# francois-rozet/sda

Measured on AMD Instinct MI355X. Metric: diffusion-steps/s (Kolmogorov 64x256x256 posterior sampling; unit = one predictor-corrector step of a 16-trajectory per-GPU shard), higher is better.
Workload: dtype f32; 1 GPU; kolmogorov256; per_gpu_batch=16, global_batch=16, guided=True, corrections=1, schedule_steps=1000, hipgraph_step=True, observation=fused Subsample (hand-written adjoint; no autograd through A), corrector_noise=row-keyed Philox (sda_randn_rows), parallelism=dp1 (batch-sharded, no in-loop collective), ranks_seen=1, process_group_live=False

## Files before the change

include/sda_hip.h:

```cpp
#ifndef SDA_HIP_H
#define SDA_HIP_H

#include <stdint.h>

#ifdef __cplusplus
extern "C" {
#endif

#define SDA_ABI_VERSION 14

enum {
    SDA_OK = 0,
    SDA_E_BADARG = -1,
    SDA_E_UNSUPPORTED = -2,
    SDA_E_LDS = -3
};

enum { SDA_ACT_NONE = 0, SDA_ACT_SILU = 1, SDA_ACT_RELU = 2, SDA_ACT_ELU = 3, SDA_ACT_GELU = 4, SDA_ACT_SELU = 5 };

int sda_abi_version(void);

typedef struct sda_conv_desc {
    const float* x;
    int64_t x_sn_outer, x_sn_inner;
    int32_t n_inner;
    int32_t x_n_off;
    int64_t x_sc, x_sy, x_sx;
    int32_t cx;
    const float* ctx;
    int64_t ctx_sn;
    int32_t cctx;
    int32_t n;
    int32_t hs, ws;
    int32_t up_h, up_w;
    int32_t zins_h, zins_w;
    const float* mod;
    int64_t mod_sn;
    const float* ln_mean;
    const float* ln_rstd;
    int32_t act_in;
    int32_t kh, kw, stride_h, stride_w, circular;
    const float* w;
    int32_t cin_pad, cout_pad;
    const float* bias;
    float* out;
    int32_t cout, ho, wo;
    const float* dact_z;
    int32_t act_d;
    const float* res;
    int32_t mt;
    int32_t explicit_pad, pad_h, pad_w;
    int64_t out_sn, out_sc, out_sy, out_sx;
    const float* w_wino4;
    int32_t pool_h, pool_w;
    const float* w_wino4_zp;
    const void* w_h2;
    float w_h2_scale;
    float x_amax_static;
    const float* x_amax;
    float* out_amax;
} sda_conv_desc;

int sda_conv_igemm(const sda_conv_desc* d, void* stream);
int sda_conv_parity4(const sda_conv_desc* d, void* stream);
int sda_conv_igemm_path(const sda_conv_desc* d);
int64_t sda_conv_igemm_lds_bytes(const sda_conv_desc* d);

typedef struct sda_wgrad_desc {
    sda_conv_desc conv;
    const float* g;
    float* dw;
    float* db;
    float* work;
    int32_t slabs;
    int32_t accumulate;
} sda_wgrad_desc;

int sda_conv_wgrad(const sda_wgrad_desc* d, void* stream);
int sda_conv_wgrad_slabs(const sda_wgrad_desc* d);
int64_t sda_conv_wgrad_work_floats(const sda_wgrad_desc* d);
int sda_conv_wgrad3_serves(const sda_wgrad_desc* d);
int64_t sda_conv_wgrad3_work_floats(const sda_wgrad_desc* d);
int sda_conv_wgrad3(const sda_wgrad_desc* d, void* stream);
int sda_conv_wgrad3x_serves(const sda_wgrad_desc* d);
int64_t sda_conv_wgrad3x_work_floats(const sda_wgrad_desc* d);
int sda_conv_wgrad3x(const sda_wgrad_desc* d, void* stream);
int sda_plane_sum(const float* x, const float* y, int n, int c, int64_t hw, float* out, int64_t out_sn, int sum_images,
                  int accumulate, void* stream);

typedef struct sda_block1d_desc {
    int32_t n, c, len;
    int32_t circular, act, unbiased;
    float eps;
    int32_t k_pad, m_pad;
    const float* a;
    const float* mod;
    int64_t mod_sn;
    const float* w1; const float* b1;
    const float* w2; const float* b2;
    float* z;
    float* mean; float* rstd;
    float* y;
    const float* g;
    float* gx;
} sda_block1d_desc;
int sda_block1d_fwd(const sda_block1d_desc* d, void* stream);
int sda_block1d_bwd(const sda_block1d_desc* d, void* stream);
int sda_block1d_tile(const sda_block1d_desc* d);

#define SDA_NET1D_MAXB 8
typedef struct sda_net1d_desc {
    int32_t n, len;
    int32_t cin, c, cout;
    int32_t nblocks;
    int32_t circular, act, unbiased;
    float eps;
    const float* x; int64_t x_sn, x_sc, x_sx;
    float* out; int64_t out_sn, out_sc, out_sx;
    const float* w;
    const float* bias;
    const float* mod[SDA_NET1D_MAXB];
    int64_t mod_sn;
    float* a_save; float* z_save; int64_t save_stride;
    float* mean_save; float* rstd_save; int64_t stat_stride;
} sda_net1d_desc;
int sda_net1d_fwd(const sda_net1d_desc* d, void* stream);
int sda_net1d_bwd(const sda_net1d_desc* d, void* stream);

typedef struct sda_net1d_fuse {
    float cx0, cx1, cn;
    const float* coef;
    const float* y; int64_t y_sn;
    int32_t p_start, p_step, p_stop;
    int32_t c_start, c_step, c_stop;
    float std, gamma;
    float* ghat;
    const float* eps;
    int32_t mode;
    float* xs;
    const float* step_coef;
    float* partial; int32_t partial_stride;
} sda_net1d_fuse;
int sda_net1d_fwd_fused(const sda_net1d_desc* d, const sda_net1d_fuse* f, void* stream);
int sda_net1d_bwd_fused(const sda_net1d_desc* d, const sda_net1d_fuse* f, void* stream);
int sda_net1d_tiles(const sda_net1d_desc* d);

typedef struct sda_net1d_train_desc {
    sda_net1d_desc net;
    float* tail_in;
    float* g_save; int64_t g_stride;
    float* mod_part; int32_t mod_tiles;
} sda_net1d_train_desc;
int sda_net1d_fwd_train(const sda_net1d_train_desc* t, void* stream);
int sda_net1d_bwd_train(const sda_net1d_train_desc* t, void* stream);

typedef struct sda_net1d_wgrad_desc {
    sda_net1d_desc net;
    const float* tail_in;
    const float* g_save; int64_t g_stride;
    const float* gout; int64_t gout_sn, gout_sc, gout_sx;
    const float* mod_part; int32_t mod_tiles;
    float* dw[2 + 2 * SDA_NET1D_MAXB];
    float* db[2 + 2 * SDA_NET1D_MAXB];
    float* dmod[SDA_NET1D_MAXB]; int64_t dmod_sn;
    float* work;
    int32_t slabs;
} sda_net1d_wgrad_desc;
int sda_net1d_wgrad(const sda_net1d_wgrad_desc* d, void* stream);
int sda_net1d_wgrad_slabs(const sda_net1d_wgrad_desc* d);
int64_t sda_net1d_wgrad_work_floats(const sda_net1d_wgrad_desc* d);

typedef struct sda_net1d_pack_desc {
    int32_t nblocks, cin, c, cout, cin_keep;
    const float* w[2 + 2 * SDA_NET1D_MAXB];
    const float* b[2 + 2 * SDA_NET1D_MAXB];
    float* wf; float* wb; float* bias;
} sda_net1d_pack_desc;
int sda_net1d_pack(const sda_net1d_pack_desc* p, void* stream);

int sda_step1d_prologue(const float* table, int row_len, int64_t* istep, const float* t_dev, int nt,
                        int alpha_kind, float eta, float k, int sigma_kind,
                        const float* freqs, int nf, const float* w0, const float* b0, int hidden, const float* w2, const float* b2, int e,
                        const float* wp, const float* bp, int cp,
                        float* out_coef, int64_t* out_step, float* mod, void* stream);
int sda_pc_correct_keyed(float* x, const float* eps, int b, int64_t per_sample, const float* partial, int nchunk, float tau,
                         float sigma, const float* coef_dev, uint64_t seed, int64_t row0, const int64_t* draw_dev, int64_t draw_mul,
                         int64_t draw_add, void* stream);

int sda_pack_conv_weight(const float* w, int cout, int cin, int kh, int kw, int transpose, int cin_keep,
                         float* dst, int k_pad, int m_pad, void* stream);

int sda_pack_conv_weight_wino4(const float* w, int cout, int cin, int transpose, int cin_keep, float* dst, int k_pad,
                               int m_pad, void* stream);
int sda_pack_conv_weight_wino4_zp(const float* w_wino4, int k_pad, int m_pad, float* dst, void* stream);
int64_t sda_wino4_zp_floats(int k_pad, int m_pad);

int sda_ln_stats(const float* x, int n, int c, int hw, const float* mod, int64_t mod_sn, float eps, int unbiased,
                 float* mean, float* rstd, void* stream);
int sda_ln_apply(const float* x, int n, int c, int hw, const float* mod, int64_t mod_sn, const float* mean,
                 const float* rstd, float* y, void* stream);
int sda_ln_bwd(const float* gh, const float* x, int n, int c, int h, int w, const float* mod, int64_t mod_sn,
               const float* mean, const float* rstd, int unbiased, int pool_h, int pool_w, const float* res, float* gx,
               void* stream);
int sda_ln_bwd_amax(const float* gh, const float* x, int n, int c, int h, int w, const float* mod, int64_t mod_sn,
                    const float* mean, const float* rstd, int unbiased, int pool_h, int pool_w, const float* res, float* gx,
                    float* amax, void* stream);

int sda_time_embed(const float* t, int nt, const float* freqs, int nf, const float* w0, const float* b0, int hidden,
                   const float* w2, const float* b2, int e, float* emb, void* stream);
int sda_linear_small(const float* x, int rows, int in_f, const float* w, const float* b, int out_f, float* y,
                     void* stream);

int sda_linear(const float* x, int rows, int in_f, const float* w, const float* b, int out_f, int trans_w, int act_in,
// ... 201 lines not shown
```

sda_amd/_lib.py:

```python
import ctypes
import os
from ctypes import POINTER, Structure, c_float, c_int, c_int32, c_int64, c_uint32, c_uint64, c_void_p

import torch

HERE = os.path.dirname(os.path.abspath(__file__))
LIB_PATH = os.environ.get('SDA_HIP_LIB') or os.path.join(HERE, 'lib', 'libsda_hip.so')

ACT_IDS = {None: 0, 'none': 0, 'SiLU': 1, 'ReLU': 2, 'ELU': 3, 'GELU': 4, 'SELU': 5}

c_fp = c_void_p


class ConvDesc(Structure):
    _fields_ = [
        ('x', c_fp),
        ('x_sn_outer', c_int64), ('x_sn_inner', c_int64),
        ('n_inner', c_int32),
        ('x_n_off', c_int32),
        ('x_sc', c_int64), ('x_sy', c_int64), ('x_sx', c_int64),
        ('cx', c_int32),
        ('ctx', c_fp),
        ('ctx_sn', c_int64),
        ('cctx', c_int32),
        ('n', c_int32),
        ('hs', c_int32), ('ws', c_int32),
        ('up_h', c_int32), ('up_w', c_int32),
        ('zins_h', c_int32), ('zins_w', c_int32),
        ('mod', c_fp),
        ('mod_sn', c_int64),
        ('ln_mean', c_fp),
        ('ln_rstd', c_fp),
        ('act_in', c_int32),
        ('kh', c_int32), ('kw', c_int32), ('stride_h', c_int32), ('stride_w', c_int32), ('circular', c_int32),
        ('w', c_fp),
        ('cin_pad', c_int32), ('cout_pad', c_int32),
        ('bias', c_fp),
        ('out', c_fp),
        ('cout', c_int32), ('ho', c_int32), ('wo', c_int32),
        ('dact_z', c_fp),
        ('act_d', c_int32),
        ('res', c_fp),
        ('mt', c_int32),
        ('explicit_pad', c_int32), ('pad_h', c_int32), ('pad_w', c_int32),
        ('out_sn', c_int64), ('out_sc', c_int64), ('out_sy', c_int64), ('out_sx', c_int64),
        ('w_wino4', c_fp),
        ('pool_h', ctypes.c_int32), ('pool_w', ctypes.c_int32),
        ('w_wino4_zp', c_fp),
        ('w_h2', ctypes.c_void_p), ('w_h2_scale', ctypes.c_float), ('x_amax_static', ctypes.c_float),
        ('x_amax', c_fp), ('out_amax', c_fp),
    ]


class Conv3dDesc(Structure):
    _fields_ = [
        ('x', c_fp), ('w', c_fp), ('bias', c_fp), ('z', c_fp), ('res', c_fp), ('out', c_fp),
        ('n', c_int32), ('cin', c_int32), ('cout', c_int32),
        ('in_size', c_int32 * 3), ('out_size', c_int32 * 3),
        ('k', c_int32 * 3), ('pad', c_int32 * 3), ('stride', c_int32 * 3), ('up', c_int32 * 3), ('dil', c_int32 * 3),
        ('circular', c_int32), ('act', c_int32), ('act_in', c_int32),
    ]


class Block1dDesc(Structure):
    _fields_ = [
        ('n', c_int32), ('c', c_int32), ('len', c_int32),
        ('circular', c_int32), ('act', c_int32), ('unbiased', c_int32),
        ('eps', c_float),
        ('k_pad', c_int32), ('m_pad', c_int32),
        ('a', c_fp),
        ('mod', c_fp),
        ('mod_sn', c_int64),
        ('w1', c_fp), ('b1', c_fp),
        ('w2', c_fp), ('b2', c_fp),
        ('z', c_fp),
        ('mean', c_fp), ('rstd', c_fp),
        ('y', c_fp),
        ('g', c_fp),
        ('gx', c_fp),
    ]


NET1D_MAXB = 8


class Net1dDesc(Structure):
    _fields_ = [
        ('n', c_int32), ('len', c_int32),
        ('cin', c_int32), ('c', c_int32), ('cout', c_int32),
        ('nblocks', c_int32),
        ('circular', c_int32), ('act', c_int32), ('unbiased', c_int32),
        ('eps', c_float),
        ('x', c_fp), ('x_sn', c_int64), ('x_sc', c_int64), ('x_sx', c_int64),
        ('out', c_fp), ('out_sn', c_int64), ('out_sc', c_int64), ('out_sx', c_int64),
        ('w', c_fp),
        ('bias', c_fp),
        ('mod', c_fp * NET1D_MAXB),
        ('mod_sn', c_int64),
        ('a_save', c_fp), ('z_save', c_fp), ('save_stride', c_int64),
        ('mean_save', c_fp), ('rstd_save', c_fp), ('stat_stride', c_int64),
    ]


class Net1dTrainDesc(Structure):
    _fields_ = [('net', Net1dDesc), ('tail_in', c_fp), ('g_save', c_fp), ('g_stride', c_int64), ('mod_part', c_fp), ('mod_tiles', c_int32)]


NET1D_MAXV = 2 + 2 * NET1D_MAXB


class Net1dWgradDesc(Structure):
    _fields_ = [
        ('net', Net1dDesc),
        ('tail_in', c_fp),
        ('g_save', c_fp), ('g_stride', c_int64),
        ('gout', c_fp), ('gout_sn', c_int64), ('gout_sc', c_int64), ('gout_sx', c_int64),
        ('mod_part', c_fp), ('mod_tiles', c_int32),
        ('dw', c_fp * NET1D_MAXV),
        ('db', c_fp * NET1D_MAXV),
        ('dmod', c_fp * NET1D_MAXB), ('dmod_sn', c_int64),
        ('work', c_fp),
        ('slabs', c_int32),
    ]


class Net1dPackDesc(Structure):
    _fields_ = [
        ('nblocks', c_int32), ('cin', c_int32), ('c', c_int32), ('cout', c_int32), ('cin_keep', c_int32),
        ('w', c_fp * NET1D_MAXV),
        ('b', c_fp * NET1D_MAXV),
        ('wf', c_fp), ('wb', c_fp), ('bias', c_fp),
    ]


MLP_MAXG = 32


class MlpDesc(Structure):
    _fields_ = [
        ('rows', c_int32), ('ngemm', c_int32),
        ('act', c_int32), ('unbiased', c_int32),
        ('eps', c_float),
        ('kind', c_int32 * MLP_MAXG),
        ('in_f', c_int32 * MLP_MAXG), ('out_f', c_int32 * MLP_MAXG),
        ('w_off', c_int32 * MLP_MAXG), ('b_off', c_int32 * MLP_MAXG),
        ('w', c_fp), ('bias', c_fp),
        ('x', c_fp), ('x_ld', c_int64),
        ('out', c_fp), ('out_ld', c_int64),
        ('a_save', c_fp), ('z_save', c_fp), ('save_stride', c_int64), ('save_ld', c_int32),
        ('mean_save', c_fp), ('rstd_save', c_fp), ('stat_stride', c_int64),
    ]


class MlpTrainDesc(Structure):
    _fields_ = [('mlp', MlpDesc), ('g_save', c_fp), ('g_stride', c_int64), ('g_ld', c_int32)]


class MlpWgradDesc(Structure):
    _fields_ = [
        ('rows', c_int32), ('ngemm', c_int32),
        ('act', c_int32),
        ('kind', c_int32 * MLP_MAXG),
        ('in_f', c_int32 * MLP_MAXG), ('out_f', c_int32 * MLP_MAXG),
        ('src', c_fp * MLP_MAXG), ('src_ld', c_int64 * MLP_MAXG),
        ('mean', c_fp * MLP_MAXG), ('rstd', c_fp * MLP_MAXG),
        ('g', c_fp * MLP_MAXG), ('g_ld', c_int64),
        ('dw', c_fp * MLP_MAXG), ('db', c_fp * MLP_MAXG),
        ('work', c_fp),
        ('slabs', c_int32), ('accumulate', c_int32),
    ]


ADAMW_MAXT = 32


class AdamWDesc(Structure):
    _fields_ = [
        ('ntensor', c_int32),
        ('decay', c_float), ('one_m_beta1', c_float), ('beta2', c_float), ('one_m_beta2', c_float),
        ('step_size', c_float), ('rsqrt_bc2', c_float), ('eps', c_float),
        ('p', c_fp * ADAMW_MAXT), ('g', c_fp * ADAMW_MAXT), ('m', c_fp * ADAMW_MAXT), ('v', c_fp * ADAMW_MAXT),
        ('fwd', c_fp * ADAMW_MAXT), ('bwd', c_fp * ADAMW_MAXT),
        ('numel', c_int64 * ADAMW_MAXT),
        ('pack_kind', c_int32 * ADAMW_MAXT),
        ('out_f', c_int32 * ADAMW_MAXT), ('in_f', c_int32 * ADAMW_MAXT),
        ('blk0', c_int32 * (ADAMW_MAXT + 1)),
    ]


class MlpWin(Structure):
    _fields_ = [
        ('nw', c_int32), ('len', c_int32), ('c', c_int32), ('emb_n', c_int32),
        ('x', c_fp), ('emb', c_fp),
        ('cx0', c_float), ('cx1', c_float), ('cn', c_float),
        ('coef', c_fp),
        ('y', c_fp), ('y_sn', c_int64),
        ('p_start', c_int32), ('p_step', c_int32), ('p_stop', c_int32),
        ('c_start', c_int32), ('c_step', c_int32), ('c_stop', c_int32),
        ('std', c_float), ('gamma', c_float),
        ('eps', c_fp), ('ghat', c_fp),
        ('gwin', c_fp),
    ]

# ... 207 lines not shown
```

sda_amd/build.py:

```python
import hashlib
import os
import subprocess
import sys

HERE = os.path.dirname(os.path.abspath(__file__))
CSRC = os.path.join(HERE, 'csrc')
LIBDIR = os.environ.get('SDA_LIBDIR') or os.path.join(HERE, 'lib')
ARCH = 'gfx950'
SOURCES = ['conv_igemm.hip', 'conv_wino4.hip', 'conv_small1d.hip', 'conv_few.hip', 'conv_par4.hip', 'conv_h2.hip', 'conv3d.hip', 'conv_wgrad.hip', 'conv_wgrad3.hip', 'block1d.hip', 'net1d.hip', 'net1d_train.hip', 'step1d.hip', 'norm.hip', 'elementwise.hip', 'linear.hip', 'mlp1d.hip', 'mlp_train.hip', 'optim.hip', 'train_loss.hip', 'observe.hip', 'metrics.hip', 'noise.hip', 'chain.hip', 'probe.hip']
HIPCC = os.environ.get('HIPCC', '/opt/rocm/bin/hipcc')
EXTRA_FLAGS = os.environ.get('SDA_EXTRA_HIPCC_FLAGS', '').split()
EMU_SOURCES = ['conv_igemm.hip', 'conv_wgrad.hip', 'conv_wgrad3.hip', 'chain.hip', 'mlp_train.hip', 'net1d_train.hip', 'optim.hip']
CONV_PARTS = 4


def _digest(deps, flags=()):
    h = hashlib.sha256()
    for d in deps:
        h.update(os.path.basename(d).encode())
        with open(d, 'rb') as f:
            h.update(f.read())
    h.update(' '.join(flags).encode())
    return h.hexdigest()


def _newer(target, deps, flags=()):
    stamp = target + '.stamp'
    if not os.path.exists(target) or not os.path.exists(stamp):
        return True
    with open(stamp) as f:
        return f.read().strip() != _digest(deps, flags)


def _stamp(target, deps, flags=()):
    with open(target + '.stamp', 'w') as f:
        f.write(_digest(deps, flags))


def _headers():
    hs = [os.path.join(CSRC, f) for f in os.listdir(CSRC) if f.endswith('.hpp')]
    hs.append(os.path.join(os.path.dirname(HERE), 'include', 'sda_hip.h'))
    return hs


def build(force=False, verbose=False):
    os.makedirs(LIBDIR, exist_ok=True)
    objs = []
    hdrs = _headers()
    procs = []
    units = []
    for src in SOURCES:
        if src == 'conv_igemm.hip':
            units += [(src, f'_p{k}', [f'-DSDA_CONV_PART={k}']) for k in range(CONV_PARTS)]
        else:
            units.append((src, '', []))
    for src, suffix, flags in units:
        sp = os.path.join(CSRC, src)
        if not os.path.exists(sp):
            continue
        obj = os.path.join(LIBDIR, src.replace('.hip', suffix + '.o'))
        objs.append(obj)
        cflags = ['-O3', '-std=c++17', '-fPIC', '-ffp-contract=off'] + flags + EXTRA_FLAGS
        if force or _newer(obj, [sp] + hdrs, cflags):
            cmd = [HIPCC, f'--offload-arch={ARCH}'] + cflags + ['-c', sp, '-o', obj]
            if verbose:
                print(' '.join(cmd))
            procs.append((src + suffix, obj, [sp] + hdrs, cflags, subprocess.Popen(cmd, stdout=subprocess.PIPE, stderr=subprocess.STDOUT)))
    for src, obj, deps, cflags, p in procs:
        out, _ = p.communicate()
        if p.returncode != 0:
            raise RuntimeError(f'hipcc failed on {src}:\n{out.decode()}')
        _stamp(obj, deps, cflags)
    lib = os.path.join(LIBDIR, 'libsda_hip.so')
    if force or procs or _newer(lib, objs):
        cmd = [HIPCC, f'--offload-arch={ARCH}', '-shared', '-fPIC', '-o', lib] + objs
        if verbose:
            print(' '.join(cmd))
        subprocess.check_call(cmd)
        _stamp(lib, objs)
    return lib


def build_emu(force=False):
    os.makedirs(LIBDIR, exist_ok=True)
    srcs = [os.path.join(CSRC, f) for f in EMU_SOURCES]
    lib = os.path.join(LIBDIR, 'libsda_emu.so')
    if force or _newer(lib, srcs + _headers()):
        subprocess.check_call([HIPCC, '--offload-host-only', '-DSDA_HOST_EMU', '-O2', '-std=c++17', '-fPIC',
                               '-ffp-contract=off', '-shared'] + srcs + ['-o', lib])
        _stamp(lib, srcs + _headers())
    return lib


if __name__ == '__main__':
    force = '--force' in sys.argv
    if '--emu' in sys.argv:
        print(build_emu(force))
    else:
        print(build(force, verbose=True))
```

sda_amd/csrc/conv_h2.hip:

```cpp
#include "sda_common.hpp"
#include <stdlib.h>
#include <type_traits>

typedef _Float16 h2_h8 __attribute__((ext_vector_type(8)));
typedef float h2_f4 __attribute__((ext_vector_type(4)));
typedef float h2_f16v __attribute__((ext_vector_type(16)));

#define H2_TS 16
#define H2_HS (H2_TS + 2)
#define H2_NPX (H2_HS * H2_HS)
#define H2_CK 16
#define H2_KQ 32
#define H2_PXB 80
#define H2_BTILE (H2_NPX * H2_PXB)
#define H2_ASLAB (9 * 3 * 2 * 1024)
#define H2_STAGE (H2_ASLAB + H2_BTILE)
#define H2_LDS (2 * H2_STAGE)
#define H2_BM 96
#define H2_BM_OF(MB) (32 * (MB))
#define H2_MB_OF(rows) ((rows) % 96 == 0 ? 3 : ((rows) % 64 == 0 ? 2 : 0))
#define H2_PRND 3
#define H2_TARGET_EXP 11

__host__ __device__ __forceinline__ float h2_scale_of(float amax) {
// ... 346 lines not shown
                float bias[16], opnd[2][16];
#pragma unroll
                for (int r = 0; r < 16; ++r) bias[r] = BIAS ? d.bias[co0 + 32 * m + (r & 3) + 8 * (r >> 2) + 4 * (lane >> 5)] : 0.f;
                if (EPI != 0) {
#pragma unroll
                    for (int f = 0; f < 2; ++f)
#pragma unroll
                        for (int r = 0; r < 16; ++r)
                            opnd[f][r] = op[obase + (int64_t)(32 * m + (r & 3) + 8 * (r >> 2)) * osc + (int64_t)(FROW * f) * OW];
                }
#pragma unroll
                for (int f = 0; f < 2; ++f)
#pragma unroll
                    for (int r = 0; r < 16; ++r) {
                        float v = acc[m][f][r] * inv + bias[r];
                        if (EPI == 1) v *= sda_dact(SDA_ACT_SILU, opnd[f][r]);
                        if (EPI == 2) v += opnd[f][r];
                        amax = fmaxf(amax, fabsf(v));
                        if (!(ABL & 8) || v == 1.2345e30f) d.out[obase + (int64_t)(32 * m + (r & 3) + 8 * (r >> 2)) * osc + (int64_t)(FROW * f) * OW] = v;
                    }
            }
        };
        using h2_c0 = std::integral_constant<int, 0>;
        using h2_c1 = std::integral_constant<int, 1>;
        using h2_c2 = std::integral_constant<int, 2>;
        if (d.dact_z) {
            if (d.bias) epilogue(h2_c1{}, std::true_type{}); else epilogue(h2_c1{}, std::false_type{});
        } else if (d.res) {
            if (d.bias) epilogue(h2_c2{}, std::true_type{}); else epilogue(h2_c2{}, std::false_type{});
        } else {
            if (d.bias) epilogue(h2_c0{}, std::true_type{}); else epilogue(h2_c0{}, std::false_type{});
        }
    }
    if (a.out_amax) {
#pragma unroll
        for (int off = 32; off > 0; off >>= 1) amax = fmaxf(amax, __shfl_down(amax, off, SDA_WAVE));
        if (lane == 0) atomicMax(reinterpret_cast<unsigned int*>(a.out_amax), __float_as_uint(amax));
    }
}

__global__ void pack_h2_kernel(const float* __restrict__ w, int cout, int cin, int transpose, float scale, h2_h8* __restrict__ dst,
                               int64_t units, int ntap, int mb) {
    const int64_t u = (int64_t)blockIdx.x * blockDim.x + threadIdx.x;
    if (u >= units) return;
    const int lane = (int)(u & 63);
    int64_t t = u >> 6;
    const int piece = (int)(t & 1); t >>= 1;
    const int m = (int)(t % mb); t /= mb;
    const int tap = (int)(t % ntap); t /= ntap;
    const int M = transpose ? cin : cout, K = transpose ? cout : cin;
    const int nchunk = K / H2_CK;
    const int chunk = (int)(t % nchunk);
    const int ct = (int)(t / nchunk);
    const int row = 32 * mb * ct + 32 * m + (lane & 31);
    h2_h8 out;
#pragma unroll
    for (int i = 0; i < 8; ++i) {
        const int k = H2_CK * chunk + 8 * (lane >> 5) + i;
        float v = 0.f;
        if (row < M) {
            const int co = transpose ? k : row, ci = transpose ? row : k, tp = transpose ? ntap - 1 - tap : tap;
            v = w[((int64_t)co * cin + ci) * ntap + tp] * scale;
        }
        const _Float16 h = (_Float16)v;
        out[i] = piece ? (_Float16)(v - (float)h) : h;
    }
    dst[u] = out;
}

extern "C" int64_t sda_conv_h2_packed_bytes(int cout, int cin, int transpose) {
    const int M = transpose ? cin : cout, K = transpose ? cout : cin;
    const int mb = M > 0 ? H2_MB_OF(M) : 0;
    if (M <= 0 || K <= 0 || !mb || K % H2_KQ) return 0;
    return (int64_t)(M / H2_BM_OF(mb)) * (K / H2_CK) * (9 * mb * 2 * 1024);
}

extern "C" float sda_conv_h2_scale(float amax) { return h2_scale_of(amax); }

extern "C" int sda_pack_conv_weight_h2(const float* w, int cout, int cin, int transpose, float w_amax, void* dst, void* stream) {
    const int64_t bytes = sda_conv_h2_packed_bytes(cout, cin, transpose);
    if (!w || !dst || bytes == 0) return SDA_E_BADARG;
    const int64_t units = bytes / 16;
    hipLaunchKernelGGL(pack_h2_kernel, dim3((unsigned)((units + 255) / 256)), dim3(256), 0, (hipStream_t)stream, w, cout, cin, transpose,
                       h2_scale_of(w_amax), reinterpret_cast<h2_h8*>(dst), units, 9, H2_MB_OF(transpose ? cin : cout));
    return sda_launch_status();
}

extern "C" int64_t sda_conv_h2_up_packed_bytes(int cout, int cin) {
    const int mb = cout > 0 ? H2_MB_OF(cout) : 0;
    if (cout <= 0 || cin <= 0 || !mb || cin % H2_KQ) return 0;
    return (int64_t)4 * (cout / H2_BM_OF(mb)) * (cin / H2_CK) * (4 * mb * 2 * 1024);
}

extern "C" int sda_pack_conv_weight_h2_up(const float* wsum, int cout, int cin, float w_amax, void* dst, void* stream) {
    const int64_t bytes = sda_conv_h2_up_packed_bytes(cout, cin);
    if (!wsum || !dst || bytes == 0) return SDA_E_BADARG;
    const int64_t units = bytes / 16;
    hipLaunchKernelGGL(pack_h2_kernel, dim3((unsigned)((units + 255) / 256)), dim3(256), 0, (hipStream_t)stream, wsum, 4 * cout, cin, 0,
                       h2_scale_of(w_amax), reinterpret_cast<h2_h8*>(dst), units, 4, H2_MB_OF(cout));
    return sda_launch_status();
}

extern "C" int64_t sda_conv_h2_rows_packed_bytes(int rows, int k, int ntap) {
    const int mb = rows > 0 ? H2_MB_OF(rows) : 0;
    if (rows <= 0 || k <= 0 || !mb || k % H2_KQ || (ntap != 1 && ntap != 2 && ntap != 4 && ntap != 9)) return 0;
    return (int64_t)(rows / H2_BM_OF(mb)) * (k / H2_CK) * ((int64_t)ntap * mb * 2 * 1024);
}

extern "C" int sda_pack_conv_weight_h2_rows(const float* w, int rows, int k, int ntap, float w_amax, void* dst, void* stream) {
    const int64_t bytes = sda_conv_h2_rows_packed_bytes(rows, k, ntap);
    if (!w || !dst || bytes == 0) return SDA_E_BADARG;
    const int64_t units = bytes / 16;
    hipLaunchKernelGGL(pack_h2_kernel, dim3((unsigned)((units + 255) / 256)), dim3(256), 0, (hipStream_t)stream, w, rows, k, 0,
                       h2_scale_of(w_amax), reinterpret_cast<h2_h8*>(dst), units, ntap, H2_MB_OF(rows));
    return sda_launch_status();
}

__global__ __launch_bounds__(256) void absmax_kernel(const float* __restrict__ x, int64_t n4, int64_t n, float* __restrict__ amax) {
    float m = 0.f;
    const h2_f4* x4 = reinterpret_cast<const h2_f4*>(x);
    const int64_t stride = (int64_t)gridDim.x * 256;
    int64_t i = (int64_t)blockIdx.x * 256 + threadIdx.x;
    for (; i + 3 * stride < n4; i += 4 * stride) {
        h2_f4 v[4];
#pragma unroll
        for (int k = 0; k < 4; ++k) v[k] = __builtin_nontemporal_load(x4 + i + k * stride);
#pragma unroll
        for (int k = 0; k < 4; ++k) m = fmaxf(fmaxf(fmaxf(m, fabsf(v[k][0])), fabsf(v[k][1])), fmaxf(fabsf(v[k][2]), fabsf(v[k][3])));
    }
    for (; i < n4; i += stride) {
        const h2_f4 v = __builtin_nontemporal_load(x4 + i);
        m = fmaxf(fmaxf(fmaxf(m, fabsf(v[0])), fabsf(v[1])), fmaxf(fabsf(v[2]), fabsf(v[3])));
    }
    if (blockIdx.x == 0 && threadIdx.x < (int)(n - 4 * n4)) m = fmaxf(m, fabsf(x[4 * n4 + threadIdx.x]));
#pragma unroll
    for (int off = 32; off > 0; off >>= 1) m = fmaxf(m, __shfl_down(m, off, SDA_WAVE));
    if ((threadIdx.x & 63) == 0) atomicMax(reinterpret_cast<unsigned int*>(amax), __float_as_uint(m));
}

__global__ void absmax_zero_kernel(float* __restrict__ amax) { amax[0] = 0.f; }

extern "C" int sda_absmax(const float* x, int64_t numel, float* amax, void* stream) {
    if (!x || !amax || numel <= 0 || (reinterpret_cast<uintptr_t>(x) & 15)) return SDA_E_BADARG;
    hipLaunchKernelGGL(absmax_zero_kernel, dim3(1), dim3(1), 0, (hipStream_t)stream, amax);
    const int64_t n4 = numel / 4;
    const int64_t want = (n4 + 255) / 256;
    const unsigned blocks = (unsigned)(want < 1 ? 1 : (want > 2048 ? 2048 : want));
    hipLaunchKernelGGL(absmax_kernel, dim3(blocks), dim3(256), 0, (hipStream_t)stream, x, n4, numel, amax);
    return sda_launch_status();
}

static bool h2_ok(const sda_conv_desc* d) {
    if (!d || !d->x || !d->out || !d->w_h2) return false;
    const bool up = d->up_h == 2 && d->up_w == 2;
    const bool pool = d->pool_h == 2 && d->pool_w == 2;
    const bool zins = d->zins_h == 2 && d->zins_w == 2;
    const bool s2 = d->stride_h == 2 && d->stride_w == 2;
    if (d->kh != 3 || d->kw != 3 || d->explicit_pad || (int)up + (int)pool + (int)zins + (int)s2 > 1) return false;
    if (!(s2 || (d->stride_h == 1 && d->stride_w == 1)) || !(up || (d->up_h == 1 && d->up_w == 1)) ||
        !(zins || (d->zins_h == 1 && d->zins_w == 1)) || !(pool || (d->pool_h <= 1 && d->pool_w <= 1)))
        return false;
    if (d->cctx != 0 || d->n_inner != 1 || d->x_n_off != 0) return false;
    const int ts = (pool || s2) ? 2 * H2_TS : H2_TS;
    const int mb = d->cout > 0 ? H2_MB_OF(d->cout) : 0;
    if (d->cx % H2_KQ || !mb || d->hs % ts || d->ws % ts) return false;
    if (s2 ? (2 * d->ho != d->hs || 2 * d->wo != d->ws) : (d->ho != ((up || zins) ? 2 : 1) * d->hs || d->wo != ((up || zins) ? 2 : 1) * d->ws)) return false;
    if (up && (d->dact_z || d->act_in != SDA_ACT_NONE)) return false;
    if (pool && (d->dact_z || d->res || d->bias || d->ln_mean || d->act_in != SDA_ACT_NONE)) return false;
    if ((zins || s2) && (d->dact_z || d->ln_mean || d->act_in != SDA_ACT_NONE)) return false;
    if (d->out_sn || d->out_sc || d->out_sy || d->out_sx) return false;
    if ((d->ln_mean == nullptr) != (d->ln_rstd == nullptr)) return false;
    if (d->mod && !d->ln_mean) return false;
    if (d->ln_mean && d->act_in != SDA_ACT_NONE) return false;
    if (d->act_in != SDA_ACT_NONE && d->act_in != SDA_ACT_SILU) return false;
    if (d->dact_z && d->act_d != SDA_ACT_SILU) return false;
    if (d->dact_z && d->res) return false;
    if (d->x_sc < 0 || d->x_sy < 0 || d->x_sx < 0 ||
        (int64_t)d->cx * d->x_sc + (int64_t)d->hs * d->x_sy + (int64_t)d->ws * d->x_sx >= (1LL << 31))
        return false;
    const int64_t tiles = (int64_t)d->n * (d->hs / ts) * (d->ws / ts) * (d->cout / H2_BM_OF(mb)) * ((up || zins) ? 4 : 1);
    return tiles >= 1 && tiles <= 0x3fffffffLL;
}

extern "C" int sda_conv_h2_supported(const sda_conv_desc* d) { return h2_ok(d) ? 1 : 0; }

template <int LOADER, int MODE>
static int h2_launch(const sda_conv_desc* d, const h2_args& a, unsigned grid, int lds, int mb, hipStream_t stream) {
    static bool set3[SDA_MAX_DEVICES], set2[SDA_MAX_DEVICES];
    int rc;
    if (mb == 3) {
        if ((rc = sda_raise_dyn_lds(reinterpret_cast<const void*>(conv_h2_kernel<LOADER, MODE, 0, 3>), lds, set3)) != SDA_OK) return rc;
        hipLaunchKernelGGL((conv_h2_kernel<LOADER, MODE, 0, 3>), dim3(grid), dim3(512), (size_t)lds, stream, *d, a);
    } else {
        if ((rc = sda_raise_dyn_lds(reinterpret_cast<const void*>(conv_h2_kernel<LOADER, MODE, 0, 2>), lds, set2)) != SDA_OK) return rc;
        hipLaunchKernelGGL((conv_h2_kernel<LOADER, MODE, 0, 2>), dim3(grid), dim3(512), (size_t)lds, stream, *d, a);
    }
    return sda_launch_status();
}

extern "C" int sda_conv_h2(const sda_conv_desc* d, void* stream) {
    if (!h2_ok(d)) return SDA_E_UNSUPPORTED;
    h2_args a;
    a.w = d->w_h2;
    a.w_scale = d->w_h2_scale;
    a.x_amax = d->x_amax;
    a.x_amax_static = d->x_amax_static;
    a.out_amax = d->out_amax;
    const bool up = d->up_h == 2, pool = d->pool_h == 2, zins = d->zins_h == 2, s2 = d->stride_h == 2;
    const bool planes = pool || s2;
    a.tiles_x = d->ws / (planes ? 2 * H2_TS : H2_TS);
    a.tiles_y = d->hs / (planes ? 2 * H2_TS : H2_TS);
    const int mb = H2_MB_OF(d->cout);
    a.n_ct = (d->cout / H2_BM_OF(mb)) * ((up || zins) ? 4 : 1);
    a.c16 = d->cx / H2_CK;
    a.nchunk = a.c16 * (planes ? 4 : 1);
    a.stagger = 0;
#ifdef SDA_H2_ABLATE
    { static const int stg = getenv("SDA_H2_STAGGER") ? atoi(getenv("SDA_H2_STAGGER")) : 0; a.stagger = stg; }
#endif
    if (!(a.w_scale > 0.f) || (!a.x_amax && !(a.x_amax_static > 0.f))) return SDA_E_BADARG;
    const int lds = H2_LDS;
    a.ntiles = (int)((int64_t)d->n * a.tiles_x * a.tiles_y * a.n_ct);
    int cus = sda_cu_count();
    if (cus <= 0) cus = 256;
    unsigned grid = (unsigned)(a.ntiles < cus ? a.ntiles : cus);
    if (grid >= 8) grid &= ~7u;
    int rc = SDA_OK;
#ifdef SDA_H2_ABLATE
    {
        static const int abl_env = getenv("SDA_H2_ABL") ? atoi(getenv("SDA_H2_ABL")) : 0;
        const int abl = mb == 3 ? abl_env : 0;
        static bool seta[16][SDA_MAX_DEVICES];
        const void* fn = nullptr;
#define H2_ABL_CASE(v) case v: fn = reinterpret_cast<const void*>(conv_h2_kernel<0, 0, v>); \
            if (!d->ln_mean && d->act_in == SDA_ACT_NONE) { if ((rc = sda_raise_dyn_lds(fn, lds, seta[v])) != SDA_OK) return rc; \
                hipLaunchKernelGGL((conv_h2_kernel<0, 0, v>), dim3(grid), dim3(512), (size_t)lds, (hipStream_t)stream, *d, a); return sda_launch_status(); } break;
        switch (abl) {
            H2_ABL_CASE(1) H2_ABL_CASE(2) H2_ABL_CASE(3) H2_ABL_CASE(4) H2_ABL_CASE(7) H2_ABL_CASE(8) H2_ABL_CASE(11) H2_ABL_CASE(15)
            default: break;
        }
    }
#endif
    if (zins) return h2_launch<0, 3>(d, a, grid, lds, mb, (hipStream_t)stream);
    if (s2) return h2_launch<0, 4>(d, a, grid, lds, mb, (hipStream_t)stream);
    if (pool) return h2_launch<0, 2>(d, a, grid, lds, mb, (hipStream_t)stream);
    if (up) return d->ln_mean ? h2_launch<2, 1>(d, a, grid, lds, mb, (hipStream_t)stream) : h2_launch<0, 1>(d, a, grid, lds, mb, (hipStream_t)stream);
    if (d->ln_mean) return h2_launch<2, 0>(d, a, grid, lds, mb, (hipStream_t)stream);
    if (d->act_in != SDA_ACT_NONE) return h2_launch<1, 0>(d, a, grid, lds, mb, (hipStream_t)stream);
    return h2_launch<0, 0>(d, a, grid, lds, mb, (hipStream_t)stream);
}
```

sda_amd/csrc/conv_igemm.hip:

```cpp
#include "sda_common.hpp"
#include <stdlib.h>
#include <string.h>

#ifndef SDA_CONV_CK
#define SDA_CONV_CK 8
#endif
#ifndef SDA_CONV_PART
#define SDA_CONV_PART 0
#endif
#define SDA_CONV_BP 128
#define SDA_CONV_THREADS 256
#define SDA_CONV_MAXPOS 4

struct ConvGeom {
    int cin;
    int hv, wv;
    int pad_h, pad_w;
    int tn, tr, tw;
    int tr_shift, tw_shift;
    int tiles_x, tiles_y, tiles_n;
    int n_pt, n_ct, grid;
    int in_rows, in_cols, plane;
    int S;
    int ntaps;
// ... 556 lines not shown
            float* slab = smem + 2 * BUF + wave * (16 * 32 * NT);
            const int64_t hw_w = g.o_sc;
            const int px4 = (lane & 15) * 4;
            const int64_t gb = conv_pix_out_base(d, g, wave * 32 * NT + px4, n0, oy0, ox0);
            const bool gvalid = gb >= 0;
            const int64_t gbs = gvalid ? gb : 0;
#pragma unroll
            for (int m = 0; m < MT; ++m) {
#pragma unroll
                for (int h = 0; h < 2; ++h) {
#pragma unroll
                    for (int q = 0; q < NT; ++q)
#pragma unroll
                        for (int rr = 0; rr < 8; ++rr)
                            slab[((rr & 3) + 8 * (rr >> 2) + 4 * khalf) * (32 * NT) + q * 32 + l31] = acc[m][q][8 * h + rr];
#pragma unroll
                    for (int it0 = 0; it0 < 4; it0 += 2) {
                        f32x4 val[2], zz[2], rs[2];
                        float bia[2];
#pragma unroll
                        for (int u = 0; u < 2; ++u) {
                            const int lr = (it0 + u) * 4 + (lane >> 4);
                            const int co = co0 + m * 32 + 16 * h + lr;
                            const bool ok = gvalid && co < d.cout;
                            const int64_t off = gbs + (int64_t)(ok ? co : 0) * hw_w;
                            val[u] = *reinterpret_cast<const f32x4*>(slab + lr * (32 * NT) + px4);
                            bia[u] = (d.bias && ok) ? d.bias[co] : 0.f;
                            if (d.dact_z) zz[u] = *reinterpret_cast<const f32x4*>(d.dact_z + off);
                            if (d.res) rs[u] = *reinterpret_cast<const f32x4*>(d.res + off);
                        }
                        if (d.dact_z) {
                            if (d.act_d == SDA_ACT_SILU) {
#pragma unroll
                                for (int u = 0; u < 2; ++u)
#pragma unroll
                                    for (int e = 0; e < 4; ++e) zz[u][e] = sda_dact(SDA_ACT_SILU, zz[u][e]);
                            } else {
#pragma unroll
                                for (int u = 0; u < 2; ++u)
#pragma unroll
                                    for (int e = 0; e < 4; ++e) zz[u][e] = sda_dact(d.act_d, zz[u][e]);
                            }
                        }
#pragma unroll
                        for (int u = 0; u < 2; ++u) {
                            const int lr = (it0 + u) * 4 + (lane >> 4);
                            const int co = co0 + m * 32 + 16 * h + lr;
                            f32x4 v = val[u] + bia[u];
                            if (d.dact_z) v *= zz[u];
                            if (d.res) v += rs[u];
                            if (gvalid && co < d.cout) *reinterpret_cast<f32x4*>(d.out + gbs + (int64_t)co * hw_w) = v;
                        }
                    }
                }
            }
            continue;
        }
        const int64_t hw_o = g.o_sc;
#pragma unroll
        for (int q = 0; q < NT; ++q) {
            const int64_t obase = conv_pix_out_base(d, g, (wave * NT + q) * 32 + l31, n0, oy0, ox0);
            const bool pvalid = obase >= 0;
            const int64_t ob = pvalid ? obase : 0;
#pragma unroll
            for (int m = 0; m < MT; ++m) {
                const int cb = co0 + m * 32 + 4 * khalf;
                float bia[16], zv[16], rv[16];
#pragma unroll
                for (int r = 0; r < 16; ++r) {
                    const int co = cb + (r & 3) + 8 * (r >> 2);
                    const bool ok = pvalid && co < d.cout;
                    const int64_t off = ob + (int64_t)(ok ? co : 0) * hw_o;
                    bia[r] = (d.bias && ok) ? d.bias[co] : 0.f;
                    zv[r] = d.dact_z ? d.dact_z[off] : 0.f;
                    rv[r] = d.res ? d.res[off] : 0.f;
                }
                if (d.dact_z) {
                    if (d.act_d == SDA_ACT_SILU) {
#pragma unroll
                        for (int r = 0; r < 16; ++r) zv[r] = sda_dact(SDA_ACT_SILU, zv[r]);
                    } else {
#pragma unroll
                        for (int r = 0; r < 16; ++r) zv[r] = sda_dact(d.act_d, zv[r]);
                    }
                } else {
#pragma unroll
                    for (int r = 0; r < 16; ++r) zv[r] = 1.f;
                }
#pragma unroll
                for (int r = 0; r < 16; ++r) {
                    const int co = cb + (r & 3) + 8 * (r >> 2);
                    const float v = (acc[m][q][r] + bia[r]) * zv[r] + rv[r];
                    if (pvalid && co < d.cout) d.out[ob + (int64_t)co * hw_o] = v;
                }
            }
        }
        }
    }
}

template <int MT, int NT, int SPAD, int KH, int KW, int CK>
static int conv_launch_ws(const sda_conv_desc* d, const ConvGeom& g, hipStream_t stream) {
    constexpr int lds = conv_ws_lds_bytes(NT, conv_ws_buf_floats(MT, SPAD, KH * KW, CK));
    static_assert(lds <= 160 * 1024, "stage buffers exceed the LDS");
    auto kern = conv_igemm_ws_kernel<MT, NT, SPAD, KH, KW, CK>;
    static bool attr_set[SDA_MAX_DEVICES];
    if (lds > 48 * 1024) {
        const int rc = sda_raise_dyn_lds(reinterpret_cast<const void*>(kern), lds, attr_set);
        if (rc != SDA_OK) return rc;
    }
    const int cus = sda_cu_count();
    if (!cus) return SDA_E_BADARG;
    const int per_cu = (conv_ws_two_per_cu(MT, NT, SPAD, CK) && 2 * lds <= 160 * 1024) ? 2 : 1;
    int grid = cus * per_cu;
    grid -= grid % 8;
    const int need = (g.grid + 7) / 8 * 8;
    if (grid > need) grid = need;
    if (grid < 8) grid = 8;
    hipLaunchKernelGGL(kern, dim3(grid), dim3(512), (size_t)lds, stream, *d, g);
    return sda_launch_status();
}

template <int MT, int NPOS>
static int conv_launch_t(const sda_conv_desc* d, const ConvGeom& g, hipStream_t stream) {
    auto kern = conv_igemm_kernel<MT, NPOS>;
    static bool attr_set[SDA_MAX_DEVICES];
    const int rc = g.lds_bytes > 48 * 1024 ? sda_raise_dyn_lds(reinterpret_cast<const void*>(kern), 160 * 1024, attr_set) : SDA_OK;
    if (rc != SDA_OK) return rc;
    hipLaunchKernelGGL(kern, dim3(g.grid), dim3(SDA_CONV_THREADS), (size_t)g.lds_bytes, stream, *d, g);
    return sda_launch_status();
}

typedef int (*conv_launch_fn)(const sda_conv_desc*, const ConvGeom&, hipStream_t);
conv_launch_fn sda_conv_variant_p0(const ConvPick& p), sda_conv_variant_p1(const ConvPick& p), sda_conv_variant_p2(const ConvPick& p),
    sda_conv_variant_p3(const ConvPick& p);
#define CONV_WS_VARIANT(KH, KW, MT, NT, SPAD, CK) {CONV_WS_PICK(KH, KW, MT, NT, SPAD, CK) conv_launch_ws<MT, NT, SPAD, KH, KW, CK>},
#define CONV_V1_VARIANT(MT, NPOS) {CONV_V1_PICK(MT, NPOS) conv_launch_t<MT, NPOS>},
#define CONV_PART_NAME_(stem, k) stem##k
#define CONV_PART_NAME(stem, k) CONV_PART_NAME_(stem, k)
conv_launch_fn CONV_PART_NAME(sda_conv_variant_p, SDA_CONV_PART)(const ConvPick& p) {
    static const struct { ConvPick pick; conv_launch_fn launch; } rows[] = {
        CONV_PART_NAME(CONV_ROWS_P, SDA_CONV_PART)(CONV_WS_VARIANT, CONV_V1_VARIANT)};
    for (const auto& v : rows)
        if (!memcmp(&v.pick, &p, sizeof(p))) return v.launch;
    return nullptr;
}

#if SDA_CONV_PART == 0
int sda_wino4_try(const sda_conv_desc* d, hipStream_t stream);
int sda_small1d_try(const sda_conv_desc* d, hipStream_t stream);
int sda_few_try(const sda_conv_desc* d, hipStream_t stream);
int sda_wino4_path(const sda_conv_desc* d), sda_small1d_path(const sda_conv_desc* d), sda_few_path(const sda_conv_desc* d);
typedef const sda_conv_desc* conv_dp;
struct ConvTier { bool (*offered)(conv_dp d); int (*run)(conv_dp d, hipStream_t stream); int (*path)(conv_dp d); };
static const ConvTier CONV_TIERS[] = {
    {[](conv_dp d) { return !!d->w_wino4; }, sda_wino4_try, [](conv_dp d) { const int p = sda_wino4_path(d); return p == 2 ? 5 : p ? 2 : 0; }},
    {[](conv_dp d) { return d->pool_h > 1 || d->pool_w > 1; }, nullptr, nullptr},
    {[](conv_dp d) { return d->kh == 1 && d->kw == 3; }, sda_small1d_try, [](conv_dp d) { return sda_small1d_path(d) ? 3 : 0; }},
    {[](conv_dp d) { return d->kh == 3 && d->kw == 3 && d->cout <= 16; }, sda_few_try, [](conv_dp d) { return sda_few_path(d) ? 4 : 0; }},
};

extern "C" int sda_conv_igemm(const sda_conv_desc* d, void* stream) {
    if (!d) return SDA_E_BADARG;
    for (const ConvTier& t : CONV_TIERS) {
        if (!t.offered(d)) continue;
        if (!t.run) return SDA_E_UNSUPPORTED;
        const int rc = t.run(d, (hipStream_t)stream);
        if (rc != SDA_E_UNSUPPORTED) return rc;
    }
    static const ConvSwitches sw = [] {
        const char *v1 = getenv("SDA_CONV_V1"), *nt = getenv("SDA_CONV_NT"), *ck32 = getenv("SDA_CONV_CK32"), *ck16 = getenv("SDA_CONV_CK16");
        return ConvSwitches{v1 != nullptr, nt ? atoi(nt) : 0, !(ck32 && atoi(ck32) == 0), !(ck16 && atoi(ck16) == 0)};
    }();
    ConvGeom g; ConvPick p;
    const int rc = conv_pick(d, sw, &g, &p);
    if (rc != SDA_OK) return rc;
    for (auto part : {sda_conv_variant_p0, sda_conv_variant_p1, sda_conv_variant_p2, sda_conv_variant_p3})
        if (conv_launch_fn launch = part(p)) return launch(d, g, (hipStream_t)stream);
    return SDA_E_UNSUPPORTED;
}

extern "C" int sda_conv_igemm_path(const sda_conv_desc* d) {
    if (!d) return SDA_E_BADARG;
    for (const ConvTier& t : CONV_TIERS) {
        if (!t.offered(d)) continue;
        if (!t.path) return SDA_E_UNSUPPORTED;
        if (const int id = t.path(d)) return id;
    }
    return 0;
}

extern "C" int64_t sda_conv_igemm_lds_bytes(const sda_conv_desc* d) {
    ConvGeom g;
    int rc = conv_plan(d, &g);
    return rc != SDA_OK ? (int64_t)rc : g.lds_bytes;
}


__global__ void pack_conv_weight_kernel(const float* __restrict__ w, int cout, int cin, int kh, int kw, int transpose,
                                        int cin_keep, float* __restrict__ dst, int k_pad, int m_pad) {
    const int64_t total = (int64_t)kh * kw * k_pad * m_pad;
    for (int64_t i = (int64_t)blockIdx.x * blockDim.x + threadIdx.x; i < total; i += (int64_t)gridDim.x * blockDim.x) {
        int mm = (int)(i % m_pad);
        int64_t r = i / m_pad;
        int kk = (int)(r % k_pad);
        int tap = (int)(r / k_pad);
        int dy = tap / kw, dx = tap % kw;
        float v = 0.f;
        if (!transpose) {
            int ci = kk, co = mm;
            if (ci < cin && co < cout) v = w[(((int64_t)co * cin + ci) * kh + dy) * kw + dx];
        } else {
            int co = kk, ci = mm;
            int sdy = kh - 1 - dy, sdx = kw - 1 - dx;
            if (ci < cin_keep && ci < cin && co < cout) v = w[(((int64_t)co * cin + ci) * kh + sdy) * kw + sdx];
        }
        dst[i] = v;
    }
}

extern "C" int sda_pack_conv_weight(const float* w, int cout, int cin, int kh, int kw, int transpose, int cin_keep,
                                    float* dst, int k_pad, int m_pad, void* stream) {
    if (!w || !dst || cout <= 0 || cin <= 0 || kh <= 0 || kw <= 0 || k_pad <= 0 || m_pad <= 0) return SDA_E_BADARG;
    int64_t total = (int64_t)kh * kw * k_pad * m_pad;
    int blocks = (int)((total + 255) / 256);
    if (blocks > 4096) blocks = 4096;
    hipLaunchKernelGGL(pack_conv_weight_kernel, dim3(blocks), dim3(256), 0, (hipStream_t)stream, w, cout, cin, kh, kw,
                       transpose, cin_keep, dst, k_pad, m_pad);
    return sda_launch_status();
}

#endif
#endif

#ifdef SDA_HOST_EMU
#include <vector>
extern "C" int sda_conv_igemm_emulate(const sda_conv_desc* dp) {
    ConvGeom g;
    int rc = conv_plan(dp, &g);
    if (rc != SDA_OK) return rc;
    const sda_conv_desc& d = *dp;
    constexpr int CK = SDA_CONV_CK;
    const int BM = g.bm, MT = d.mt;
    std::vector<float> s_w((size_t)g.ntaps * CK * BM), s_in((size_t)CK * g.S);
    std::vector<float> acc((size_t)SDA_CONV_THREADS * MT * 16);
    for (int b = 0; b < g.grid; ++b) {
        int ct, n0, oy0, ox0;
        conv_decode_block(g, conv_logical_block(b, g.grid), ct, n0, oy0, ox0);
        const int co0 = ct * BM;
        std::fill(acc.begin(), acc.end(), 0.f);
        for (int st = 0; st < g.nstage; ++st) {
            const int c0 = st * CK;
            for (int tid = 0; tid < SDA_CONV_THREADS; ++tid) {
                const int ROW4 = BM / 4, total4 = g.ntaps * CK * ROW4;
                for (int f = tid; f < total4; f += SDA_CONV_THREADS) {
                    int row = f / ROW4, c4 = f - row * ROW4, tap = row / CK, ck = row - tap * CK;
                    const float* src = d.w + ((int64_t)tap * d.cin_pad + c0 + ck) * d.cout_pad + co0 + c4 * 4;
                    for (int q = 0; q < 4; ++q) s_w[(size_t)row * BM + c4 * 4 + q] = src[q];
                }
                for (int pos = tid; pos < g.S; pos += SDA_CONV_THREADS) {
                    ConvPos ps = conv_decode_pos(d, g, pos, n0, oy0, ox0);
                    float mean = 0.f, rstd = 1.f;
                    if (d.ln_mean && ps.xoff >= 0) { mean = d.ln_mean[ps.stat]; rstd = d.ln_rstd[ps.stat]; }
                    for (int ck = 0; ck < CK; ++ck) s_in[(size_t)ck * g.S + pos] = conv_load_value(d, g, ps, c0 + ck, mean, rstd);
                }
            }
            for (int wave = 0; wave < 4; ++wave) {
                int dy = 0, dx = 0;
                for (int tap = 0; tap < g.ntaps; ++tap) {
                    for (int k2 = 0; k2 < CK / 2; ++k2) {
                        for (int m = 0; m < MT; ++m) {
                            float A[32][2], B[2][32];
                            for (int lane = 0; lane < 64; ++lane) {
                                int l31 = lane & 31, kh_ = lane >> 5, ck = 2 * k2 + kh_;
                                int pix = wave * 32 + l31;
                                int toff = dy * g.in_cols + dx + conv_pix_lds_base(d, g, pix);
                                B[kh_][l31] = s_in[(size_t)ck * g.S + toff];
                                A[l31][kh_] = s_w[((size_t)tap * CK + ck) * BM + m * 32 + l31];
                            }
                            for (int lane = 0; lane < 64; ++lane)
                                for (int r = 0; r < 16; ++r) {
                                    int i = mfma32_row(r, lane), j = lane & 31;
                                    float& c = acc[((size_t)(wave * 64 + lane) * MT + m) * 16 + r];
                                    c = fmaf(A[i][0], B[0][j], c);
                                    c = fmaf(A[i][1], B[1][j], c);
                                }
                        }
                    }
                    if (++dx == d.kw) { dx = 0; ++dy; }
                }
            }
        }
        for (int tid = 0; tid < SDA_CONV_THREADS; ++tid) {
            int lane = tid & 63, wave = tid >> 6, pix = wave * 32 + (lane & 31);
            int64_t obase = conv_pix_out_base(d, g, pix, n0, oy0, ox0);
            for (int m = 0; m < MT; ++m)
                for (int r = 0; r < 16; ++r)
                    conv_epilogue_store(d, g, obase, co0 + m * 32 + mfma32_row(r, lane), acc[((size_t)tid * MT + m) * 16 + r]);
        }
    }
    return SDA_OK;
}

extern "C" int sda_conv_igemm_pick(const sda_conv_desc* d, int force_v1, int nt, int ck32, int ck16, int out[16]) {
    ConvGeom g; ConvPick p;
    const int rc = conv_pick(d, ConvSwitches{force_v1 != 0, nt, ck32 != 0, ck16 != 0}, &g, &p);
    if (rc != SDA_OK) return rc;
    const int lds = p.kernel ? conv_ws_lds_bytes(p.nt, conv_ws_buf_floats(p.mt, p.spad, p.kh * p.kw, p.ck)) : (int)g.lds_bytes;
    const int geom[8] = {g.tn, g.tr, g.tw, g.S, g.grid, g.nstage, g.wide_out, lds};
    memcpy(out, &p, sizeof(p));
    memcpy(out + 8, geom, sizeof(geom));
    return SDA_OK;
}
extern "C" int sda_conv_igemm_variants(int* out, int cap) {
    static const ConvPick rows[] = {CONV_ROWS_P0(CONV_WS_PICK, CONV_V1_PICK) CONV_ROWS_P1(CONV_WS_PICK, CONV_V1_PICK)
                                    CONV_ROWS_P2(CONV_WS_PICK, CONV_V1_PICK) CONV_ROWS_P3(CONV_WS_PICK, CONV_V1_PICK)};
    if (cap >= (int)(sizeof(rows) / sizeof(rows[0]))) memcpy(out, rows, sizeof(rows));
    return (int)(sizeof(rows) / sizeof(rows[0]));
}

extern "C" void sda_pack_conv_weight_host(const float* w, int cout, int cin, int kh, int kw, int transpose, int cin_keep,
                                          float* dst, int k_pad, int m_pad) {
    const int64_t total = (int64_t)kh * kw * k_pad * m_pad;
    for (int64_t i = 0; i < total; ++i) {
        int mm = (int)(i % m_pad);
        int64_t r = i / m_pad;
        int kk = (int)(r % k_pad), tap = (int)(r / k_pad), dy = tap / kw, dx = tap % kw;
        float v = 0.f;
        if (!transpose) {
            if (kk < cin && mm < cout) v = w[(((int64_t)mm * cin + kk) * kh + dy) * kw + dx];
        } else {
            int sdy = kh - 1 - dy, sdx = kw - 1 - dx;
            if (mm < cin_keep && mm < cin && kk < cout) v = w[(((int64_t)kk * cin + mm) * kh + sdy) * kw + sdx];
        }
        dst[i] = v;
    }
// ... 3 lines not shown
```

sda_amd/csrc/conv_par4.hip:

```cpp
#include "sda_common.hpp"
#include <stdlib.h>

#define P4_CK 8
#define P4_TR 8
#define P4_TW 16
#define P4_HR (P4_TR + 1)
#define P4_HC (P4_TW + 1)
#define P4_NPOS (P4_HR * P4_HC)
#define P4_PLANE 176
#define P4_BM_OF(MT) (32 * (MT))
#define P4_WSZ_OF(MT) (9 * P4_CK * P4_BM_OF(MT))
#define P4_BUF_OF(MT) (P4_WSZ_OF(MT) + P4_CK * P4_PLANE)
#define P4_NLD ((P4_CK * P4_NPOS + 255) / 256)
#define P4_NW_OF(MT) ((P4_WSZ_OF(MT) / 4 + 255) / 256)

typedef float p4_f32x16 __attribute__((ext_vector_type(16)));
typedef float p4_f32x2 __attribute__((ext_vector_type(2)));

__device__ constexpr int P4_CL[9] = {0, 1, 1, 2, 2, 3, 3, 3, 3};
__device__ constexpr int P4_DY[9] = {0, 0, 0, 0, 1, 0, 0, 1, 1};
__device__ constexpr int P4_DX[9] = {0, 0, 1, 0, 0, 0, 1, 0, 1};

template <int MT>
__global__ __launch_bounds__(512, 2) void conv_par4_kernel(const sda_conv_desc d, int tiles_x, int tiles_y, int n_ct) {
    constexpr int P4_BM = P4_BM_OF(MT), P4_WSZ = P4_WSZ_OF(MT), P4_BUF = P4_BUF_OF(MT), P4_NW = P4_NW_OF(MT);
    extern __shared__ __attribute__((aligned(16))) float smem[];
    const int tid = threadIdx.x, lane = tid & 63, l31 = lane & 31, khalf = lane >> 5;
    const int wave = __builtin_amdgcn_readfirstlane(tid >> 6);
    int t = blockIdx.x;
    const int ct = t % n_ct; t /= n_ct;
    const int bx = t % tiles_x; t /= tiles_x;
    const int by = t % tiles_y;
    const int n = t / tiles_y;
    const int oy0 = by * P4_TR, ox0 = bx * P4_TW, co0 = ct * P4_BM;
    const int nstage = d.cin_pad / P4_CK;
    if (wave >= 4) {
        const int ptid = tid - 256;
        const float* gimg = d.x + (int64_t)n * d.x_sn_outer;
        unsigned goff[P4_NLD];
        int loff[P4_NLD];
        unsigned live = 0;
#pragma unroll
        for (int i = 0; i < P4_NLD; ++i) {
            const int e = ptid + 256 * i;
            const bool in = e < P4_CK * P4_NPOS;
            const int ch = in ? e / P4_NPOS : 0, pos = in ? e - ch * P4_NPOS : 0;
            const int hy = pos / P4_HC, hx = pos - hy * P4_HC;
            int y = oy0 + hy, x = ox0 + hx;
            bool ok = in;
            if (d.circular) {
                y = y >= d.hs ? y - d.hs : y;
                x = x >= d.ws ? x - d.ws : x;
            } else {
                ok = ok && y < d.hs && x < d.ws;
            }
            goff[i] = (unsigned)(ch * (int)d.x_sc + (ok ? y : 0) * (int)d.x_sy + (ok ? x : 0) * (int)d.x_sx);
            loff[i] = in ? P4_WSZ + ch * P4_PLANE + hy * P4_HC + hx : -1;
            live |= ok ? (1u << i) : 0u;
        }
        unsigned woff[P4_NW];
#pragma unroll
        for (int i = 0; i < P4_NW; ++i) {
            const int f = ptid + 256 * i;
            const int row = f / (P4_BM / 4), c4 = f - row * (P4_BM / 4);
            const int tap = row / P4_CK, ck = row - tap * P4_CK;
            woff[i] = (unsigned)((tap * d.cin_pad + ck) * d.cout_pad + co0 + 4 * c4);
        }
        auto produce = [&](int st, float* buf) {
            const float* ws = d.w + (int64_t)(st * P4_CK) * d.cout_pad;
#pragma unroll
            for (int i = 0; i < P4_NW; ++i) {
                const int f = ptid + 256 * i;
                if (i + 1 < P4_NW || f < P4_WSZ / 4)
                    __builtin_amdgcn_global_load_lds((const __attribute__((address_space(1))) void*)(ws + woff[i]),
                                                     (__attribute__((address_space(3))) void*)(buf + (f - lane) * 4), 16, 0, 0);
            }
            const float* xs = gimg + (int64_t)(st * P4_CK) * d.x_sc;
            float vin[P4_NLD];
#pragma unroll
            for (int i = 0; i < P4_NLD; ++i) vin[i] = xs[goff[i]];
#pragma unroll
            for (int i = 0; i < P4_NLD; ++i)
                if (loff[i] >= 0) buf[loff[i]] = ((live >> i) & 1u) ? vin[i] : 0.f;
            asm volatile("s_waitcnt vmcnt(0)" ::: "memory");
        };
        produce(0, smem);
        __syncthreads();
        for (int st = 0; st < nstage; ++st) {
            if (st + 1 < nstage) produce(st + 1, smem + ((st + 1) & 1) * P4_BUF);
            __syncthreads();
        }
        return;
    }
    p4_f32x16 acc[4][MT];
#pragma unroll
    for (int c = 0; c < 4; ++c)
#pragma unroll
        for (int m = 0; m < MT; ++m)
#pragma unroll
            for (int r = 0; r < 16; ++r) acc[c][m][r] = 0.f;
    const int bbase = P4_WSZ + khalf * P4_PLANE + (2 * wave + (l31 >> 4)) * P4_HC + (l31 & 15);
    const int abase = khalf * P4_BM + l31;
    __syncthreads();
    for (int st = 0; st < nstage; ++st) {
        const float* buf = smem + (st & 1) * P4_BUF;
#pragma unroll
        for (int k2 = 0; k2 < P4_CK / 2; ++k2) {
            float b[4];
#pragma unroll
            for (int o = 0; o < 4; ++o) b[o] = buf[bbase + 2 * k2 * P4_PLANE + (o >> 1) * P4_HC + (o & 1)];
#pragma unroll
            for (int tap = 0; tap < 9; ++tap) {
                float a[MT];
#pragma unroll
                for (int m = 0; m < MT; ++m) a[m] = buf[abase + (tap * P4_CK + 2 * k2) * P4_BM + 32 * m];
#pragma unroll
                for (int m = 0; m < MT; ++m)
                    acc[P4_CL[tap]][m] = __builtin_amdgcn_mfma_f32_32x32x2f32(a[m], b[2 * P4_DY[tap] + P4_DX[tap]], acc[P4_CL[tap]][m], 0, 0, 0);
            }
        }
        __syncthreads();
    }
    const int oy = oy0 + 2 * wave + (l31 >> 4), ox = ox0 + (l31 & 15);
    const int64_t row_sz = d.out_sy / 2;
    const int64_t pbase = (int64_t)n * d.out_sn + (int64_t)oy * d.out_sy + (int64_t)ox * d.out_sx;
    const int64_t cbase = pbase + (int64_t)(co0 + 4 * khalf) * d.out_sc;
#pragma unroll
    for (int m = 0; m < MT; ++m)
#pragma unroll
        for (int rh = 0; rh < 2; ++rh) {
            p4_f32x2 rv[16];
#pragma unroll
            for (int j = 0; j < 8; ++j) {
                const int r = 8 * rh + j;
                const int64_t o = cbase + (int64_t)(32 * m + (r & 3) + 8 * (r >> 2)) * d.out_sc;
#pragma unroll
                for (int py = 0; py < 2; ++py)
                    rv[2 * j + py] = d.res ? *reinterpret_cast<const p4_f32x2*>(d.res + o + py * row_sz) : p4_f32x2{0.f, 0.f};
            }
#pragma unroll
            for (int j = 0; j < 8; ++j) {
                const int r = 8 * rh + j;
                const int64_t o = cbase + (int64_t)(32 * m + (r & 3) + 8 * (r >> 2)) * d.out_sc;
#pragma unroll
                for (int py = 0; py < 2; ++py) {
                    const p4_f32x2 v = p4_f32x2{acc[2 * py][m][r], acc[2 * py + 1][m][r]} + rv[2 * j + py];
                    *reinterpret_cast<p4_f32x2*>(d.out + o + py * row_sz) = v;
                }
            }
        }
}

static bool par4_ok(const sda_conv_desc* d) {
    static const bool off = getenv("SDA_CONV_PAR4") && atoi(getenv("SDA_CONV_PAR4")) == 0;
    if (off || !d || !d->x || !d->w || !d->out) return false;
    if (d->kh != 2 || d->kw != 2 || !d->explicit_pad || d->pad_h != 0 || d->pad_w != 0 || d->stride_h != 1 || d->stride_w != 1 ||
        d->up_h != 1 || d->up_w != 1 || d->zins_h != 1 || d->zins_w != 1)
        return false;
    if (d->cctx != 0 || d->mod || d->ln_mean || d->ln_rstd || d->act_in != SDA_ACT_NONE || d->dact_z || d->bias || d->n_inner != 1 ||
        d->x_n_off != 0)
        return false;
    if ((d->cout % 32) || d->cout_pad != d->cout || d->cin_pad % P4_CK || d->cx != d->cin_pad) return false;
    if (d->ho != d->hs || d->wo != d->ws || (d->ho % P4_TR) || (d->wo % P4_TW)) return false;
    if (d->out_sx != 2 || d->out_sy != 4 * (int64_t)d->wo || d->out_sc != 4 * (int64_t)d->ho * d->wo ||
        d->out_sn != d->out_sc * d->cout)
        return false;
    if ((reinterpret_cast<uintptr_t>(d->out) & 7) || (d->res && (reinterpret_cast<uintptr_t>(d->res) & 7)) ||
        (reinterpret_cast<uintptr_t>(d->w) & 15) || (d->cout_pad & 3))
        return false;
    if (d->x_sc < 0 || d->x_sy < 0 || d->x_sx < 0 ||
        (int64_t)d->cx * d->x_sc + (int64_t)d->hs * d->x_sy + (int64_t)d->ws * d->x_sx >= (1LL << 31))
        return false;
    if ((int64_t)9 * d->cin_pad * d->cout_pad >= (1LL << 31)) return false;
    const int64_t tiles = (int64_t)d->n * (d->ho / P4_TR) * (d->wo / P4_TW) * (d->cout / P4_BM_OF(d->cout % 96 == 0 ? 3 : (d->cout % 64 == 0 ? 2 : 1)));
    return tiles >= 1 && tiles <= 0x7fffffffLL;
}

template <int MT>
static int par4_launch(const sda_conv_desc* d, hipStream_t stream) {
    static bool attr_set[SDA_MAX_DEVICES];
    const int lds = 2 * P4_BUF_OF(MT) * 4;
    const int rc = sda_raise_dyn_lds(reinterpret_cast<const void*>(conv_par4_kernel<MT>), lds, attr_set);
    if (rc != SDA_OK) return rc;
    const int tx = d->wo / P4_TW, ty = d->ho / P4_TR, n_ct = d->cout / P4_BM_OF(MT);
    hipLaunchKernelGGL(conv_par4_kernel<MT>, dim3((unsigned)((int64_t)d->n * tx * ty * n_ct)), dim3(512), (size_t)lds, stream, *d, tx, ty, n_ct);
    return sda_launch_status();
}

extern "C" int sda_conv_parity4(const sda_conv_desc* d, void* stream) {
    if (!par4_ok(d)) return SDA_E_UNSUPPORTED;
    return d->cout % 96 == 0 ? par4_launch<3>(d, (hipStream_t)stream)
                             : (d->cout % 64 == 0 ? par4_launch<2>(d, (hipStream_t)stream) : par4_launch<1>(d, (hipStream_t)stream));
}
```

sda_amd/csrc/conv_wino4.hip:

```cpp
#include "sda_common.hpp"
#include <stdlib.h>
#include <type_traits>

#define W4_CK 8
#define W4_BM_OF(MF) (32 * (MF))
#define W4_T 32
#define W4_HC 18
#define W4_HRW 10
#define W4_HS 24
#define W4_HPLANE (W4_HRW * W4_HS)
#define W4_NSLOT 3
#define W4_UPP_OF(MF) (2 * (MF) * 64 * 4)
#define W4_UBUF_OF(MF) (8 * W4_UPP_OF(MF))
#define W4_NULZ_OF(MF) ((MF) == 3 ? 7 : (MF) == 2 ? 5 : 3)
#define W4_UZP_OF(MF) (W4_NULZ_OF(MF) * 4 * 256)
#define W4_VKQ 128
#define W4_VPP (4 * W4_VKQ)
#define W4_VBUF (8 * W4_VPP)
#define W4_LDS_BYTES_OF(MF) ((2 * W4_UBUF_OF(MF) + 2 * W4_VBUF + 4 * 2 * W4_HPLANE) * 4)

struct Wino4Geom {
    int cin, hv, wv;
    int bx_n, by_n;
    int n_ct, grid, nstage, debug, mtiles;
    int walk;
    int sc, sx, sy, sn;
    long long* trace;
    int mf;
};

typedef float f32x4 __attribute__((ext_vector_type(4)));
typedef float f32x2 __attribute__((ext_vector_type(2)));
typedef unsigned w4_u32x2 __attribute__((ext_vector_type(2)));

template <int I, int N, class F>
__device__ __forceinline__ void w4_static_for(F&& f) {
    if constexpr (I < N) {
        f(std::integral_constant<int, I>{});
        w4_static_for<I + 1, N>(f);
    }
}

static int wino4_config(const sda_conv_desc* d);

int sda_wino4_plan(const sda_conv_desc* d, Wino4Geom* g) {
    if (!d || !d->x || !d->w_wino4 || !d->out) return SDA_E_UNSUPPORTED;
    if (d->kh != 3 || d->kw != 3 || d->stride_h != 1 || d->stride_w != 1 || d->zins_h != 1 || d->zins_w != 1)
        return SDA_E_UNSUPPORTED;
    if (d->explicit_pad || d->out_sn || d->out_sc || d->out_sy || d->out_sx) return SDA_E_UNSUPPORTED;
    if (d->cctx < 0 || (d->cctx > 0 && !d->ctx) || (d->cout % 32) || d->cout_pad != d->cout || d->cin_pad % W4_CK || d->cin_pad < d->cx) return SDA_E_UNSUPPORTED;
    if ((d->ho & 7) || (d->wo & 15) || d->ho != d->hs * d->up_h || d->wo != d->ws * d->up_w) return SDA_E_UNSUPPORTED;
    if (d->up_h > 2 || d->up_w > 2 || d->up_h < 1 || d->up_w < 1) return SDA_E_UNSUPPORTED;
    if (d->pool_h > 1 || d->pool_w > 1) {
        if (!d->w_wino4_zp || (reinterpret_cast<uintptr_t>(d->w_wino4_zp) & 15)) return SDA_E_UNSUPPORTED;
        if (d->pool_h != 2 || d->pool_w != 2 || d->mod || d->ln_mean || d->act_in != SDA_ACT_NONE || d->res || d->dact_z || d->cctx ||
            (reinterpret_cast<uintptr_t>(d->out) & 3))
            return SDA_E_UNSUPPORTED;
    }
    if (d->mod && d->mod_sn != 0) return SDA_E_UNSUPPORTED;
    if (d->act_in != SDA_ACT_NONE && d->act_in != SDA_ACT_SILU) return SDA_E_UNSUPPORTED;
    if ((d->ln_mean == nullptr) != (d->ln_rstd == nullptr)) return SDA_E_UNSUPPORTED;
    if (wino4_config(d) < 0) return SDA_E_UNSUPPORTED;
    if ((reinterpret_cast<uintptr_t>(d->out) & 7) || (d->res && (reinterpret_cast<uintptr_t>(d->res) & 7)) ||
        (d->dact_z && (reinterpret_cast<uintptr_t>(d->dact_z) & 7)) || (reinterpret_cast<uintptr_t>(d->w_wino4) & 15) ||
        (d->bias && (reinterpret_cast<uintptr_t>(d->bias) & 15)))
        return SDA_E_UNSUPPORTED;
    if (d->x_sc < 0 || d->x_sy < 0 || d->x_sx < 0 || d->n_inner < 1) return SDA_E_UNSUPPORTED;
    if (d->cctx > 0 && (d->x_sy != d->ws || d->x_sx != 1 || d->mod || d->ln_mean || d->act_in != SDA_ACT_NONE || d->up_h != 1 ||
                        d->up_w != 1 || d->ctx_sn < 0 || (int64_t)d->cctx * d->hs * d->ws >= (1LL << 28)))
        return SDA_E_UNSUPPORTED;
    if ((int64_t)d->cx * d->x_sc + (int64_t)d->hs * d->x_sy + (int64_t)d->ws * d->x_sx >= (1LL << 30)) return SDA_E_UNSUPPORTED;
    if ((int64_t)48 * d->ho * d->wo * 4 >= (1LL << 31)) return SDA_E_UNSUPPORTED;
    if ((int64_t)d->cout * d->ho * d->wo >= (1LL << 30) || (int64_t)d->n * d->hs * d->ws >= (1LL << 31)) return SDA_E_UNSUPPORTED;
    g->cin = d->cx + d->cctx;
    g->hv = d->ho; g->wv = d->wo;
    g->bx_n = d->wo / 16; g->by_n = d->ho / 8;
    g->mf = d->cout % 96 == 0 ? 3 : (d->cout % 64 == 0 ? 2 : 1);
    g->n_ct = d->cout / W4_BM_OF(g->mf);
    g->mtiles = d->cout / 16;
    const int64_t total = (int64_t)g->bx_n * g->by_n * d->n * g->n_ct;
    if (total > 0x3fffffffLL || total < 1) return SDA_E_UNSUPPORTED;
    g->grid = (int)total;
    g->nstage = d->cin_pad / W4_CK;
    if ((int64_t)g->nstage * total > 0x7fffffffLL) return SDA_E_UNSUPPORTED;
#ifdef SDA_W4_VARIANTS
    g->debug = sda_debug_env();
#else
    { static const int dbg = sda_debug_env(); g->debug = dbg; }
#endif
    g->trace = nullptr;
    g->walk = 1; g->sc = 1; g->sx = 0; g->sy = 0; g->sn = 0;
    return SDA_OK;
}

struct W4Tile { int ct, n, by, bx; };
__device__ __forceinline__ W4Tile w4_decode(const Wino4Geom& g, int tile) {
    W4Tile t;
    t.ct = tile % g.n_ct;
    int rest = tile / g.n_ct;
    t.bx = rest % g.bx_n; rest /= g.bx_n;
    t.by = rest % g.by_n;
    t.n = rest / g.by_n;
    return t;
}

struct W4Cur { int st, ct, bx, by, n; };
__device__ __forceinline__ int w4_eq(int a, int n) { return (int)(((unsigned)(n - a) - 1u) >> 31); }
__device__ __forceinline__ int w4_ge(int a, int n) { return (int)((unsigned)(n - 1 - a) >> 31); }
__device__ __forceinline__ void w4_advance(const Wino4Geom& g, W4Cur& c) {
    const int t_next = w4_eq(c.st + 1, g.nstage);
    c.st = (c.st + 1) * (1 - t_next);
    const int ct = c.ct + t_next * g.sc;
    const int cc = w4_ge(ct, g.n_ct);
    c.ct = ct - cc * g.n_ct;
    const int bx = c.bx + t_next * g.sx + cc;
    const int cx = w4_ge(bx, g.bx_n);
    c.bx = bx - cx * g.bx_n;
    const int by = c.by + t_next * g.sy + cx;
    const int cy = w4_ge(by, g.by_n);
    c.by = by - cy * g.by_n;
    c.n += t_next * g.sn + cy;
}

#define W4_DBG(b) SDA_DBG(g, b)
#define W4_TRACE_DECL long long w4tr_[8] = {0, 0, 0, 0, 0, 0, 0, 0}; long long w4tl_ = 0, w4tb_ = 0; (void)w4tr_; (void)w4tl_; (void)w4tb_; if constexpr (VAR == 11) w4tb_ = __builtin_readcyclecounter()
#define W4_T0() do { if constexpr (VAR == 11) w4tl_ = __builtin_readcyclecounter(); } while (0)
#define W4_STAMP(k) do { if constexpr (VAR == 11) if (!SDA_DBG(g, 4096)) { const long long n_ = __builtin_readcyclecounter(); w4tr_[k] += n_ - w4tl_; w4tl_ = n_; } } while (0)
#define W4_MARK(v) do { if constexpr (VAR == 11) if SDA_DBG(g, 8192) asm volatile("s_memtime %0" : "=s"(v) :: "memory"); } while (0)
#define W4_MARK_ADD(k, a, b) do { if constexpr (VAR == 11) if SDA_DBG(g, 8192) w4tr_[k] += (long long)((b) - (a)); } while (0)
#define W4_MARK_WAIT() do { if constexpr (VAR == 11) if SDA_DBG(g, 8192) asm volatile("s_waitcnt lgkmcnt(0)" ::: "memory"); } while (0)
#define W4_TRACE_OUT() do { if constexpr (VAR == 11) { w4tr_[7] = __builtin_readcyclecounter() - w4tb_; if (g.trace && lane == 0) for (int k_ = 0; k_ < 8; ++k_) g.trace[(blockIdx.x * 8 + wave) * 8 + k_] = w4tr_[k_]; } } while (0)

__device__ __forceinline__ void w4_ld1(float& dst, const char* base, unsigned off) {
    asm volatile("s_nop 4\n\tglobal_load_dword %0, %1, %2" : "=v"(dst) : "v"(off), "s"(base) : "memory");
}
__device__ __forceinline__ void w4_ld2(f32x2& dst, const char* base, unsigned off) {
    asm volatile("s_nop 4\n\tglobal_load_dwordx2 %0, %1, %2" : "=v"(dst) : "v"(off), "s"(base) : "memory");
}
template <int OFF>
__device__ __forceinline__ void w4_ld4(f32x4& dst, const char* base, unsigned off) {
    asm volatile("s_nop 4\n\tglobal_load_dwordx4 %0, %1, %2 offset:%3" : "=v"(dst) : "v"(off), "s"(base), "n"(OFF) : "memory");
}


__device__ __forceinline__ f32x2 w4_dsilu2(f32x2 z) {
    z = f32x2{__builtin_fmaxf(z[0], -80.f), __builtin_fmaxf(z[1], -80.f)};
    const f32x2 t = z * f32x2{-1.4426950408889634f, -1.4426950408889634f};
    const f32x2 e = {__builtin_amdgcn_exp2f(t[0]), __builtin_amdgcn_exp2f(t[1])};
    const f32x2 dn = e + f32x2{1.f, 1.f};
    const f32x2 sg = {__builtin_amdgcn_rcpf(dn[0]), __builtin_amdgcn_rcpf(dn[1])};
    const f32x2 u = z * e;
    const f32x2 w = __builtin_elementwise_fma(u, sg, f32x2{1.f, 1.f});
    return sg * w;
}

template <int ZP>
__host__ __device__ constexpr bool w4_dead(int p) { return ZP != 0 && ((p >> 2) == 2 || (p & 3) == 2); }

template <bool MOD, bool LN, bool SILU, int EPM, int VAR = 0, int ZP = 0, int MF = 3>
__global__ __launch_bounds__(512, 2) void conv_wino4_kernel(const sda_conv_desc d, const Wino4Geom g) {
    static_assert(MF >= 1 && MF <= 3, "cout tile = 32, 64 or 96");
    static_assert(MF == 3 || EPM != 1, "the helper-fed epilogue operand exists for the 96-cout tile only");
    static_assert(MF > 1 || ZP != 1, "the 32-cout tile has no up-sampled zero-position form");
    constexpr bool ZPOS = ZP != 0;
    constexpr bool EPI = EPM == 1;
    constexpr int W4_BM = W4_BM_OF(MF), W4_UPP = W4_UPP_OF(MF), W4_UBUF = W4_UBUF_OF(MF), W4_UZP = W4_UZP_OF(MF);
    constexpr int W4_LDS_BYTES = W4_LDS_BYTES_OF(MF);
    constexpr int NULZ = W4_NULZ_OF(MF);
    constexpr int NUF = 4 * MF;
    (void)W4_BM; (void)W4_UZP; (void)W4_LDS_BYTES; (void)NULZ; (void)NUF;
    extern __shared__ __attribute__((aligned(16))) float smem[];
    const int tid = threadIdx.x, lane = tid & 63;
    const int wave = __builtin_amdgcn_readfirstlane(tid >> 6);
    float* const ubuf = smem;
    float* const vbuf = smem + 2 * W4_UBUF;

    const int xcd = blockIdx.x & 7, slot = blockIdx.x >> 3, per_xcd = gridDim.x >> 3;
    const int tq = g.grid >> 3, tr_ = g.grid & 7;
    const int t_begin = xcd * tq + (xcd < tr_ ? xcd : tr_);
    const int t_cnt = tq + (xcd < tr_ ? 1 : 0);
    int first, my_tiles;
    if (g.walk) {
        first = t_begin + slot;
        my_tiles = slot < t_cnt ? (t_cnt - slot + per_xcd - 1) / per_xcd : 0;
    } else {
        const int sq = t_cnt / per_xcd, sr = t_cnt % per_xcd;
        first = t_begin + slot * sq + (slot < sr ? slot : sr);
        my_tiles = sq + (slot < sr ? 1 : 0);
    }
    if (my_tiles <= 0) return;
    const int Q = my_tiles * g.nstage;
    W4Cur c0;
    {
        const W4Tile t0 = w4_decode(g, first);
        c0.st = 0; c0.ct = t0.ct; c0.bx = t0.bx; c0.by = t0.by; c0.n = t0.n;
    }

    if (wave >= 4) {
        const int pw = wave - 4;
        if (W4_DBG(8192)) return;
        float* const priv = smem + 2 * W4_UBUF + 2 * W4_VBUF + pw * (2 * W4_HPLANE);
        int hy[W4_NSLOT], hx[W4_NSLOT], lidx[W4_NSLOT];
#pragma unroll
        for (int i = 0; i < W4_NSLOT; ++i) {
            const int pos = lane + 64 * i;
            const bool valid = pos < W4_HRW * W4_HC;
            hy[i] = valid ? pos / W4_HC : -1000;
            hx[i] = valid ? pos - W4_HC * (pos / W4_HC) : 0;
            lidx[i] = valid ? (pos / W4_HC) * W4_HS + hx[i] : W4_HS - 1;
        }
        const int up_sh_h = d.up_h == 2 ? 1 : 0, up_sh_w = d.up_w == 2 ? 1 : 0;
        const bool circ = d.circular != 0;
        constexpr int NSL = ZP == 1 ? 1 : W4_NSLOT;
        const int sj = lane / 10, si = lane - 10 * (lane / 10);
        int lidx4[4];
        {
            const int r0 = 2 * sj - 1 < 0 ? 0 : 2 * sj - 1, r1 = 2 * sj > W4_HRW - 1 ? W4_HRW - 1 : 2 * sj;
            const int q0 = 2 * si - 1 < 0 ? 0 : 2 * si - 1, q1 = 2 * si > W4_HC - 1 ? W4_HC - 1 : 2 * si;
            const bool sv = lane < 60;
            lidx4[0] = sv ? r0 * W4_HS + q0 : W4_HS - 1; lidx4[1] = sv ? r0 * W4_HS + q1 : W4_HS - 1;
            lidx4[2] = sv ? r1 * W4_HS + q0 : W4_HS - 1; lidx4[3] = sv ? r1 * W4_HS + q1 : W4_HS - 1;
        }
        const int pe = lane >> 5;
        const int pbase = pe * W4_HPLANE + (2 * ((lane & 31) >> 3)) * W4_HS + 2 * (lane & 7);
        const int vwr = pw * W4_VKQ + lane * 2;
        const unsigned lane16 = lane * 16u;

        unsigned goff[W4_NSLOT], gstat[W4_NSLOT] = {0u, 0u, 0u}, glive = 0;
        const float* gimg = d.x;
        const float* gctx = d.ctx;
        auto geometry = [&](const W4Cur& t) {
            const int m_img = t.n + d.x_n_off;
            const int m_out = d.n_inner == 1 ? m_img : m_img / d.n_inner;
            gimg = d.x + (int64_t)m_out * d.x_sn_outer + (int64_t)(m_img - m_out * d.n_inner) * d.x_sn_inner;
            if (d.cctx > 0) gctx = d.ctx + (int64_t)t.n * d.ctx_sn;
            glive = 0;
            if constexpr (ZP == 1) {
                const int sy0 = 4 * t.by - 1 + sj, sx0 = 8 * t.bx - 1 + si;
                const bool inside = sy0 >= 0 && sy0 < d.hs && sx0 >= 0 && sx0 < d.ws;
                const int syw = sy0 < 0 ? sy0 + d.hs : (sy0 >= d.hs ? sy0 - d.hs : sy0);
                const int sxw = sx0 < 0 ? sx0 + d.ws : (sx0 >= d.ws ? sx0 - d.ws : sx0);
                const bool ok = lane < 60 && (circ || inside);
                const int sy = ok ? syw : 0, sx = ok ? sxw : 0;
                goff[0] = (unsigned)(sy * (int)d.x_sy + sx * (int)d.x_sx) * 4u;
                glive = ok ? 1u : 0u;
                if constexpr (LN) gstat[0] = (unsigned)((t.n * d.hs + sy) * d.ws + sx) * 4u;
                return;
            }
#pragma unroll
            for (int i = 0; i < W4_NSLOT; ++i) {
                const int vy0 = 8 * t.by - 1 + hy[i], vx0 = 16 * t.bx - 1 + hx[i];
                const bool inside = vy0 >= 0 && vy0 < g.hv && vx0 >= 0 && vx0 < g.wv;
                const int vyw = vy0 < 0 ? vy0 + g.hv : (vy0 >= g.hv ? vy0 - g.hv : vy0);
                const int vxw = vx0 < 0 ? vx0 + g.wv : (vx0 >= g.wv ? vx0 - g.wv : vx0);
                const bool ok = (hy[i] >= 0) && (circ || inside);
                const int vy = ok ? vyw : 0, vx = ok ? vxw : 0;
                const int sy = vy >> up_sh_h, sx = vx >> up_sh_w;
                goff[i] = (unsigned)(sy * (int)d.x_sy + sx * (int)d.x_sx) * 4u;
                glive |= ok ? (1u << i) : 0u;
                if constexpr (LN) gstat[i] = (unsigned)((t.n * d.hs + sy) * d.ws + sx) * 4u;
            }
        };
        struct Halo { float v[2][W4_NSLOT]; float mean[W4_NSLOT], rstd[W4_NSLOT], mv[2]; unsigned live; };
        auto issue = [&](const W4Cur& t, Halo& h) {
#pragma unroll
            for (int ch = 0; ch < 2; ++ch) {
                const int cc = W4_CK * t.st + 2 * pw + ch;
                const int cce = cc < g.cin ? cc : 0;
                const char* xc = reinterpret_cast<const char*>(gimg + (int64_t)cce * d.x_sc);
                if (cce >= d.cx) xc = reinterpret_cast<const char*>(gctx + (int64_t)(cce - d.cx) * (d.hs * d.ws));
#pragma unroll
                for (int i = 0; i < NSL; ++i) w4_ld1(h.v[ch][i], xc, goff[i]);
                if constexpr (MOD) w4_ld1(h.mv[ch], reinterpret_cast<const char*>(d.mod + cce), 0u);
            }
            if constexpr (LN) {
#pragma unroll
                for (int i = 0; i < NSL; ++i) {
                    w4_ld1(h.mean[i], reinterpret_cast<const char*>(d.ln_mean), gstat[i]);
                    w4_ld1(h.rstd[i], reinterpret_cast<const char*>(d.ln_rstd), gstat[i]);
                }
            }
        };
        auto tag = [&](Halo& h) { h.live = glive; };
#define W4_WAIT_HALO(N, h)                                                                                                     \
    do {                                                                                                                       \
        asm volatile("s_waitcnt vmcnt(%6)" : "+v"((h).v[0][0]), "+v"((h).v[0][1]), "+v"((h).v[0][2]), "+v"((h).v[1][0]),         \
                     "+v"((h).v[1][1]), "+v"((h).v[1][2]) : "n"((N) > 63 ? 63 : (N)) : "memory");    \
        if constexpr (LN) asm volatile("" : "+v"((h).mean[0]), "+v"((h).mean[1]), "+v"((h).mean[2]), "+v"((h).rstd[0]),        \
                                       "+v"((h).rstd[1]), "+v"((h).rstd[2]) :: "memory");                                      \
        if constexpr (MOD) asm volatile("" : "+v"((h).mv[0]), "+v"((h).mv[1]) :: "memory");                                    \
    } while (0)
        const bool raw_commit = !MOD && !LN && !SILU && circ && (g.cin % W4_CK) == 0;
        auto commit_raw = [&](const Halo& h) {
#pragma unroll
            for (int ch = 0; ch < 2; ++ch)
#pragma unroll
                for (int i = 0; i < W4_NSLOT; ++i) priv[ch * W4_HPLANE + lidx[i]] = h.v[ch][i];
        };
        auto commit = [&](const W4Cur& t, const Halo& h) {
#pragma unroll
            for (int ch = 0; ch < 2; ++ch) {
                const int cc = W4_CK * t.st + 2 * pw + ch;
                const bool real = cc < g.cin;
                if constexpr (ZP == 1) {
                    float v = h.v[ch][0];
                    if constexpr (MOD) v += h.mv[ch];
                    if constexpr (LN) v = (v - h.mean[0]) * h.rstd[0];
                    if constexpr (SILU) v = sda_act(SDA_ACT_SILU, v);
                    v = (real && (h.live & 1u)) ? v : 0.f;
#pragma unroll
                    for (int k = 0; k < 4; ++k) priv[ch * W4_HPLANE + lidx4[k]] = v;
                    continue;
                }
                float val[W4_NSLOT];
// ... 354 lines not shown
                        const int p = 2 * s + h;
                        if (w4_dead<ZP>(p)) continue;
                        if constexpr (VAR == 12 || VAR == 14) { if (k4 == 1) continue; }
                        if constexpr (VAR == 13 || VAR == 15) { if (k4 == 1 || m == 2) continue; }
                        f32x4 c;
                        if (FIRST && k4 == 0) c = (p == 5) ? binit[m] : f32x4{0.f, 0.f, 0.f, 0.f};
                        else c = acc[p][m];
                        const float aop = (ZPOS && s == 7) ? av7[m][k4] : ((ZPOS && s == 1) ? av[s & 1][m][k4] : av[s & 1][m][2 * h + k4]);
                        acc[p][m] = __builtin_amdgcn_mfma_f32_16x16x4f32(aop, bv[s & 1][k4][h], c, 0, 0, 0);
                    }
            if constexpr (MF == 1) {
                if constexpr (s == 6) {
                    __builtin_amdgcn_sched_group_barrier(0x100, 3, 0);
                    __builtin_amdgcn_sched_group_barrier(0x008, 4, 0);
                } else if constexpr (nmfma == 2) {
                    __builtin_amdgcn_sched_group_barrier(0x008, 1, 0);
                    __builtin_amdgcn_sched_group_barrier(0x100, 3, 0);
                    __builtin_amdgcn_sched_group_barrier(0x008, 1, 0);
                } else {
                    __builtin_amdgcn_sched_group_barrier(0x008, 1, 0);
                    __builtin_amdgcn_sched_group_barrier(0x100, 2, 0);
                    __builtin_amdgcn_sched_group_barrier(0x008, 1, 0);
                    __builtin_amdgcn_sched_group_barrier(0x100, 1, 0);
                    __builtin_amdgcn_sched_group_barrier(0x008, 2, 0);
                }
            } else if constexpr (MF == 2) {
                if constexpr (s == 6) {
                    __builtin_amdgcn_sched_group_barrier(0x100, 4, 0);
                    __builtin_amdgcn_sched_group_barrier(0x008, 8, 0);
                } else if constexpr (nmfma == 4) {
                    __builtin_amdgcn_sched_group_barrier(0x008, 1, 0);
                    __builtin_amdgcn_sched_group_barrier(0x100, 2, 0);
                    __builtin_amdgcn_sched_group_barrier(0x008, 1, 0);
                    __builtin_amdgcn_sched_group_barrier(0x100, 1, 0);
                    __builtin_amdgcn_sched_group_barrier(0x008, 1, 0);
                    __builtin_amdgcn_sched_group_barrier(0x100, 1, 0);
                    __builtin_amdgcn_sched_group_barrier(0x008, 1, 0);
                } else {
                    __builtin_amdgcn_sched_group_barrier(0x008, 1, 0);
                    __builtin_amdgcn_sched_group_barrier(0x100, 2, 0);
                    __builtin_amdgcn_sched_group_barrier(0x008, 2, 0);
                    __builtin_amdgcn_sched_group_barrier(0x100, 1, 0);
                    __builtin_amdgcn_sched_group_barrier(0x008, 2, 0);
                    __builtin_amdgcn_sched_group_barrier(0x100, 1, 0);
                    __builtin_amdgcn_sched_group_barrier(0x008, 3, 0);
                }
            } else if constexpr (s == 6) {
                __builtin_amdgcn_sched_group_barrier(0x100, 5, 0);
                __builtin_amdgcn_sched_group_barrier(0x008, 12, 0);
            } else if constexpr (nmfma == 6) {
                __builtin_amdgcn_sched_group_barrier(0x008, 1, 0);
                __builtin_amdgcn_sched_group_barrier(0x100, 2, 0);
                __builtin_amdgcn_sched_group_barrier(0x008, 1, 0);
                __builtin_amdgcn_sched_group_barrier(0x100, 1, 0);
                __builtin_amdgcn_sched_group_barrier(0x008, 1, 0);
                __builtin_amdgcn_sched_group_barrier(0x100, 1, 0);
                __builtin_amdgcn_sched_group_barrier(0x008, 1, 0);
                __builtin_amdgcn_sched_group_barrier(0x100, 1, 0);
                __builtin_amdgcn_sched_group_barrier(0x008, 2, 0);
            } else {
                __builtin_amdgcn_sched_group_barrier(0x008, 1, 0);
                __builtin_amdgcn_sched_group_barrier(0x100, 2, 0);
                __builtin_amdgcn_sched_group_barrier(0x008, 3, 0);
                __builtin_amdgcn_sched_group_barrier(0x100, 1, 0);
                __builtin_amdgcn_sched_group_barrier(0x008, 3, 0);
                __builtin_amdgcn_sched_group_barrier(0x100, 1, 0);
                __builtin_amdgcn_sched_group_barrier(0x008, 3, 0);
                __builtin_amdgcn_sched_group_barrier(0x100, 1, 0);
                __builtin_amdgcn_sched_group_barrier(0x008, 2, 0);
            }
            __builtin_amdgcn_sched_barrier(0);
            if constexpr (!FIRST && s == 0) c0.st += 1;
            if constexpr (s == 3) {
                W4_STAMP(0);
                unsigned long long mc0 = 0, mc1 = 0;
                W4_MARK(mc0);
                __builtin_amdgcn_s_barrier();
                asm volatile("" ::: "memory");
                if constexpr (VAR == 11) if SDA_DBG(g, 8192) asm volatile("s_memtime %0\n\ts_waitcnt lgkmcnt(0)" : "=s"(mc1), "+s"(mc0) :: "memory");
                W4_MARK_ADD(1, mc0, mc1);
                W4_STAMP(1);
                __builtin_amdgcn_sched_barrier(0);
            }
            if constexpr (s == 6) {
                asm volatile("s_waitcnt lgkmcnt(0)" ::: "memory");
                W4_STAMP(0);
                __builtin_amdgcn_s_barrier();
                asm volatile("" ::: "memory");
                W4_STAMP(3);
                __builtin_amdgcn_sched_barrier(0);
            }
            if constexpr (s == 7) W4_STAMP(0);
        });
        ++q;
    };
    for (int tl = 0; tl < my_tiles; ++tl) {
        f32x4 binit[MF];
        int lane_b;
        asm volatile("v_mbcnt_lo_u32_b32 %0, -1, 0\n\tv_mbcnt_hi_u32_b32 %0, -1, %0" : "=v"(lane_b));
        if constexpr (EPM == 2) {
            ard = (MF * wm * 64 + lane_b) * 4;
            brd = (lane_b >> 4) * W4_VKQ + (16 * wn + (lane_b & 15)) * 2;
        }
#pragma unroll
        for (int m = 0; m < MF; ++m) {
            binit[m] = f32x4{0.f, 0.f, 0.f, 0.f};
            if (d.bias) binit[m] = *reinterpret_cast<const f32x4*>(d.bias + W4_BM * c0.ct + 16 * MF * wm + 16 * m + 4 * (lane_b >> 4));
        }
        stage(std::true_type{}, binit);
        constexpr bool PRE = EPM == 2 && MF < 3;
        f32x2 pre0[PRE ? MF : 1][4], pre1[PRE ? MF : 1][4];
        for (int st = 1; st < g.nstage - (PRE ? 1 : 0); ++st) {
            stage(std::false_type{}, binit);
        }
        if constexpr (PRE) {
            const int hw_p = d.ho * d.wo;
            int lane_p;
            asm volatile("v_mbcnt_lo_u32_b32 %0, -1, 0\n\tv_mbcnt_hi_u32_b32 %0, -1, %0" : "=v"(lane_p));
            const int tp_ = 16 * wn + (lane_p & 15);
            const int lo0p = ((4 * (lane_p >> 4)) * hw_p + (8 * c0.by + 2 * (tp_ >> 3)) * d.wo + 16 * c0.bx + 2 * (tp_ & 7)) * 4, lo1p = lo0p + d.wo * 4;
            const float* pp = d.dact_z ? d.dact_z : d.res;
            const auto r_pre = __builtin_amdgcn_make_buffer_rsrc(const_cast<float*>(pp + ((int64_t)c0.n * d.cout + W4_BM * c0.ct + 16 * MF * wm) * hw_p),
                                                                 (short)0, 16 * MF * hw_p * 4, 0x00020000);
#pragma unroll
            for (int m = 0; m < MF; ++m)
#pragma unroll
                for (int r = 0; r < 4; ++r) {
                    pre0[m][r] = __builtin_bit_cast(f32x2, __builtin_amdgcn_raw_buffer_load_b64(r_pre, lo0p, (16 * m + r) * hw_p * 4, 0));
                    pre1[m][r] = __builtin_bit_cast(f32x2, __builtin_amdgcn_raw_buffer_load_b64(r_pre, lo1p, (16 * m + r) * hw_p * 4, 0));
                }
            __builtin_amdgcn_sched_barrier(0);
            if (g.nstage > 1) stage(std::false_type{}, binit);
        }
        {
            const W4Cur& tt = c0;
            const int hw_o = d.ho * d.wo;
            int lane_e;
            asm volatile("v_mbcnt_lo_u32_b32 %0, -1, 0\n\tv_mbcnt_hi_u32_b32 %0, -1, %0" : "=v"(lane_e));
            const int li_e = lane_e & 15, kq_e = lane_e >> 4;
            const int t = 16 * wn + li_e;
            const int oy = 8 * tt.by + 2 * (t >> 3), ox = 16 * tt.bx + 2 * (t & 7);
            const int lo0 = ((4 * kq_e) * hw_o + oy * d.wo + ox) * 4, lo1 = lo0 + d.wo * 4;
            const int64_t sbase = ((int64_t)tt.n * d.cout + W4_BM * tt.ct + 16 * MF * wm) * hw_o;
            const int plane_bytes = 16 * MF * hw_o * 4;
            auto rsrc_of = [&](const float* p) {
                return __builtin_amdgcn_make_buffer_rsrc(const_cast<float*>(p + sbase), (short)0, plane_bytes, 0x00020000);
            };
            auto run = [&](auto DACT_, auto RES_) {
                constexpr int DACT_KIND = decltype(DACT_)::value;
                constexpr bool DACT = DACT_KIND != 0, RES = decltype(RES_)::value;
                const auto r_out = rsrc_of(d.out);
                const auto r_z = rsrc_of(DACT ? d.dact_z : d.out);
                const auto r_res = rsrc_of(RES ? d.res : d.out);
                const float* el = ubuf + ((q + 1) & 1) * W4_UBUF + (wave * 8 * MF * 64 + lane_e) * 2;
                f32x2 el0[MF > 1 ? 4 * (MF - 1) : 1], el1[MF > 1 ? 4 * (MF - 1) : 1];
#pragma unroll
                for (int m = 0; m < MF; ++m) {
                    if constexpr (EPM != 0) __builtin_amdgcn_sched_barrier(0);
                    f32x4 s0[4], s1[4];
#pragma unroll
                    for (int nu = 0; nu < 4; ++nu) {
                        s0[nu] = (acc[nu][m] + acc[4 + nu][m]) + acc[8 + nu][m];
                        s1[nu] = (acc[4 + nu][m] - acc[8 + nu][m]) - acc[12 + nu][m];
                    }
                    const f32x4 y00 = (s0[0] + s0[1]) + s0[2], y01 = (s0[1] - s0[2]) - s0[3];
                    const f32x4 y10 = (s1[0] + s1[1]) + s1[2], y11 = (s1[1] - s1[2]) - s1[3];
                    if constexpr (EPI) {
                        if (m == 0) {
                            asm volatile("" :: "v"(y00), "v"(y01), "v"(y10), "v"(y11));
                            __builtin_amdgcn_sched_barrier(0);
                            __builtin_amdgcn_s_barrier();
                            asm volatile("" ::: "memory");
                        }
                    }
                    if constexpr (EPI) {
                        if (m == 1) {
#pragma unroll
                            for (int r = 0; r < 4 * (MF - 1); ++r) {
                                el0[r] = *reinterpret_cast<const f32x2*>(el + ((4 + r) * 2 + 0) * 128);
                                el1[r] = *reinterpret_cast<const f32x2*>(el + ((4 + r) * 2 + 1) * 128);
                            }
                            asm volatile("s_waitcnt lgkmcnt(0)" ::: "memory");
                            __builtin_amdgcn_s_barrier();
                            asm volatile("" ::: "memory");
                        }
                    }
#pragma unroll
                    for (int r = 0; r < 4; ++r) {
                        if constexpr (DACT_KIND == 1) { if (r == 2) __builtin_amdgcn_sched_barrier(0); }
                        const int so = (16 * m + r) * hw_o * 4;
                        f32x2 y0 = {y00[r], y01[r]}, y1 = {y10[r], y11[r]};
                        f32x2 e0, e1;
                        if constexpr (EPI) {
                            if (m >= 1) { e0 = el0[4 * (m - 1) + r]; e1 = el1[4 * (m - 1) + r]; }
                            else {
                                e0 = *reinterpret_cast<const f32x2*>(el + ((4 * m + r) * 2 + 0) * 128);
                                e1 = *reinterpret_cast<const f32x2*>(el + ((4 * m + r) * 2 + 1) * 128);
                            }
                        }
                        if constexpr (DACT) {
                            f32x2 q0, q1;
                            if constexpr (EPI) { q0 = e0; q1 = e1; }
                            else if constexpr (PRE) { q0 = pre0[m][r]; q1 = pre1[m][r]; }
                            else {
                                q0 = __builtin_bit_cast(f32x2, __builtin_amdgcn_raw_buffer_load_b64(r_z, lo0, so, 0));
                                q1 = __builtin_bit_cast(f32x2, __builtin_amdgcn_raw_buffer_load_b64(r_z, lo1, so, 0));
                            }
                            if (DACT_KIND == 1 || d.act_d == SDA_ACT_SILU) {
                                y0 *= w4_dsilu2(q0);
                                y1 *= w4_dsilu2(q1);
                            } else {
                                y0[0] *= sda_dact(d.act_d, q0[0]); y0[1] *= sda_dact(d.act_d, q0[1]);
                                y1[0] *= sda_dact(d.act_d, q1[0]); y1[1] *= sda_dact(d.act_d, q1[1]);
                            }
                        }
                        if constexpr (RES) {
                            if constexpr (EPI) { y0 += e0; y1 += e1; }
                            else if constexpr (PRE && !DACT) { y0 += pre0[m][r]; y1 += pre1[m][r]; }
                            else {
                                y0 += __builtin_bit_cast(f32x2, __builtin_amdgcn_raw_buffer_load_b64(r_res, lo0, so, 0));
                                y1 += __builtin_bit_cast(f32x2, __builtin_amdgcn_raw_buffer_load_b64(r_res, lo1, so, 0));
                            }
                        }
                        if (!SDA_DBG(g, 8)) {
                            __builtin_amdgcn_raw_buffer_store_b64(__builtin_bit_cast(w4_u32x2, y0), r_out, lo0, so, 0);
                            __builtin_amdgcn_raw_buffer_store_b64(__builtin_bit_cast(w4_u32x2, y1), r_out, lo1, so, 0);
                        }
                    }
                }
            };
            using K0 = std::integral_constant<int, 0>;
            using K1 = std::integral_constant<int, 1>;
            using K2 = std::integral_constant<int, 2>;
            if constexpr (ZP == 2) {
                const int wo_p = d.wo >> 1, hw_p = (d.ho >> 1) * wo_p;
                const int lo_p = ((4 * kq_e) * hw_p + (4 * tt.by + (t >> 3)) * wo_p + 8 * tt.bx + (t & 7)) * 4;
                const int64_t sbase_p = ((int64_t)tt.n * d.cout + W4_BM * tt.ct + 16 * MF * wm) * hw_p;
                const auto r_p = __builtin_amdgcn_make_buffer_rsrc(d.out + sbase_p, (short)0, 16 * MF * hw_p * 4, 0x00020000);
#pragma unroll
                for (int m = 0; m < MF; ++m) {
                    const f32x4 c0v = (acc[0][m] + 2.f * acc[4][m]) - acc[12][m];
                    const f32x4 c1v = (acc[1][m] + 2.f * acc[5][m]) - acc[13][m];
                    const f32x4 c3v = (acc[3][m] + 2.f * acc[7][m]) - acc[15][m];
                    const f32x4 y = (c0v + 2.f * c1v) - c3v;
#pragma unroll
                    for (int r = 0; r < 4; ++r) {
                        const float yr = y[r];
                        __builtin_amdgcn_raw_buffer_store_b32(__float_as_uint(yr), r_p, lo_p, (16 * m + r) * hw_p * 4, 0);
                    }
                }
            } else if constexpr (EPM == 0) {
                run(K0{}, std::false_type{});
            } else if constexpr (EPI) {
                if (d.dact_z) run(K1{}, std::false_type{});
                else run(K0{}, std::true_type{});
            } else if (d.dact_z) {
                if (d.res) run(K2{}, std::true_type{});
                else run(K2{}, std::false_type{});
            } else {
                if (d.res) run(K0{}, std::true_type{});
                else run(K0{}, std::false_type{});
            }
        }
        w4_advance(g, c0);
        W4_STAMP(2);
    }
    W4_TRACE_OUT();
}

#ifdef SDA_W4_VARIANTS
static long long* w4_trace_buf = nullptr;
static int w4_trace_grid = 0;
extern "C" int sda_w4_trace_read(double* out) {
    if (!w4_trace_buf || !out) return SDA_E_BADARG;
    static long long host[256 * 64];
    if (hipMemcpy(host, w4_trace_buf, sizeof(host), hipMemcpyDeviceToHost) != hipSuccess) return SDA_E_BADARG;
    for (int i = 0; i < 64; ++i) {
        double s = 0;
        for (int b = 0; b < w4_trace_grid; ++b) s += (double)host[b * 64 + i];
        out[i] = s / w4_trace_grid;
    }
    return SDA_OK;
}
#endif

template <bool MOD, bool LN, bool SILU, int EPI, int VAR, int ZP, int MF>
static int wino4_launch_mf(const sda_conv_desc* d, const Wino4Geom& g, int grid, hipStream_t stream) {
    static_assert(W4_LDS_BYTES_OF(MF) <= 160 * 1024, "LDS");
    static bool attr_set[SDA_MAX_DEVICES];
    const int rc = sda_raise_dyn_lds(reinterpret_cast<const void*>(conv_wino4_kernel<MOD, LN, SILU, EPI, VAR, ZP, MF>), W4_LDS_BYTES_OF(MF), attr_set);
    if (rc != SDA_OK) return rc;
    hipLaunchKernelGGL((conv_wino4_kernel<MOD, LN, SILU, EPI, VAR, ZP, MF>), dim3(grid), dim3(512), (size_t)W4_LDS_BYTES_OF(MF), stream, *d, g);
    return sda_launch_status();
}

template <bool MOD, bool LN, bool SILU, int EPI, int VAR, int ZP = 0>
static int wino4_launch_t(const sda_conv_desc* d, const Wino4Geom& g, int grid, hipStream_t stream) {
    if constexpr ((VAR == 0 || VAR == 11) && EPI != 1) {
        if (g.mf == 2) return wino4_launch_mf<MOD, LN, SILU, EPI, VAR, ZP, 2>(d, g, grid, stream);
        if constexpr (ZP != 1 && VAR == 0) {
            if (g.mf == 1) return wino4_launch_mf<MOD, LN, SILU, EPI, VAR, ZP, 1>(d, g, grid, stream);
        }
    }
    if (g.mf != 3) return SDA_E_UNSUPPORTED;
    return wino4_launch_mf<MOD, LN, SILU, EPI, VAR, ZP, 3>(d, g, grid, stream);
}

static int wino4_config(const sda_conv_desc* d) {
    const bool mod = d->mod != nullptr, ln = d->ln_mean != nullptr, silu = d->act_in == SDA_ACT_SILU;
    const int key = (mod ? 4 : 0) | (ln ? 2 : 0) | (silu ? 1 : 0);
    return (key == 0 || key == 1 || key == 2 || key == 6) ? key : -1;
}

static int wino4_epm(const sda_conv_desc* d, const Wino4Geom& g) {
    static const bool epi_on = !(getenv("SDA_W4_EPI") && atoi(getenv("SDA_W4_EPI")) == 0);
    const bool epi = epi_on && g.mf == 3 && ((d->res != nullptr) != (d->dact_z != nullptr)) && g.nstage >= 12 &&
                     (!d->dact_z || d->act_d == SDA_ACT_SILU);
    return epi ? 1 : ((d->res || d->dact_z) ? 2 : 0);
}

static int wino4_zp(const sda_conv_desc* d, const Wino4Geom& g) {
    static const bool zp_on = !(getenv("SDA_W4_ZP") && atoi(getenv("SDA_W4_ZP")) == 0);
    if (d->pool_h > 1 || d->pool_w > 1) return 2;
    if (!(zp_on && d->w_wino4_zp && !(reinterpret_cast<uintptr_t>(d->w_wino4_zp) & 15) && d->up_h == 2 && d->up_w == 2 && wino4_config(d) == 2))
        return 0;
    if (g.mf == 3) return wino4_epm(d, g) == 1 ? 1 : 0;
    return (g.mf == 2 && ((d->res != nullptr) != (d->dact_z != nullptr)) && (!d->dact_z || d->act_d == SDA_ACT_SILU)) ? 1 : 0;
}

int sda_wino4_launch(const sda_conv_desc* d, const Wino4Geom& g_in, hipStream_t stream) {
    const int cus = sda_cu_count();
    if (!cus) return SDA_E_BADARG;
    int grid = cus - cus % 8;
    const int need = (g_in.grid + 7) / 8 * 8;
    if (grid > need) grid = need;
    if (grid < 8) grid = 8;
    static const bool walk_on = !(getenv("SDA_W4_WALK") && atoi(getenv("SDA_W4_WALK")) == 0);
    Wino4Geom g = g_in;
    g.walk = walk_on ? 1 : 0;
    {
        int step = walk_on ? grid / 8 : 1;
        g.sc = step % g.n_ct; step /= g.n_ct;
        g.sx = step % g.bx_n; step /= g.bx_n;
        g.sy = step % g.by_n;
        g.sn = step / g.by_n;
    }
    const int epm = wino4_epm(d, g);
#define W4_LAUNCH3(MOD, LN, SILU)                                                                                              \
    (epm == 1 ? wino4_launch_t<MOD, LN, SILU, 1, 0>(d, g, grid, stream)                                                        \
              : epm == 2 ? wino4_launch_t<MOD, LN, SILU, 2, 0>(d, g, grid, stream)                                             \
                         : wino4_launch_t<MOD, LN, SILU, 0, 0>(d, g, grid, stream))
    const int zp = wino4_zp(d, g);
#ifdef SDA_W4_VARIANTS
    if (zp && getenv("SDA_W4_VAR") && atoi(getenv("SDA_W4_VAR")) == 11) {
        static long long* tbuf = nullptr;
        if (!tbuf && hipMalloc(&tbuf, 256 * 64 * sizeof(long long)) != hipSuccess) return SDA_E_BADARG;
        (void)hipMemsetAsync(tbuf, 0, 256 * 64 * sizeof(long long), stream);
        Wino4Geom gt = g; gt.trace = tbuf; w4_trace_buf = tbuf; w4_trace_grid = grid;
        return zp == 2 ? wino4_launch_t<false, false, false, 0, 11, 2>(d, gt, grid, stream)
                       : wino4_launch_t<false, true, false, 1, 11, 1>(d, gt, grid, stream);
    }
#endif
    if (zp == 2) return wino4_launch_t<false, false, false, 0, 0, 2>(d, g, grid, stream);
    if (zp == 1) return g.mf == 2 ? wino4_launch_mf<false, true, false, 2, 0, 1, 2>(d, g, grid, stream)
                                  : wino4_launch_t<false, true, false, 1, 0, 1>(d, g, grid, stream);
    switch (wino4_config(d)) {
        case 0: {
#ifdef SDA_W4_VARIANTS
            const char* ev = getenv("SDA_W4_VAR");
            switch (ev ? atoi(ev) : 0) {
                case 11: {
                    static long long* tbuf = nullptr;
                    if (!tbuf && hipMalloc(&tbuf, 256 * 64 * sizeof(long long)) != hipSuccess) return SDA_E_BADARG;
                    (void)hipMemsetAsync(tbuf, 0, 256 * 64 * sizeof(long long), stream);
                    Wino4Geom gt = g; gt.trace = tbuf; w4_trace_buf = tbuf; w4_trace_grid = grid;
                    return epm == 1 ? wino4_launch_t<false, false, false, 1, 11>(d, gt, grid, stream)
                         : epm == 2 ? wino4_launch_t<false, false, false, 2, 11>(d, gt, grid, stream)
                                    : wino4_launch_t<false, false, false, 0, 11>(d, gt, grid, stream);
                }
                case 12: if (epm == 0) return wino4_launch_t<false, false, false, 0, 12>(d, g, grid, stream); break;
                case 13: if (epm == 0) return wino4_launch_t<false, false, false, 0, 13>(d, g, grid, stream); break;
                case 14: if (epm == 0) return wino4_launch_t<false, false, false, 0, 14>(d, g, grid, stream); break;
                case 15: if (epm == 0) return wino4_launch_t<false, false, false, 0, 15>(d, g, grid, stream); break;
                default: break;
            }
#endif
            return W4_LAUNCH3(false, false, false);
        }
        case 1: return W4_LAUNCH3(false, false, true);
        case 2: return W4_LAUNCH3(false, true, false);
        case 6: return epm == 0 ? wino4_launch_t<true, true, false, 0, 0>(d, g, grid, stream)
                                : wino4_launch_t<true, true, false, 2, 0>(d, g, grid, stream);
        default: return SDA_E_UNSUPPORTED;
    }
#undef W4_LAUNCH3
}

static bool wino4_disabled() {
    static const bool off = (getenv("SDA_CONV_WINO") && atoi(getenv("SDA_CONV_WINO")) == 0) ||
                            (getenv("SDA_CONV_WINO4") && atoi(getenv("SDA_CONV_WINO4")) == 0);
    return off;
}

int sda_wino4_path(const sda_conv_desc* d) {
    Wino4Geom g;
    if (wino4_disabled() || sda_wino4_plan(d, &g) != SDA_OK) return 0;
    return wino4_zp(d, g) ? 2 : 1;
}

int sda_wino4_try(const sda_conv_desc* d, hipStream_t stream) {
    if (wino4_disabled()) return SDA_E_UNSUPPORTED;
    Wino4Geom g;
    const int rc = sda_wino4_plan(d, &g);
    if (rc != SDA_OK) return rc;
    return sda_wino4_launch(d, g, stream);
}

__global__ void pack_wino4_kernel(const float* __restrict__ w, int cout, int cin, int transpose, int cin_keep,
                                  float* __restrict__ dst, int k_pad, int m_pad) {
    const float G[4][3] = {{1.f, 0.f, 0.f}, {0.5f, 0.5f, 0.5f}, {0.5f, -0.5f, 0.5f}, {0.f, 0.f, 1.f}};
    const int64_t total = (int64_t)k_pad * m_pad;
    const int mtiles = m_pad / 16;
    for (int64_t i = (int64_t)blockIdx.x * blockDim.x + threadIdx.x; i < total; i += (int64_t)gridDim.x * blockDim.x) {
        const int mm = (int)(i % m_pad), kk = (int)(i / m_pad);
        float gk[3][3];
        bool live;
        int co, ci;
        if (!transpose) { ci = kk; co = mm; live = ci < cin && co < cout; }
        else { co = kk; ci = mm; live = ci < cin_keep && ci < cin && co < cout; }
#pragma unroll
        for (int dy = 0; dy < 3; ++dy)
#pragma unroll
            for (int dx = 0; dx < 3; ++dx) {
                const int sy = transpose ? 2 - dy : dy, sx = transpose ? 2 - dx : dx;
                gk[dy][dx] = live ? w[(((int64_t)co * cin + ci) * 3 + sy) * 3 + sx] : 0.f;
            }
        float tmp[4][3];
#pragma unroll
        for (int xi = 0; xi < 4; ++xi)
#pragma unroll
            for (int dx = 0; dx < 3; ++dx) tmp[xi][dx] = G[xi][0] * gk[0][dx] + G[xi][1] * gk[1][dx] + G[xi][2] * gk[2][dx];
        const int st = kk >> 3, kq_ = (kk >> 1) & 3, k4 = kk & 1, mt = mm >> 4, ii = mm & 15;
#pragma unroll
        for (int xi = 0; xi < 4; ++xi)
#pragma unroll
            for (int nu = 0; nu < 4; ++nu) {
                const float uu = tmp[xi][0] * G[nu][0] + tmp[xi][1] * G[nu][1] + tmp[xi][2] * G[nu][2];
                const int pp = 2 * xi + (nu >> 1), h = nu & 1;
                dst[((((int64_t)st * 8 + pp) * mtiles + mt) * 64 + (kq_ * 16 + ii)) * 4 + 2 * h + k4] = uu;
            }
    }
}

extern "C" int sda_pack_conv_weight_wino4(const float* w, int cout, int cin, int transpose, int cin_keep, float* dst,
                                          int k_pad, int m_pad, void* stream) {
    if (!w || !dst || cout <= 0 || cin <= 0 || k_pad <= 0 || m_pad <= 0 || (k_pad & 7) || (m_pad % 32)) return SDA_E_BADARG;
    int64_t total = (int64_t)k_pad * m_pad;
    int blocks = (int)((total + 255) / 256);
    if (blocks > 4096) blocks = 4096;
    hipLaunchKernelGGL(pack_wino4_kernel, dim3(blocks), dim3(256), 0, (hipStream_t)stream, w, cout, cin, transpose, cin_keep,
                       dst, k_pad, m_pad);
    return sda_launch_status();
}

__global__ void pack_wino4_zp_kernel(const float* __restrict__ src, float* __restrict__ dst, int nstage, int n_ct, int mf) {
    const int upp = W4_UPP_OF(mf), uzp = W4_UZP_OF(mf);
    const int64_t total = (int64_t)nstage * n_ct * uzp;
    const int mtiles = 2 * mf * n_ct;
    for (int64_t i = (int64_t)blockIdx.x * blockDim.x + threadIdx.x; i < total; i += (int64_t)gridDim.x * blockDim.x) {
        const int j = (int)(i % uzp);
        const int64_t blk = i / uzp;
        const int ct = (int)(blk % n_ct), st = (int)(blk / n_ct);
        auto at = [&](int pair, int m, int lane, int e) {
            return src[((((int64_t)st * 8 + pair) * mtiles + 2 * mf * ct + m) * 64 + lane) * 4 + e];
        };
        float v = 0.f;
        if (j < 3 * upp) {
            const int fi = j / upp, r = j % upp;
            v = at(fi == 0 ? 0 : (fi == 1 ? 2 : 6), r / 256, (r % 256) / 4, r & 3);
        } else if (j < 4 * upp) {
            const int r = j - 3 * upp, e = r & 3;
            v = e < 2 ? at(1, r / 256, (r % 256) / 4, 2 + e) : at(3, r / 256, (r % 256) / 4, e);
        } else if (j < 4 * upp + upp / 2) {
            const int r = j - 4 * upp;
            v = at(7, r / 128, (r % 128) / 2, 2 + (r & 1));
        }
        dst[i] = v;
    }
}

static int wino4_mf_of(int m_pad) { return m_pad % 96 == 0 ? 3 : (m_pad % 64 == 0 ? 2 : (m_pad % 32 == 0 ? 1 : 0)); }

extern "C" int64_t sda_wino4_zp_floats(int k_pad, int m_pad) {
    const int mf = wino4_mf_of(m_pad);
    if (k_pad <= 0 || m_pad <= 0 || (k_pad & 7) || !mf) return SDA_E_BADARG;
    return (int64_t)(k_pad / 8) * (m_pad / W4_BM_OF(mf)) * W4_UZP_OF(mf);
}

extern "C" int sda_pack_conv_weight_wino4_zp(const float* w_wino4, int k_pad, int m_pad, float* dst, void* stream) {
    const int mf = wino4_mf_of(m_pad);
    if (!w_wino4 || !dst || k_pad <= 0 || m_pad <= 0 || (k_pad & 7) || !mf) return SDA_E_BADARG;
    const int64_t total = sda_wino4_zp_floats(k_pad, m_pad);
    int blocks = (int)((total + 255) / 256);
    if (blocks > 4096) blocks = 4096;
    hipLaunchKernelGGL(pack_wino4_zp_kernel, dim3(blocks), dim3(256), 0, (hipStream_t)stream, w_wino4, dst, k_pad / 8, m_pad / W4_BM_OF(mf), mf);
    return sda_launch_status();
}
```

sda_amd/engine.py:

```python
import math
from dataclasses import dataclass
from typing import List, Optional

import torch
import torch.nn as nn
from torch import Tensor

from . import ops
from ._lib import SdaHipError
from .ops import PackedConv, conv_out_size, make_conv_desc


def _lib_net1d_maxb() -> int:
    from ._lib import NET1D_MAXB
    return NET1D_MAXB


def _net1d_span_ok(sc: int, sx: int, channels: int, length: int) -> bool:
    return sc >= 0 and sx >= 0 and sc * channels + sx * length < 1 << 30


CHUNK_HBM_FRACTION = 0.45
KEEP_HBM_FRACTION = 0.45
PARITY_SPLIT = True
_warned_training = False


@dataclass
class Source:
    x: Tensor
    n: int
    cx: int
    hs: int
    ws: int
    sn_outer: int
    sc: int
    sy: int
    sx: int
    sn_inner: int = 0
    n_inner: int = 1
    ctx: Optional[Tensor] = None
    cctx: int = 0
    ctx_sn: int = 0


def _source0(src: Source, lo: int, n: int):
    sdesc = dict(x_ptr=src.x.data_ptr(), n=n, cx=src.cx, hs=src.hs, ws=src.ws, x_sn_outer=src.sn_outer,
                 x_sn_inner=src.sn_inner, n_inner=src.n_inner, x_n_off=lo, x_sc=src.sc, x_sy=src.sy, x_sx=src.sx)
    ctx = src.ctx
    if ctx is not None and src.ctx_sn:
        ctx = ctx[lo * src.ctx_sn:]
    return sdesc, ctx


def planar_source(a: Tensor) -> dict:
    n, c, h, w = a.shape
    return dict(x_ptr=a.data_ptr(), n=n, cx=c, hs=h, ws=w, x_sn_outer=c * h * w, x_sc=h * w, x_sy=w, x_sx=1)


class _ConvCache:

    def __init__(self, conv: nn.Module):
        if conv.dilation != (1,) * len(conv.dilation) or conv.groups != 1:
            raise NotImplementedError('dilated / grouped convolutions have no gfx950 kernel')
        if conv.padding_mode not in ('zeros', 'circular'):
            raise NotImplementedError(f"padding_mode={conv.padding_mode!r} (supported: 'zeros', 'circular')")
        ks = conv.kernel_size
        if any(k % 2 == 0 for k in ks):
            raise NotImplementedError('even kernel sizes are not supported')
        self.conv = conv
        self.kh, self.kw = (1, ks[0]) if len(ks) == 1 else ks
        st = conv.stride
        self.sh, self.sw = (1, st[0]) if len(st) == 1 else st
        self.circular = conv.padding_mode == 'circular'
        self.cin, self.cout = conv.in_channels, conv.out_channels
        self._key = None
        self._fwd = None
        self._bwd = {}
        self._parity = None

    def _sync(self):
        w = self.conv.weight
        key = (w.data_ptr(), ops.tensor_version(w), str(w.device), None if self.conv.bias is None else ops.tensor_version(self.conv.bias),
               ops.MULTIPLY)
        if key != self._key:
            self._key, self._fwd, self._bwd, self._parity = key, None, {}, None

    def invalidate(self):
        self._key = None

    def fwd(self) -> PackedConv:
        self._sync()
        if self._fwd is None:
            self._fwd = PackedConv(self.conv.weight, self.conv.bias, transpose=False)
        return self._fwd

    def bwd(self, cin_keep: Optional[int] = None) -> PackedConv:
        self._sync()
        if cin_keep not in self._bwd:
            self._bwd[cin_keep] = PackedConv(self.conv.weight, None, transpose=True, cin_keep=cin_keep)
        return self._bwd[cin_keep]

    def bwd_parity(self):
        self._sync()
        if self._parity is None:
            taps = []
            for k, s in ((self.kh, self.sh), (self.kw, self.sw)):
                if s == 1:
                    taps.append([(None, list(range(k)), k // 2)])
                elif s == 2 and k == 3:
                    taps.append([(0, [1], 0), (1, [0, 2], 0)])
                else:
                    taps = None
                    break
            if taps is None or (self.sh == 1 and self.sw == 1):
                self._parity = False
            else:
                w = self.conv.weight.detach()
                if w.dim() == 3:
                    w = w.unsqueeze(2)
                out = []
                for py, ty, ph in taps[0]:
                    for px, tx, pw in taps[1]:
                        sy, sx = (slice(v[0], v[-1] + 1, v[1] - v[0] if len(v) > 1 else 1) for v in (ty, tx))
                        sub = w[:, :, sy, sx].contiguous()
                        out.append((py, px, PackedConv(sub, None, transpose=True), (ph, pw)))
                self._parity = out
        return self._parity or None

    def bwd_parity4(self):
        classes = self.bwd_parity()
        if not classes or len(classes) != 4 or [(py, px) for py, px, _, _ in classes] != [(0, 0), (0, 1), (1, 0), (1, 1)]:
            return None
        if getattr(self, '_parity4', None) is None or self._parity4[0] is not classes:
            pks = [pk for _, _, pk, _ in classes]
            if any(pk.k_pad != pks[0].k_pad or pk.m_pad != pks[0].m_pad or pk.m_pad != pk.m_real for pk in pks):
                return None
            self._parity4 = (classes, torch.cat([pk.packed for pk in pks]))
        return self._parity4[1]


def launch_conv(pk: PackedConv, src: dict, out: Tensor, ho: int, wo: int, *, circular: bool, stride=(1, 1), up=(1, 1),
                zins=(1, 1), bias: Optional[Tensor] = None, mod: Optional[Tensor] = None, mod_sn: int = 0,
                ln=None, act_in: int = 0, dact_z: Optional[Tensor] = None, act_d: int = 0, res: Optional[Tensor] = None,
                ctx: Optional[Tensor] = None, cctx: int = 0, ctx_sn: int = 0, pad=None, parity4_w: Optional[Tensor] = None,
                pool=(1, 1), x_amax=None, out_amax: Optional[Tensor] = None, h2_only: bool = False):
    out_strides = (0, 0, 0, 0)
    if not out.is_contiguous():
        out_strides = tuple(out.stride())
        for t in (dact_z, res):
            if t is not None and tuple(t.stride()) != out_strides:
                raise SdaHipError('conv epilogue operands must share the layout of the output view')
    zp = pk.wino4_zp() if (tuple(up) == (2, 2) or tuple(pool) == (2, 2)) and hasattr(pk, 'wino4_zp') else None
    d = make_conv_desc(**src, w_ptr=pk.packed.data_ptr(), cin_pad=pk.k_pad, cout_pad=pk.m_pad, cout=pk.m_real,
                       kh=pk.kh, kw=pk.kw, out_ptr=out.data_ptr(), ho=ho, wo=wo, mt=pk.mt,
                       stride_h=stride[0], stride_w=stride[1], circular=circular, up_h=up[0], up_w=up[1],
                       zins_h=zins[0], zins_w=zins[1],
                       ctx_ptr=None if ctx is None else ctx.data_ptr(), cctx=cctx, ctx_sn=ctx_sn,
                       mod_ptr=None if mod is None else mod.data_ptr(), mod_sn=mod_sn,
                       ln_mean_ptr=None if ln is None else ln[0].data_ptr(),
                       ln_rstd_ptr=None if ln is None else ln[1].data_ptr(),
                       act_in=act_in, bias_ptr=None if bias is None else bias.data_ptr(),
                       dact_z_ptr=None if dact_z is None else dact_z.data_ptr(), act_d=act_d,
                       res_ptr=None if res is None else res.data_ptr(),
                       w_wino4_ptr=None if getattr(pk, 'wino4', None) is None else pk.wino4.data_ptr(),
                       pad=pad, out_strides=out_strides, pool=pool, w_wino4_zp_ptr=None if zp is None else zp.data_ptr())
    if pool != (1, 1):
        if tuple(pool) == (2, 2) and ops.H2_POOL and x_amax is not None and getattr(pk, 'h2', None) is not None:
            packing = pk.h2_pool()
            if packing is not None and ops.conv_h2(d, pk, x_amax, out_amax, packing=packing):
                return d
        return d if ops.conv_pooled(d) else None
    if getattr(pk, 'h2', None) is not None and parity4_w is None:
        bound = math.sqrt(src['cx']) if ln is not None else x_amax
        packing = None
        if tuple(up) == (2, 2):
            packing = pk.h2_up() if ops.H2_UP else None
            if packing is None:
                bound = None
        elif tuple(zins) == (2, 2) or tuple(stride) == (2, 2):
            packing = (pk.h2_zins() if tuple(zins) == (2, 2) else pk.h2_s2()) if ops.H2_S2 else None
            if packing is None:
                bound = None
        if ops.conv_h2(d, pk, bound, out_amax, packing=packing):
            return d
    if h2_only:
        return None
    if parity4_w is not None:
        d.w = parity4_w.data_ptr()
        d.kh = d.kw = 2
        return d if ops.conv_parity4(d) else None
    ops.conv_igemm(d)
    return d


class _Block:
    def __init__(self, block, width: int, mod_off: int):
        from .nn import LayerNorm, activation_id
        residue = block.residue
        if not (len(residue) == 4 and isinstance(residue[0], LayerNorm)):
            raise NotImplementedError('unexpected residue structure')
        self.ln = residue[0]
        self.conv1 = _ConvCache(residue[1])
        self.act = activation_id(residue[2])
        self.conv2 = _ConvCache(residue[3])
        self.project = block.project[0]
        self.width = width
        self.mod_off = mod_off


class _Level:
    pass


class UNetEngine:
    def __init__(self, unet):
        from .nn import LN_UNBIASED
        if unet.spatial not in (1, 2):
            raise NotImplementedError('this engine serves spatial = 1, 2 (spatial = 3: engine3d.UNet3dEngine)')
        self.unet = unet
        self.unbiased = LN_UNBIASED
        self.depth = len(unet.hidden_blocks)
        D = self.depth
        self.levels: List[_Level] = []
        off = 0
        for lvl in range(D):
            lev = _Level()
            lev.C = unet.hidden_channels[lvl]
            j = D - 1 - lvl
            head = unet.heads[lvl] if lvl == 0 else unet.heads[lvl][0]
            lev.head = _ConvCache(head)
            if lvl == 0:
                lev.tail = _ConvCache(unet.tails[j])
                lev.tail_ln = None
            else:
                lev.tail_ln = unet.tails[j][0]
                lev.tail = _ConvCache(unet.tails[j][2])
            lev.descent, lev.ascent = [], []
            for blk in unet.descent[lvl]:
                lev.descent.append(_Block(blk, lev.C, off)); off += lev.C
            for blk in unet.ascent[j]:
                lev.ascent.append(_Block(blk, lev.C, off)); off += lev.C
            self.levels.append(lev)
        self.mod_total = off
        self._proj_key = None
        self._proj = None
        st = unet.stride
        self.sh, self.sw = (1, st[0]) if len(st) == 1 else st

    def convs(self) -> List[_ConvCache]:
        out = []
        for lev in self.levels:
            out += [lev.head, lev.tail]
            for blk in lev.descent + lev.ascent:
                out += [blk.conv1, blk.conv2]
        return out

    def train_params(self) -> List[Tensor]:
        ps = []
        for cc in self.convs():
            ps.append(cc.conv.weight)
            if cc.conv.bias is not None:
                ps.append(cc.conv.bias)
        return ps

    def param_grads(self, pg: Optional['ParamGrads'], params: List[Tensor]) -> list:
        if pg is None:
            return [None] * len(params)
        by_id = {}
        for cc in self.convs():
            hit = pg.conv_grads.get(id(cc))
            if hit is None:
                continue
            if hit[0] is not None:
                by_id[id(cc.conv.weight)] = hit[0].view(cc.conv.weight.shape)
            if cc.conv.bias is not None and hit[1] is not None:
                by_id[id(cc.conv.bias)] = hit[1]
        return [by_id.get(id(p)) if p.requires_grad else None for p in params]

    def invalidate(self):
        for lev in self.levels:
            lev.head.invalidate()
            lev.tail.invalidate()
            for blk in lev.descent + lev.ascent:
                blk.conv1.invalidate()
                blk.conv2.invalidate()
        self._proj_key = None
        self.__dict__.pop('_net1d_cache', None)

    def _blocks(self):
        for lev in self.levels:
            yield from lev.descent
            yield from lev.ascent

    def projection(self):
        key = tuple((b.project.weight.data_ptr(), ops.tensor_version(b.project.weight), ops.tensor_version(b.project.bias)) for b in self._blocks())
        if key != self._proj_key:
            blocks = sorted(self._blocks(), key=lambda b: b.mod_off)
            w = torch.cat([b.project.weight.detach() for b in blocks], dim=0).contiguous()
            bias = torch.cat([b.project.bias.detach() for b in blocks], dim=0).contiguous()
            self._proj_key, self._proj = key, (w, bias)
        return self._proj

    def modulation(self, emb: Tensor) -> Tensor:
        w, b = self.projection()
        return ops.linear_small(emb.contiguous(), w, b)

    def modulation_train(self, emb: Tensor) -> Tensor:
        blocks = sorted(self._blocks(), key=lambda b: b.mod_off)
        w = torch.cat([b.project.weight for b in blocks], dim=0)
        bias = torch.cat([b.project.bias for b in blocks], dim=0)
        return torch.nn.functional.linear(emb, w, bias).contiguous()

    def bytes_per_image(self, hs: int, ws: int, save: bool) -> int:
        total, h, w = 0, hs, ws
        for lvl, lev in enumerate(self.levels):
            if lvl > 0:
                h = conv_out_size(h, lev.head.kh, lev.head.sh)
                w = conv_out_size(w, lev.head.kw, lev.head.sw)
# ... 98 lines not shown
        lev, blocks = plan['lev'], plan['blocks']
        convs = [lev.head] + [c for b in blocks for c in (b.conv1, b.conv2)] + [lev.tail]
        for cc in convs:
            cc._sync()
        key = (backward, cin_keep, tuple(cc._key for cc in convs))
        cache = self.__dict__.setdefault('_net1d_cache', {})
        hit = cache.get(backward)
        if hit is not None and hit[0] == key:
            return hit[1], hit[2]
        dev = lev.head.conv.weight.device
        if backward:
            order = [(lev.tail, None)] + [(c, None) for b in reversed(blocks) for c in (b.conv2, b.conv1)] + [(lev.head, cin_keep)]
        else:
            order = [(cc, None) for cc in convs]
        w = torch.empty(len(order), 3 * 64 * 64, device=dev, dtype=torch.float32)
        from . import training
        if training.net1d_enabled():
            bias = None if backward else torch.empty(len(order), 64, device=dev, dtype=torch.float32)
            self._net1d_pack(plan, convs, backward, cin_keep, w, bias)
            cache[backward] = (key, w, bias)
            return w, bias
        bias = None if backward else torch.zeros(len(order), 64, device=dev, dtype=torch.float32)
        for i, (cc, keep) in enumerate(order):
            wt = cc.conv.weight.detach().contiguous()
            cout, cin = wt.shape[0], wt.shape[1]
            ops.pack_conv_weight(wt, cout, cin, 1, 3, backward, (cin if keep is None else keep) if backward else cin, w[i], 64, 64)
            if bias is not None and cc.conv.bias is not None:
                bias[i, :cout] = cc.conv.bias.detach()
        cache[backward] = (key, w, bias)
        return w, bias

    def _net1d_desc(self, plan, n: int, length: int, mod_all, lo: int, per_image: bool, backward: bool, cin_keep: int = 0):
        from ._lib import Net1dDesc
        lev, blocks = plan['lev'], plan['blocks']
        d = Net1dDesc()
        d.n, d.len, d.c, d.nblocks = n, length, lev.C, len(blocks)
        d.circular, d.unbiased = int(lev.head.circular), int(self.unbiased)
        d.act = blocks[0].act if blocks else 0
        d.eps = blocks[0].ln.eps if blocks else 1e-5
        w, bias = self._net1d_weights(plan, backward, cin_keep)
        d.w, d.bias = w.data_ptr(), None if bias is None else bias.data_ptr()
        if not backward:
            d.cin, d.cout = lev.head.cin, lev.tail.cout
        else:
            d.cin, d.cout = lev.tail.cout, cin_keep
        keep = [w, bias]
        for k, blk in enumerate(blocks):
            mod, mod_sn = self._mod_for(blk, mod_all, lo, per_image)
            d.mod[k] = None if mod is None else mod.data_ptr()
            d.mod_sn = mod_sn
            keep.append(mod)
        return d, keep

    def _net1d_forward(self, plan, src: Source, lo: int, hi: int, mod_all, per_image: bool, out: Tensor, save: bool,
                       train: bool = False):
        n, length = hi - lo, src.ws
        d, keep = self._net1d_desc(plan, n, length, mod_all, lo, per_image, False)
        d.x = src.x.data_ptr() + 4 * lo * src.sn_outer
        d.x_sn, d.x_sc, d.x_sx = src.sn_outer, src.sc, src.sx
        d.out = out.data_ptr()
        d.out_sn, d.out_sc, d.out_sx = out.stride(0), out.stride(1), out.stride(3)
        saved = None
        if save:
            nb, C, dev = len(plan['blocks']), plan['lev'].C, out.device
            a_s = torch.empty(max(nb, 1), n, C, length, device=dev, dtype=torch.float32)
            z_s = torch.empty_like(a_s)
            m_s = torch.empty(max(nb, 1), n, length, device=dev, dtype=torch.float32)
            r_s = torch.empty_like(m_s)
            d.a_save, d.z_save, d.save_stride = a_s.data_ptr(), z_s.data_ptr(), n * C * length
            d.mean_save, d.rstd_save, d.stat_stride = m_s.data_ptr(), r_s.data_ptr(), n * length
            saved = dict(net1d=(plan, a_s, z_s, m_s, r_s), dims=[(1, length)])
        if train:
            from ._lib import Net1dTrainDesc
            t = Net1dTrainDesc()
            t.net = d
            saved['net1d_train'] = tail_in = torch.empty(n, plan['lev'].C, length, device=out.device, dtype=torch.float32)
            t.tail_in = tail_in.data_ptr()
            ops.net1d_fwd_train(t)
            return saved
        ops.net1d_launch(d, False)
        return saved

    def _net1d_backward(self, saved, g_out: Tensor, src: Source, lo: int, mod_all, per_image: bool, g_in: Tensor):
        plan, a_s, z_s, m_s, r_s = saved['net1d']
        n, length = g_out.shape[0], src.ws
        if not _net1d_span_ok(g_out.stride(1), g_out.stride(3), g_out.shape[1], length):
            g_out = g_out.contiguous()
        d, keep = self._net1d_desc(plan, n, length, mod_all, lo, per_image, True, cin_keep=src.cx)
        d.x = g_out.data_ptr()
        d.x_sn, d.x_sc, d.x_sx = g_out.stride(0), g_out.stride(1), g_out.stride(3)
        d.out = g_in.data_ptr()
        d.out_sn, d.out_sc, d.out_sx = g_in.stride(0), g_in.stride(1), g_in.stride(3)
        C = plan['lev'].C
        d.a_save, d.z_save, d.save_stride = a_s.data_ptr(), z_s.data_ptr(), n * C * length
        d.mean_save, d.rstd_save, d.stat_stride = m_s.data_ptr(), r_s.data_ptr(), n * length
        ops.net1d_launch(d, True)

    def _net1d_backward_train(self, saved, g_out: Tensor, src: Source, lo: int, mod_all, per_image: bool, g_in: Optional[Tensor],
                              pg: 'ParamGrads'):
        from ._lib import Net1dTrainDesc, Net1dWgradDesc
        plan, a_s, z_s, m_s, r_s = saved['net1d']
        lev, blocks = plan['lev'], plan['blocks']
        n, length, C, nb, dev = g_out.shape[0], src.ws, lev.C, len(blocks), g_out.device
        if not _net1d_span_ok(g_out.stride(1), g_out.stride(3), g_out.shape[1], length):
            g_out = g_out.contiguous()
        if g_in is None:
            g_in = torch.empty(n, src.cx, 1, length, device=dev, dtype=torch.float32)
        d, keep = self._net1d_desc(plan, n, length, mod_all, lo, per_image, True, cin_keep=src.cx)
        d.x = g_out.data_ptr()
        d.x_sn, d.x_sc, d.x_sx = g_out.stride(0), g_out.stride(1), g_out.stride(3)
        d.out = g_in.data_ptr()
        d.out_sn, d.out_sc, d.out_sx = g_in.stride(0), g_in.stride(1), g_in.stride(3)
        d.a_save, d.z_save, d.save_stride = a_s.data_ptr(), z_s.data_ptr(), n * C * length
        d.mean_save, d.rstd_save, d.stat_stride = m_s.data_ptr(), r_s.data_ptr(), n * length
        tiles = ops.net1d_tiles(d)
        g_s = torch.empty(2 * nb + 1, n, C, length, device=dev, dtype=torch.float32)
        mod_part = torch.empty(max(nb, 1), n, tiles, C, device=dev, dtype=torch.float32)
        t = Net1dTrainDesc()
        t.net = d
        t.g_save, t.g_stride = g_s.data_ptr(), n * C * length
        t.mod_part, t.mod_tiles = mod_part.data_ptr(), tiles
        ops.net1d_bwd_train(t)
        fd, fkeep = self._net1d_desc(plan, n, length, mod_all, lo, per_image, False)
        fd.x = src.x.data_ptr() + 4 * lo * src.sn_outer
        fd.x_sn, fd.x_sc, fd.x_sx = src.sn_outer, src.sc, src.sx
        fd.a_save, fd.z_save, fd.save_stride = d.a_save, d.z_save, d.save_stride
        fd.mean_save, fd.rstd_save, fd.stat_stride = d.mean_save, d.rstd_save, d.stat_stride
        wd = Net1dWgradDesc()
        wd.net = fd
        wd.tail_in = saved['net1d_train'].data_ptr()
        wd.g_save, wd.g_stride = t.g_save, t.g_stride
        wd.gout, wd.gout_sn, wd.gout_sc, wd.gout_sx = g_out.data_ptr(), g_out.stride(0), g_out.stride(1), g_out.stride(3)
        wd.mod_part, wd.mod_tiles = t.mod_part, tiles
        convs = [lev.head] + [c for b in blocks for c in (b.conv1, b.conv2)] + [lev.tail]
        for v, cc in enumerate(convs):
            w, b = cc.conv.weight, cc.conv.bias
            dw = torch.empty(w.shape, device=dev, dtype=torch.float32) if w.requires_grad else None
            db = torch.empty(b.shape, device=dev, dtype=torch.float32) if (b is not None and b.requires_grad) else None
            wd.dw[v], wd.db[v] = None if dw is None else dw.data_ptr(), None if db is None else db.data_ptr()
            pg.conv_grads[id(cc)] = (dw, db)
        if pg.gmod is not None:
            rows = pg.gmod[lo:] if per_image else pg.gmod
            for k, blk in enumerate(blocks):
                wd.dmod[k] = rows[:, blk.mod_off:].data_ptr()
            wd.dmod_sn = self.mod_total
        ops.net1d_wgrad(wd, dev)

    def _mod_for(self, blk: _Block, mod_all: Optional[Tensor], lo: int, per_image: bool):
        if mod_all is None:
            return None, 0
        row = mod_all[lo:] if per_image else mod_all
        return row[:, blk.mod_off:], (self.mod_total if per_image else 0)

    def _block_fwd(self, blk: _Block, a: Tensor, mod_all, lo, per_image, saved):
        n, c, h, w = a.shape
        dev = a.device
        mod, mod_sn = self._mod_for(blk, mod_all, lo, per_image)
        c1, c2 = blk.conv1, blk.conv2
        if (c1.circular == c2.circular and (c1.sh, c1.sw, c2.sh, c2.sw) == (1, 1, 1, 1) and
                ops.block1d_eligible(c, h, c1.fwd(), c2.fwd())):
            y = torch.empty_like(a)
            if saved is not None:
                mean = torch.empty(n * h * w, device=dev, dtype=torch.float32)
                rstd = torch.empty_like(mean)
                z = torch.empty_like(a)
                ops.block1d_fwd(a, mod, mod_sn, c1.fwd(), c2.fwd(), c1.circular, blk.act, blk.ln.eps, self.unbiased, y, z, mean, rstd)
                saved.append((a, mean, rstd, z))
            else:
                ops.block1d_fwd(a, mod, mod_sn, c1.fwd(), c2.fwd(), c1.circular, blk.act, blk.ln.eps, self.unbiased, y)
            return y
        mean = torch.empty(n * h * w, device=dev, dtype=torch.float32)
        rstd = torch.empty_like(mean)
        ops.ln_stats(a, mod, mod_sn, blk.ln.eps, self.unbiased, mean, rstd)
        z = torch.empty_like(a)
        pk = c1.fwd()
        z_amax = getattr(pk, 'out_amax', None)
        d1 = launch_conv(pk, planar_source(a), z, h, w, circular=c1.circular, bias=pk.bias, mod=mod, mod_sn=mod_sn,
                         ln=(mean, rstd), out_amax=z_amax)
        if not (d1 is not None and d1.w_h2):
            z_amax = None
        y = torch.empty_like(a)
        c2 = blk.conv2
        pk = c2.fwd()
        launch_conv(pk, planar_source(z), y, h, w, circular=c2.circular, bias=pk.bias, act_in=blk.act, res=a, x_amax=z_amax)
        if saved is not None:
            saved.append((a, mean, rstd, z))
        return y

    def forward_chunk(self, src: Source, lo: int, hi: int, mod_all: Optional[Tensor], per_image: bool, out: Tensor,
                      save: bool, train: bool = False):
        plan = None if train else self.net1d_plan(src)
        if plan is not None:
            return self._net1d_forward(plan, src, lo, hi, mod_all, per_image, out, save)
        n = hi - lo
        dev = out.device
        L, D = self.levels, self.depth
        saved = dict(blocks={}, tails={}, dims=[], head_in={}, tail0_in=None) if save else None
        skips, dims = [], []
        a, h, w = None, src.hs, src.ws
        for lvl, lev in enumerate(L):
            hd = lev.head
            pk = hd.fwd()
            if lvl == 0:
                ho, wo = conv_out_size(h, hd.kh, hd.sh), conv_out_size(w, hd.kw, hd.sw)
                a = torch.empty(n, lev.C, ho, wo, device=dev, dtype=torch.float32)
                sdesc, ctx = _source0(src, lo, n)
                launch_conv(pk, sdesc, a, ho, wo, circular=hd.circular, stride=(hd.sh, hd.sw), bias=pk.bias, ctx=ctx,
                            cctx=src.cctx, ctx_sn=src.ctx_sn)
            else:
                ho, wo = conv_out_size(h, hd.kh, hd.sh), conv_out_size(w, hd.kw, hd.sw)
                a2 = torch.empty(n, lev.C, ho, wo, device=dev, dtype=torch.float32)
                if save and train:
                    saved['head_in'][lvl] = a
                xa = None
                if ops.MULTIPLY == 'f16x2' and ops.H2_S2 and (hd.sh, hd.sw) == (2, 2) and getattr(pk, 'h2', None) is not None and a.is_contiguous():
                    xa = ops.absmax(a, pk.in_amax)
                launch_conv(pk, planar_source(a), a2, ho, wo, circular=hd.circular, stride=(hd.sh, hd.sw), bias=pk.bias, x_amax=xa)
                a = a2
            h, w = ho, wo
            dims.append((h, w))
            for bi, blk in enumerate(lev.descent):
                rec = [] if save else None
                a = self._block_fwd(blk, a, mod_all, lo, per_image, rec)
                if save:
                    saved['blocks'][('d', lvl, bi)] = rec[0]
            skips.append(a)
        skips.pop()
        for lvl in reversed(range(D)):
            lev = L[lvl]
            for bi, blk in enumerate(lev.ascent):
                rec = [] if save else None
                a = self._block_fwd(blk, a, mod_all, lo, per_image, rec)
                if save:
                    saved['blocks'][('a', lvl, bi)] = rec[0]
            tl = lev.tail
            pk = tl.fwd()
            if lvl > 0:
                hu, wu = dims[lvl - 1]
                uh, uw = L[lvl].head.sh, L[lvl].head.sw
                if (h * uh, w * uw) != (hu, wu):
                    raise SdaHipError(f'U-Net level {lvl}: upsampled size {(h * uh, w * uw)} != skip size {(hu, wu)} '
                                      f'(spatial sizes must be divisible by the strides, as in the reference)')
                mean = torch.empty(n * h * w, device=dev, dtype=torch.float32)
                rstd = torch.empty_like(mean)
                ops.ln_stats(a, None, 0, lev.tail_ln.eps, self.unbiased, mean, rstd)
                t = torch.empty(n, L[lvl - 1].C, hu, wu, device=dev, dtype=torch.float32)
                launch_conv(pk, planar_source(a), t, hu, wu, circular=tl.circular, up=(uh, uw), bias=pk.bias,
                            ln=(mean, rstd), res=skips.pop())
                if save:
                    saved['tails'][lvl] = (a, mean, rstd)
                a, h, w = t, hu, wu
            else:
                if save and train:
                    saved['tail0_in'] = a
                launch_conv(pk, planar_source(a), out, h, w, circular=tl.circular, bias=pk.bias)
        if save:
            saved['dims'] = dims
        return saved

    def _block_bwd(self, blk: _Block, g: Tensor, rec, mod_all, lo, per_image, g_amax_in=None, pg: Optional['ParamGrads'] = None):
        a, mean, rstd, z = rec
        n, c, h, w = a.shape
        mod, mod_sn = self._mod_for(blk, mod_all, lo, per_image)
        c1, c2 = blk.conv1, blk.conv2
        if (pg is None and c1.circular == c2.circular and (c1.sh, c1.sw, c2.sh, c2.sw) == (1, 1, 1, 1) and
                ops.block1d_eligible(c, h, c1.fwd(), c2.fwd())):
            gx = torch.empty_like(a)
            ops.block1d_bwd(g, a, z, mean, rstd, mod, mod_sn, c1.bwd(), c2.bwd(), c1.circular, blk.act, self.unbiased, gx)
            return gx, None
        gz = torch.empty_like(a)
        pk2 = c2.bwd()
        g_amax = gz_amax = None
        if getattr(pk2, 'h2', None) is not None and g.is_contiguous():
            g_amax, gz_amax = (g_amax_in if g_amax_in is not None else ops.absmax(g, pk2.in_amax)), pk2.out_amax
        d2 = launch_conv(pk2, planar_source(g), gz, h, w, circular=c2.circular, dact_z=z, act_d=blk.act, x_amax=g_amax, out_amax=gz_amax)
        if not (d2 is not None and d2.w_h2):
            gz_amax = None
        if pg is not None:
            self._wgrad(pg, c2, planar_source(z), g, h, w, act_in=blk.act)
            self._wgrad(pg, c1, planar_source(a), gz, h, w, mod=mod, mod_sn=mod_sn, ln=(mean, rstd))
        gh = torch.empty_like(a)
        c1 = blk.conv1
        launch_conv(c1.bwd(), planar_source(gz), gh, h, w, circular=c1.circular, x_amax=gz_amax)
        gx = torch.empty_like(a)
        gx_amax = None
        if getattr(pk2, 'h2', None) is not None:
            gx_amax = getattr(blk, '_gx_amax', None)
            if gx_amax is None or gx_amax.device != a.device:
                gx_amax = blk._gx_amax = torch.zeros(1, device=a.device, dtype=torch.float32)
        ops.ln_bwd(gh, a, h, w, mod, mod_sn, mean, rstd, self.unbiased, (1, 1), g, gx, out_amax=gx_amax)
        if pg is not None and mod is not None:
            pg.modulation(blk, gx, g, lo, self.mod_total)
        return gx, gx_amax

    def _wgrad(self, pg: 'ParamGrads', cc: _ConvCache, sdesc: dict, g: Tensor, ho: int, wo: int, *, mod=None, mod_sn=0, ln=None,
               act_in=0, up=(1, 1), ctx=None, cctx=0, ctx_sn=0):
        d = make_conv_desc(**sdesc, w_ptr=0, cin_pad=0, cout_pad=0, cout=cc.cout, kh=cc.kh, kw=cc.kw, out_ptr=0, ho=ho, wo=wo,
                           mt=1, stride_h=cc.sh, stride_w=cc.sw, circular=cc.circular, up_h=up[0], up_w=up[1],
                           ctx_ptr=None if ctx is None else ctx.data_ptr(), cctx=cctx, ctx_sn=ctx_sn,
                           mod_ptr=None if mod is None else mod.data_ptr(), mod_sn=mod_sn,
                           ln_mean_ptr=None if ln is None else ln[0].data_ptr(), ln_rstd_ptr=None if ln is None else ln[1].data_ptr(),
                           act_in=act_in)
        pg.conv(cc, d, g)

    def backward_chunk(self, saved, g_out: Tensor, src: Source, lo: int, mod_all, per_image: bool, g_in: Optional[Tensor],
                       pg: Optional['ParamGrads'] = None):
        if 'net1d' in saved:
            if pg is not None:
                if 'net1d_train' not in saved:
                    raise SdaHipError('this whole-net 1-D forward kept nothing for parameter gradients (it ran outside the net1d training route)')
                return self._net1d_backward_train(saved, g_out, src, lo, mod_all, per_image, g_in, pg)
            return self._net1d_backward(saved, g_out, src, lo, mod_all, per_image, g_in)
        g_out = g_out.contiguous()
        L, D = self.levels, self.depth
        dims = saved['dims']
        n = g_out.shape[0]
        dev = g_out.device
        h, w = dims[0]
        tl = L[0].tail
        g = torch.empty(n, L[0].C, h, w, device=dev, dtype=torch.float32)
        if pg is not None:
            self._wgrad(pg, tl, planar_source(saved['tail0_in']), g_out, h, w)
        launch_conv(tl.bwd(), planar_source(g_out), g, h, w, circular=tl.circular)
        g_amax = None
        g_skip = {}
        for lvl in range(D):
            lev = L[lvl]
            if lvl > 0:
                g_skip[lvl - 1] = g
                hu, wu = dims[lvl - 1]
                h, w = dims[lvl]
                uh, uw = lev.head.sh, lev.head.sw
                if (uh, uw) not in ((2, 2), (1, 2)):
                    raise NotImplementedError('VJP through Upsample is implemented for scale factor 2')
                tl = lev.tail
                a, mean, rstd = saved['tails'][lvl]
                if pg is not None:
                    self._wgrad(pg, tl, planar_source(a), g, hu, wu, ln=(mean, rstd), up=(uh, uw))
                pooled = None
                if ops.POOLED and (uh, uw) == (2, 2) and hu == 2 * h and wu == 2 * w:
                    pooled = torch.empty(n, lev.C, h, w, device=dev, dtype=torch.float32)
                    xa = None
                    if ops.MULTIPLY == 'f16x2' and getattr(tl.bwd(), 'h2', None) is not None and g.is_contiguous():
                        xa = g_amax if g_amax is not None else ops.absmax(g, tl.bwd().in_amax)
                    if launch_conv(tl.bwd(), planar_source(g), pooled, hu, wu, circular=tl.circular, pool=(2, 2), x_amax=xa) is None:
                        pooled = None
                if pooled is None:
                    ghup = torch.empty(n, lev.C, hu, wu, device=dev, dtype=torch.float32)
                    launch_conv(tl.bwd(), planar_source(g), ghup, hu, wu, circular=tl.circular)
                g = torch.empty(n, lev.C, h, w, device=dev, dtype=torch.float32)
                g_amax = None
                if ops.MULTIPLY == 'f16x2':
                    g_amax = getattr(lev, '_g_amax', None)
                    if g_amax is None or g_amax.device != dev:
                        g_amax = lev._g_amax = torch.zeros(1, device=dev, dtype=torch.float32)
                if pooled is not None:
                    ops.ln_bwd(pooled, a, h, w, None, 0, mean, rstd, self.unbiased, (1, 1), None, g, out_amax=g_amax)
                else:
                    ops.ln_bwd(ghup, a, h, w, None, 0, mean, rstd, self.unbiased, (uh, uw), None, g, out_amax=g_amax)
            for bi in reversed(range(len(lev.ascent))):
                g, g_amax = self._block_bwd(lev.ascent[bi], g, saved['blocks'][('a', lvl, bi)], mod_all, lo, per_image, g_amax, pg)
        for lvl in reversed(range(D)):
            lev = L[lvl]
            for bi in reversed(range(len(lev.descent))):
                g, g_amax = self._block_bwd(lev.descent[bi], g, saved['blocks'][('d', lvl, bi)], mod_all, lo, per_image, g_amax, pg)
            hd = lev.head
            if pg is not None:
                if lvl > 0:
                    self._wgrad(pg, hd, planar_source(saved['head_in'][lvl]), g, *dims[lvl])
                else:
                    sdesc, ctx = _source0(src, lo, n)
                    self._wgrad(pg, hd, sdesc, g, *dims[lvl], ctx=ctx, cctx=src.cctx, ctx_sn=src.ctx_sn)
            if lvl > 0:
                hu, wu = dims[lvl - 1]
                if hd.circular and ((hd.sh > 1 and hu % hd.sh) or (hd.sw > 1 and wu % hd.sw)):
                    raise NotImplementedError('VJP of a strided circular conv needs sizes divisible by the stride')
                g2 = torch.empty(n, L[lvl - 1].C, hu, wu, device=dev, dtype=torch.float32)
                skip = g_skip.pop(lvl - 1)
                classes = hd.bwd_parity() if PARITY_SPLIT and hu % hd.sh == 0 and wu % hd.sw == 0 else None
                done = False
                if (ops.MULTIPLY == 'f16x2' and ops.H2_S2 and (hd.sh, hd.sw) == (2, 2) and g.is_contiguous() and skip.is_contiguous() and
                        skip.shape == g2.shape and g.shape[2] % 16 == 0 and g.shape[3] % 16 == 0 and hd.bwd().h2_zins() is not None):
                    xa = g_amax if g_amax is not None else ops.absmax(g, hd.bwd().in_amax)
                    done = launch_conv(hd.bwd(), planar_source(g), g2, hu, wu, circular=hd.circular, zins=(hd.sh, hd.sw), res=skip,
                                       x_amax=xa, h2_only=True) is not None
                if not done and classes is not None and ops.PARITY4:
                    w4 = hd.bwd_parity4()
                    if w4 is not None and skip.is_contiguous() and skip.shape == g2.shape:
                        pk0, pad0 = classes[0][2], classes[0][3]
                        view = g2[:, :, 0::2, 0::2]
                        done = launch_conv(pk0, planar_source(g), view, view.shape[2], view.shape[3], circular=hd.circular, pad=pad0,
                                           res=skip[:, :, 0::2, 0::2], parity4_w=w4) is not None
                if done:
                    pass
                elif classes is not None:
                    gsrc = planar_source(g)
                    for py, px, pk, pad in classes:
                        ys = slice(None) if py is None else slice(py, None, 2)
                        xs = slice(None) if px is None else slice(px, None, 2)
                        view = g2[:, :, ys, xs]
                        launch_conv(pk, gsrc, view, view.shape[2], view.shape[3], circular=hd.circular, pad=pad,
                                    res=skip[:, :, ys, xs])
                else:
                    launch_conv(hd.bwd(), planar_source(g), g2, hu, wu, circular=hd.circular, zins=(hd.sh, hd.sw),
                                res=skip)
                g = g2
                g_amax = None
            elif g_in is not None:
                launch_conv(hd.bwd(cin_keep=src.cx), planar_source(g), g_in, src.hs, src.ws, circular=hd.circular,
                            zins=(hd.sh, hd.sw))



class ParamGrads:

    def __init__(self, mod_all: Optional[Tensor], per_image: bool, need_mod: bool):
        self.conv_grads = {}
        self.per_image = per_image
        self.gmod = torch.empty_like(mod_all) if (need_mod and mod_all is not None) else None
        self._mod_written = set()
        from . import training
        self.route = training.wgrad_route()

    def conv(self, cc: _ConvCache, desc, g: Tensor):
        hit = self.conv_grads.get(id(cc))
        accumulate = hit is not None
        if hit is None:
            w, b = cc.conv.weight, cc.conv.bias
# ... 169 lines not shown
```

sda_amd/ops.py:

```python
import ctypes
import math
import os
from typing import Optional

import torch
from torch import Tensor

from . import _lib
from ._lib import ACT_IDS, ConvDesc

CONV_CK = 8
WINOGRAD = os.environ.get('SDA_CONV_WINO', '1') != '0'
WINOGRAD4 = os.environ.get('SDA_CONV_WINO4', '1') != '0'
MULTIPLY = os.environ.get('SDA_MULTIPLY', 'f32')
if MULTIPLY not in ('f32', 'f16x2'):
    raise ValueError(f"SDA_MULTIPLY={MULTIPLY!r} (expected 'f32' or 'f16x2')")


def set_multiply(mode: str) -> str:
    global MULTIPLY
    if mode not in ('f32', 'f16x2'):
        raise ValueError(f"multiply mode {mode!r} (expected 'f32' or 'f16x2')")
    prev, MULTIPLY = MULTIPLY, mode
    return prev


H2_UP = os.environ.get('SDA_H2_UP', '1') != '0'
H2_POOL = os.environ.get('SDA_H2_POOL', '1') != '0'
H2_S2 = os.environ.get('SDA_H2_S2', '1') != '0'


def tensor_version(t) -> int:
    return 0 if t is None or t.is_inference() else t._version


def _dev(*tensors):
    for t in tensors:
        if t is None:
            continue
        if not t.is_cuda:
            raise _lib.SdaHipError('sda_amd ops run on MI355X only: got a CPU tensor (there is no CPU fallback)')
        if t.dtype != torch.float32:
            raise _lib.SdaHipError(f'sda_amd ops are fp32: got {t.dtype}')


def _ptr(t: Optional[Tensor]):
    return None if t is None else t.data_ptr()


def _stream():
    return torch.cuda.current_stream().cuda_stream


def round_up(v: int, m: int) -> int:
    return (v + m - 1) // m * m


def pick_mt(cout: int) -> int:
    best, best_pad = 1, None
    for mt in (3, 4, 2, 1):
        pad = round_up(cout, 32 * mt)
        if best_pad is None or pad < best_pad:
            best, best_pad = mt, pad
    return best


def conv_out_size(size_v: int, k: int, stride: int) -> int:
    return (size_v + 2 * (k // 2) - k) // stride + 1


def make_conv_desc(*, x_ptr, n, cx, hs, ws, x_sc, x_sy, x_sx, x_sn_outer, x_sn_inner=0, n_inner=1, x_n_off=0,
                   w_ptr, cin_pad, cout_pad, cout, kh, kw, out_ptr, ho, wo, mt,
                   stride_h=1, stride_w=1, circular=False, up_h=1, up_w=1, zins_h=1, zins_w=1,
                   ctx_ptr=None, cctx=0, ctx_sn=0, mod_ptr=None, mod_sn=0, ln_mean_ptr=None, ln_rstd_ptr=None,
                   act_in=0, bias_ptr=None, dact_z_ptr=None, act_d=0, res_ptr=None,
                   w_wino4_ptr=None, pad=None, out_strides=(0, 0, 0, 0), pool=(1, 1), w_wino4_zp_ptr=None) -> ConvDesc:
    d = ConvDesc()
    d.x = x_ptr
    d.x_sn_outer, d.x_sn_inner, d.n_inner, d.x_n_off = x_sn_outer, x_sn_inner, n_inner, x_n_off
    d.x_sc, d.x_sy, d.x_sx = x_sc, x_sy, x_sx
    d.cx = cx
    d.ctx, d.ctx_sn, d.cctx = ctx_ptr, ctx_sn, cctx
    d.n, d.hs, d.ws = n, hs, ws
    d.up_h, d.up_w, d.zins_h, d.zins_w = up_h, up_w, zins_h, zins_w
    d.mod, d.mod_sn = mod_ptr, mod_sn
    d.ln_mean, d.ln_rstd = ln_mean_ptr, ln_rstd_ptr
    d.act_in = act_in
    d.kh, d.kw, d.stride_h, d.stride_w, d.circular = kh, kw, stride_h, stride_w, int(bool(circular))
    d.w, d.cin_pad, d.cout_pad = w_ptr, cin_pad, cout_pad
    d.bias = bias_ptr
    d.out, d.cout, d.ho, d.wo = out_ptr, cout, ho, wo
    d.dact_z, d.act_d = dact_z_ptr, act_d
    d.res = res_ptr
    d.mt = mt
    d.w_wino4 = w_wino4_ptr
    d.explicit_pad = 0 if pad is None else 1
    d.pad_h, d.pad_w = (0, 0) if pad is None else pad
    d.out_sn, d.out_sc, d.out_sy, d.out_sx = out_strides
    d.pool_h, d.pool_w = pool
    d.w_wino4_zp = w_wino4_zp_ptr
    return d


class ConvProfile:

    def __init__(self):
        self.records = []
        self.family_bytes = {}
        self.mem_records = []

    def flops(self, d: ConvDesc) -> float:
        pixels = d.ho * d.wo / (d.zins_h * d.zins_w)
        return 2.0 * d.n * pixels * d.cout * (d.cx + d.cctx) * d.kh * d.kw

    def alg_bytes(self, d: ConvDesc):
        cin = d.cx + d.cctx
        rd = 4.0 * d.n * d.cx * d.hs * d.ws + 4.0 * d.cctx * d.hs * d.ws * (d.n if d.ctx_sn else 1)
        rd += 4.0 * cin * d.cout * (16 if d.w_wino4 and conv_path(d) in (2, 5) else d.kh * d.kw)
        if d.ln_mean:
            rd += 8.0 * d.n * d.hs * d.ws
        out = 4.0 * d.n * d.cout * d.ho * d.wo / (max(1, d.pool_h) * max(1, d.pool_w))
        rd += out * ((1 if d.res else 0) + (1 if d.dact_z else 0))
        return rd, out

    def bracket_mem(self, kernel: str, nbytes: float, launch):
        e0, e1 = torch.cuda.Event(enable_timing=True), torch.cuda.Event(enable_timing=True)
        e0.record()
        launch()
        e1.record()
        self.mem_records.append((e0, e1, nbytes, kernel))

    def mem_summary(self):
        torch.cuda.synchronize()
        out = {}
        for a, b, nb, k in self.mem_records:
            r = out.setdefault(k, dict(launches=0, ms=0.0, bytes=0.0))
            r['launches'] += 1
            r['ms'] += a.elapsed_time(b)
            r['bytes'] += nb
        return out

    def summary(self):
        torch.cuda.synchronize()
        out = dict(launches=len(self.records), total_ms=0.0, total_flops=0.0, families={})
        for a, b, f, fam in self.records:
            ms = a.elapsed_time(b)
            out['total_ms'] += ms
            out['total_flops'] += f
            r = out['families'].setdefault(fam, dict(launches=0, ms=0.0, flops=0.0))
            r['launches'] += 1
            r['ms'] += ms
            r['flops'] += f
        return out


conv_profile: Optional[ConvProfile] = None


def conv_igemm(desc: ConvDesc):
    lib = _lib.load()
    prof = conv_profile
    if prof is not None:
        e0, e1 = torch.cuda.Event(enable_timing=True), torch.cuda.Event(enable_timing=True)
        e0.record()
        _lib.check(lib.sda_conv_igemm(ctypes.byref(desc), _stream()), 'sda_conv_igemm')
        e1.record()
        fam = CONV_FAMILIES[max(0, conv_path(desc))]
        prof.records.append((e0, e1, prof.flops(desc) / float(max(1, desc.zins_h) * max(1, desc.zins_w)), fam))
        rd, wr = prof.alg_bytes(desc)
        b = prof.family_bytes.setdefault(fam, [0.0, 0.0])
        b[0] += rd
        b[1] += wr
        return
    _lib.check(lib.sda_conv_igemm(ctypes.byref(desc), _stream()), 'sda_conv_igemm')


def absmax(x: Tensor, out: Tensor) -> Tensor:
    _dev(x, out)
    if not x.is_contiguous():
        raise _lib.SdaHipError('absmax reads a contiguous tensor')
    _lib.check(_lib.load().sda_absmax(x.data_ptr(), x.numel(), out.data_ptr(), _stream()), 'sda_absmax')
    return out


def conv_h2(desc: ConvDesc, pk: 'PackedConv', x_amax, out_amax: Optional[Tensor], packing=None) -> bool:
    if getattr(pk, 'h2', None) is None or x_amax is None:
        return False
    lib = _lib.load()
    if packing is None:
        desc.w_h2, desc.w_h2_scale = pk.h2.data_ptr(), pk.h2_scale
    else:
        desc.w_h2, desc.w_h2_scale = packing[0].data_ptr(), packing[1]
    if torch.is_tensor(x_amax):
        desc.x_amax, desc.x_amax_static = x_amax.data_ptr(), 0.0
    else:
        desc.x_amax, desc.x_amax_static = None, float(x_amax)
    desc.out_amax = None if out_amax is None else out_amax.data_ptr()
    if not lib.sda_conv_h2_supported(ctypes.byref(desc)):
        desc.w_h2 = None
        return False
    prof = conv_profile
    if prof is not None:
        e0, e1 = torch.cuda.Event(enable_timing=True), torch.cuda.Event(enable_timing=True)
        e0.record()
    if out_amax is not None:
        out_amax.zero_()
    _lib.check(lib.sda_conv_h2(ctypes.byref(desc), _stream()), 'sda_conv_h2')
    if prof is not None:
        e1.record()
        fam = 'h2up' if (desc.up_h == 2 or desc.pool_h == 2) else 'h2s2' if (desc.zins_h == 2 or desc.stride_h == 2) else 'h2'
        prof.records.append((e0, e1, prof.flops(desc) / float(max(1, desc.zins_h) * max(1, desc.zins_w)), fam))
        rd, wr = prof.alg_bytes(desc)
        b = prof.family_bytes.setdefault(fam, [0.0, 0.0])
        b[0] += rd
        b[1] += wr
    return True


PARITY4 = os.environ.get('SDA_CONV_PAR4', '1') != '0'
WINO4_BM64 = os.environ.get('SDA_W4_BM64', '1') != '0'


def conv_parity4(desc: ConvDesc) -> bool:
    lib = _lib.load()
    prof = conv_profile
    if prof is not None:
        e0, e1 = torch.cuda.Event(enable_timing=True), torch.cuda.Event(enable_timing=True)
        e0.record()
    rc = lib.sda_conv_parity4(ctypes.byref(desc), _stream())
    if rc == -2:
        return False
    _lib.check(rc, 'sda_conv_parity4')
    if prof is not None:
        e1.record()
        prof.records.append((e0, e1, 2.0 * desc.n * desc.ho * desc.wo * desc.cout * desc.cx * 9, 'par4'))
        b = prof.family_bytes.setdefault('par4', [0.0, 0.0])
        b[0] += 4.0 * desc.n * desc.cx * desc.hs * desc.ws + 4.0 * 9 * desc.cx * desc.cout + (16.0 * desc.n * desc.cout * desc.ho * desc.wo if desc.res else 0.0)
        b[1] += 16.0 * desc.n * desc.cout * desc.ho * desc.wo
    return True


POOLED = os.environ.get('SDA_CONV_POOLED', '1') != '0'


def conv_pooled(desc: ConvDesc) -> bool:
    lib = _lib.load()
    if lib.sda_conv_igemm_path(ctypes.byref(desc)) < 0:
        return False
    conv_igemm(desc)
    return True


CONV_FAMILIES = ('direct', 'wino', 'wino4', 'small1d', 'few', 'wino4zp')


def conv_path(desc: ConvDesc) -> int:
    return _lib.load().sda_conv_igemm_path(ctypes.byref(desc))


def pack_conv_weight(w: Tensor, cout: int, cin: int, kh: int, kw: int, transpose: bool, keep: int, dst: Tensor,
                     k_pad: int, m_pad: int):
    _lib.check(_lib.load().sda_pack_conv_weight(w.data_ptr(), cout, cin, kh, kw, int(transpose), keep, dst.data_ptr(),
                                                k_pad, m_pad, _stream()), 'sda_pack_conv_weight')




def wgrad_desc(conv: ConvDesc, g: Tensor, dw: Tensor, db: Optional[Tensor], accumulate: bool, slabs: int = 0):
    d = _lib.WgradDesc()
    d.conv = conv
    d.g, d.dw, d.db = g.data_ptr(), dw.data_ptr(), _ptr(db)
    d.work = 1
    d.slabs, d.accumulate = slabs, int(bool(accumulate))
    return d


def wgrad_flops(conv: ConvDesc) -> float:
    return 2.0 * conv.n * conv.ho * conv.wo * conv.cout * (conv.cx + conv.cctx) * conv.kh * conv.kw


WGRAD_ROUTES = ('general', 'tiled', 'tiled_ht')


def conv_wgrad(conv: ConvDesc, g: Tensor, dw: Tensor, db: Optional[Tensor], accumulate: bool, slabs: int = 0, route: str = 'general'):
    if route not in WGRAD_ROUTES:
        raise ValueError(f"conv_wgrad route {route!r} (expected 'general', 'tiled' or 'tiled_ht')")
    _dev(g, dw, db)
    if not g.is_contiguous() or tuple(g.shape) != (conv.n, conv.cout, conv.ho, conv.wo):
        raise _lib.SdaHipError(f'conv_wgrad: cotangent must be planar contiguous {(conv.n, conv.cout, conv.ho, conv.wo)}, got {tuple(g.shape)}')
    cin = conv.cx + conv.cctx
    if not dw.is_contiguous() or dw.numel() != conv.cout * cin * conv.kh * conv.kw or (db is not None and db.numel() != conv.cout):
        raise _lib.SdaHipError('conv_wgrad: dw / db do not match the layer')
    lib = _lib.load()
    d = wgrad_desc(conv, g, dw, db, accumulate, slabs)
    if route != 'general' and lib.sda_conv_wgrad3_serves(ctypes.byref(d)):
        planner, launch, name, family = lib.sda_conv_wgrad3_work_floats, lib.sda_conv_wgrad3, 'sda_conv_wgrad3', 'wgrad3'
    elif route == 'tiled_ht' and lib.sda_conv_wgrad3x_serves(ctypes.byref(d)):
        planner, launch, name, family = lib.sda_conv_wgrad3x_work_floats, lib.sda_conv_wgrad3x, 'sda_conv_wgrad3x', 'wgrad3x'
    else:
        planner, launch, name, family = lib.sda_conv_wgrad_work_floats, lib.sda_conv_wgrad, 'sda_conv_wgrad', 'wgrad'
    floats = planner(ctypes.byref(d))
    _lib.check(int(min(floats, 0)), name + '_work_floats')
    work = torch.empty(int(floats), device=g.device, dtype=torch.float32)
    d.work = work.data_ptr()
    prof = conv_profile
    if prof is not None:
        e0, e1 = torch.cuda.Event(enable_timing=True), torch.cuda.Event(enable_timing=True)
        e0.record()
        _lib.check(launch(ctypes.byref(d), _stream()), name)
        e1.record()
        prof.records.append((e0, e1, wgrad_flops(conv), family))
        return
    _lib.check(launch(ctypes.byref(d), _stream()), name)


def plane_sum(x: Tensor, y: Optional[Tensor], out: Tensor, out_sn: int, sum_images: bool, accumulate: bool):
    _dev(x, y, out)
    if not x.is_contiguous() or (y is not None and (not y.is_contiguous() or y.shape != x.shape)):
        raise _lib.SdaHipError('plane_sum: operands must be planar contiguous and alike')
    n, c = x.shape[0], x.shape[1]
    hw = x[0, 0].numel()

    def launch():
        _lib.check(_lib.load().sda_plane_sum(x.data_ptr(), _ptr(y), n, c, hw, out.data_ptr(), out_sn, int(bool(sum_images)),
                                             int(bool(accumulate)), _stream()), 'sda_plane_sum')
    if conv_profile is not None:
        conv_profile.bracket_mem('plane_sum', 4.0 * n * c * hw * (2 if y is not None else 1), launch)
    else:
        launch()

class PackedConv:

    def __init__(self, weight: Tensor, bias: Optional[Tensor], transpose: bool = False, cin_keep: Optional[int] = None):
        _dev(weight, bias)
        w = weight.detach().contiguous()
        cout, cin = w.shape[0], w.shape[1]
        ks = tuple(w.shape[2:])
        self.kh, self.kw = (1, ks[0]) if len(ks) == 1 else ks
        self._transpose = bool(transpose)
        self._w_ref = w if (MULTIPLY == 'f16x2' and len(ks) == 2) else None
        self._h2_up = None
        self._h2_pool = None
        self._h2_zins = None
        self._h2_s2 = None
        if transpose:
            keep = cin if cin_keep is None else cin_keep
            self.k_real, self.m_real = cout, keep
        else:
            keep = cin
            self.k_real, self.m_real = cin, cout
        self.mt = pick_mt(self.m_real)
        self.k_pad = round_up(self.k_real, CONV_CK)
        self.m_pad = round_up(self.m_real, 32 * self.mt)
        self.packed = torch.empty(self.kh * self.kw * self.k_pad * self.m_pad, device=w.device, dtype=torch.float32)
        pack_conv_weight(w, cout, cin, self.kh, self.kw, transpose, keep, self.packed, self.k_pad, self.m_pad)
        self.bias = None if (bias is None or transpose) else bias.detach().contiguous()
        self.wino4 = None
        if (WINOGRAD and WINOGRAD4 and (self.kh, self.kw) == (3, 3) and self.m_pad == self.m_real and
                (self.m_real % 96 == 0 or (WINO4_BM64 and self.m_real % 32 == 0))):
            self.wino4 = torch.empty(16 * self.k_pad * self.m_pad, device=w.device, dtype=torch.float32)
            _lib.check(_lib.load().sda_pack_conv_weight_wino4(w.data_ptr(), cout, cin, int(transpose), keep,
                                                              self.wino4.data_ptr(), self.k_pad, self.m_pad, _stream()),
                       'sda_pack_conv_weight_wino4')
        self._wino4_zp = None
        if self.wino4 is not None:
            lib = _lib.load()
            self._wino4_zp = torch.empty(int(lib.sda_wino4_zp_floats(self.k_pad, self.m_pad)), device=w.device, dtype=torch.float32)
            _lib.check(lib.sda_pack_conv_weight_wino4_zp(self.wino4.data_ptr(), self.k_pad, self.m_pad, self._wino4_zp.data_ptr(), _stream()),
                       'sda_pack_conv_weight_wino4_zp')

        self.h2 = None
        if MULTIPLY == 'f16x2' and (self.kh, self.kw) == (3, 3) and (not transpose or keep == cin) and w.numel() > 0:
# ... 793 lines not shown
```

Before: 0.1370 diffusion-steps/s.

## Fuse SiLU and its derivative into the Winograd conv epilogue for 384-channel blocks

Adds an activated-output epilogue to the Winograd F(4,3) conv kernel. The first conv of a residual block now writes silu(z) directly, and optionally silu'(z) for the backward pass. The second conv reads the activated tensor without re-applying SiLU on input. In the guided backward, the transposed conv multiplies by the stored derivative instead of recomputing dsilu from z. This removes per-element activation recomputation in the conv prologue and backward epilogue, at the cost of an extra derivative tensor write. It is gated to SiLU, 384 channels, modulated, non-H2 blocks, and the new kernels are built in a separate translation unit.

```diff
diff --git a/include/sda_hip.h b/include/sda_hip.h
--- a/include/sda_hip.h
+++ b/include/sda_hip.h
@@ -59,6 +59,9 @@
     float x_amax_static;
     const float* x_amax;
     float* out_amax;
+    int32_t act_out;
+    int32_t dact_mul;
+    float* out_dact;
 } sda_conv_desc;
 
 int sda_conv_igemm(const sda_conv_desc* d, void* stream);
diff --git a/sda_amd/_lib.py b/sda_amd/_lib.py
--- a/sda_amd/_lib.py
+++ b/sda_amd/_lib.py
@@ -49,6 +49,7 @@
         ('w_wino4_zp', c_fp),
         ('w_h2', ctypes.c_void_p), ('w_h2_scale', ctypes.c_float), ('x_amax_static', ctypes.c_float),
         ('x_amax', c_fp), ('out_amax', c_fp),
+        ('act_out', c_int32), ('dact_mul', c_int32), ('out_dact', c_fp),
     ]
 
 
diff --git a/sda_amd/build.py b/sda_amd/build.py
--- a/sda_amd/build.py
+++ b/sda_amd/build.py
@@ -7,7 +7,7 @@
 CSRC = os.path.join(HERE, 'csrc')
 LIBDIR = os.environ.get('SDA_LIBDIR') or os.path.join(HERE, 'lib')
 ARCH = 'gfx950'
-SOURCES = ['conv_igemm.hip', 'conv_wino4.hip', 'conv_small1d.hip', 'conv_few.hip', 'conv_par4.hip', 'conv_h2.hip', 'conv3d.hip', 'conv_wgrad.hip', 'conv_wgrad3.hip', 'block1d.hip', 'net1d.hip', 'net1d_train.hip', 'step1d.hip', 'norm.hip', 'elementwise.hip', 'linear.hip', 'mlp1d.hip', 'mlp_train.hip', 'optim.hip', 'train_loss.hip', 'observe.hip', 'metrics.hip', 'noise.hip', 'chain.hip', 'probe.hip']
+SOURCES = ['conv_igemm.hip', 'conv_wino4.hip', 'conv_wino4_act.hip', 'conv_small1d.hip', 'conv_few.hip', 'conv_par4.hip', 'conv_h2.hip', 'conv3d.hip', 'conv_wgrad.hip', 'conv_wgrad3.hip', 'block1d.hip', 'net1d.hip', 'net1d_train.hip', 'step1d.hip', 'norm.hip', 'elementwise.hip', 'linear.hip', 'mlp1d.hip', 'mlp_train.hip', 'optim.hip', 'train_loss.hip', 'observe.hip', 'metrics.hip', 'noise.hip', 'chain.hip', 'probe.hip']
 HIPCC = os.environ.get('HIPCC', '/opt/rocm/bin/hipcc')
 EXTRA_FLAGS = os.environ.get('SDA_EXTRA_HIPCC_FLAGS', '').split()
 EMU_SOURCES = ['conv_igemm.hip', 'conv_wgrad.hip', 'conv_wgrad3.hip', 'chain.hip', 'mlp_train.hip', 'net1d_train.hip', 'optim.hip']
@@ -61,11 +61,12 @@
         obj = os.path.join(LIBDIR, src.replace('.hip', suffix + '.o'))
         objs.append(obj)
         cflags = ['-O3', '-std=c++17', '-fPIC', '-ffp-contract=off'] + flags + EXTRA_FLAGS
-        if force or _newer(obj, [sp] + hdrs, cflags):
+        deps = [sp] + hdrs + ([os.path.join(CSRC, 'conv_wino4.hip')] if src == 'conv_wino4_act.hip' else [])
+        if force or _newer(obj, deps, cflags):
             cmd = [HIPCC, f'--offload-arch={ARCH}'] + cflags + ['-c', sp, '-o', obj]
             if verbose:
                 print(' '.join(cmd))
-            procs.append((src + suffix, obj, [sp] + hdrs, cflags, subprocess.Popen(cmd, stdout=subprocess.PIPE, stderr=subprocess.STDOUT)))
+            procs.append((src + suffix, obj, deps, cflags, subprocess.Popen(cmd, stdout=subprocess.PIPE, stderr=subprocess.STDOUT)))
     for src, obj, deps, cflags, p in procs:
         out, _ = p.communicate()
         if p.returncode != 0:
diff --git a/sda_amd/csrc/conv_h2.hip b/sda_amd/csrc/conv_h2.hip
--- a/sda_amd/csrc/conv_h2.hip
+++ b/sda_amd/csrc/conv_h2.hip
@@ -522,6 +522,7 @@
 
 static bool h2_ok(const sda_conv_desc* d) {
     if (!d || !d->x || !d->out || !d->w_h2) return false;
+    if (d->act_out != SDA_ACT_NONE || d->out_dact || d->dact_mul) return false;
     const bool up = d->up_h == 2 && d->up_w == 2;
     const bool pool = d->pool_h == 2 && d->pool_w == 2;
     const bool zins = d->zins_h == 2 && d->zins_w == 2;
diff --git a/sda_amd/csrc/conv_igemm.hip b/sda_amd/csrc/conv_igemm.hip
--- a/sda_amd/csrc/conv_igemm.hip
+++ b/sda_amd/csrc/conv_igemm.hip
@@ -732,6 +732,7 @@
 int sda_few_try(const sda_conv_desc* d, hipStream_t stream);
 int sda_wino4_path(const sda_conv_desc* d), sda_small1d_path(const sda_conv_desc* d), sda_few_path(const sda_conv_desc* d);
 typedef const sda_conv_desc* conv_dp;
+static bool conv_epx(conv_dp d) { return d->act_out != SDA_ACT_NONE || d->out_dact || d->dact_mul; }
 struct ConvTier { bool (*offered)(conv_dp d); int (*run)(conv_dp d, hipStream_t stream); int (*path)(conv_dp d); };
 static const ConvTier CONV_TIERS[] = {
     {[](conv_dp d) { return !!d->w_wino4; }, sda_wino4_try, [](conv_dp d) { const int p = sda_wino4_path(d); return p == 2 ? 5 : p ? 2 : 0; }},
@@ -742,6 +743,7 @@
 
 extern "C" int sda_conv_igemm(const sda_conv_desc* d, void* stream) {
     if (!d) return SDA_E_BADARG;
+    if (conv_epx(d)) return d->w_wino4 ? sda_wino4_try(d, (hipStream_t)stream) : SDA_E_UNSUPPORTED;
     for (const ConvTier& t : CONV_TIERS) {
         if (!t.offered(d)) continue;
         if (!t.run) return SDA_E_UNSUPPORTED;
@@ -762,6 +764,7 @@
 
 extern "C" int sda_conv_igemm_path(const sda_conv_desc* d) {
     if (!d) return SDA_E_BADARG;
+    if (conv_epx(d)) return d->w_wino4 && sda_wino4_path(d) == 1 ? 2 : SDA_E_UNSUPPORTED;
     for (const ConvTier& t : CONV_TIERS) {
         if (!t.offered(d)) continue;
         if (!t.path) return SDA_E_UNSUPPORTED;
diff --git a/sda_amd/csrc/conv_par4.hip b/sda_amd/csrc/conv_par4.hip
--- a/sda_amd/csrc/conv_par4.hip
+++ b/sda_amd/csrc/conv_par4.hip
@@ -154,6 +154,7 @@
 static bool par4_ok(const sda_conv_desc* d) {
     static const bool off = getenv("SDA_CONV_PAR4") && atoi(getenv("SDA_CONV_PAR4")) == 0;
     if (off || !d || !d->x || !d->w || !d->out) return false;
+    if (d->act_out != SDA_ACT_NONE || d->out_dact || d->dact_mul) return false;
     if (d->kh != 2 || d->kw != 2 || !d->explicit_pad || d->pad_h != 0 || d->pad_w != 0 || d->stride_h != 1 || d->stride_w != 1 ||
         d->up_h != 1 || d->up_w != 1 || d->zins_h != 1 || d->zins_w != 1)
         return false;
diff --git a/sda_amd/csrc/conv_wino4.hip b/sda_amd/csrc/conv_wino4.hip
--- a/sda_amd/csrc/conv_wino4.hip
+++ b/sda_amd/csrc/conv_wino4.hip
@@ -41,6 +41,9 @@
     }
 }
 
+int sda_wino4_launch_epx(const sda_conv_desc* d, const Wino4Geom& g, int grid, int epm, hipStream_t stream);
+
+#ifndef SDA_W4_ACT_UNIT
 static int wino4_config(const sda_conv_desc* d);
 
 int sda_wino4_plan(const sda_conv_desc* d, Wino4Geom* g) {
@@ -61,6 +64,17 @@
     if (d->act_in != SDA_ACT_NONE && d->act_in != SDA_ACT_SILU) return SDA_E_UNSUPPORTED;
     if ((d->ln_mean == nullptr) != (d->ln_rstd == nullptr)) return SDA_E_UNSUPPORTED;
     if (wino4_config(d) < 0) return SDA_E_UNSUPPORTED;
+    if (d->act_out != SDA_ACT_NONE || d->out_dact || d->dact_mul) {
+        const int key = wino4_config(d);
+        if (d->cout % 96 || d->up_h != 1 || d->up_w != 1 || d->pool_h > 1 || d->pool_w > 1 || d->res) return SDA_E_UNSUPPORTED;
+        if (d->act_out != SDA_ACT_NONE) {
+            if (d->act_out != SDA_ACT_SILU || d->dact_z || d->dact_mul || (key != 0 && key != 6) ||
+                (reinterpret_cast<uintptr_t>(d->out_dact) & 7) || d->out_dact == d->out)
+                return SDA_E_UNSUPPORTED;
+        } else if (d->out_dact || !d->dact_z || key != 0) {
+            return SDA_E_UNSUPPORTED;
+        }
+    }
     if ((reinterpret_cast<uintptr_t>(d->out) & 7) || (d->res && (reinterpret_cast<uintptr_t>(d->res) & 7)) ||
         (d->dact_z && (reinterpret_cast<uintptr_t>(d->dact_z) & 7)) || (reinterpret_cast<uintptr_t>(d->w_wino4) & 15) ||
         (d->bias && (reinterpret_cast<uintptr_t>(d->bias) & 15)))
@@ -93,6 +107,8 @@
     return SDA_OK;
 }
 
+#endif
+
 struct W4Tile { int ct, n, by, bx; };
 __device__ __forceinline__ W4Tile w4_decode(const Wino4Geom& g, int tile) {
     W4Tile t;
@@ -154,12 +170,29 @@
     return sg * w;
 }
 
+template <bool WITH_D>
+__device__ __forceinline__ void w4_silu_dsilu2(f32x2 z, f32x2& s, f32x2& dz) {
+    const f32x2 zc = f32x2{__builtin_fmaxf(z[0], -80.f), __builtin_fmaxf(z[1], -80.f)};
+    const f32x2 t = zc * f32x2{-1.4426950408889634f, -1.4426950408889634f};
+    const f32x2 e = {__builtin_amdgcn_exp2f(t[0]), __builtin_amdgcn_exp2f(t[1])};
+    const f32x2 dn = e + f32x2{1.f, 1.f};
+    const f32x2 sg = {__builtin_amdgcn_rcpf(dn[0]), __builtin_amdgcn_rcpf(dn[1])};
+    s = z * sg;
+    if constexpr (WITH_D) {
+        const f32x2 u = zc * e;
+        const f32x2 w = __builtin_elementwise_fma(u, sg, f32x2{1.f, 1.f});
+        dz = sg * w;
+    }
+}
+
 template <int ZP>
 __host__ __device__ constexpr bool w4_dead(int p) { return ZP != 0 && ((p >> 2) == 2 || (p & 3) == 2); }
 
-template <bool MOD, bool LN, bool SILU, int EPM, int VAR = 0, int ZP = 0, int MF = 3>
+template <bool MOD, bool LN, bool SILU, int EPM, int VAR = 0, int ZP = 0, int MF = 3, int EPX = 0>
 __global__ __launch_bounds__(512, 2) void conv_wino4_kernel(const sda_conv_desc d, const Wino4Geom g) {
     static_assert(MF >= 1 && MF <= 3, "cout tile = 32, 64 or 96");
+    static_assert(EPX == 0 || (MF == 3 && ZP == 0 && VAR == 0), "the activated-output / plain-factor epilogues exist for the full 96-cout kernels only");
+    static_assert(EPX == 0 || (EPX == 3 ? EPM != 0 : EPM == 0), "activated output: launches without an operand; plain factor: launches with one");
     static_assert(MF == 3 || EPM != 1, "the helper-fed epilogue operand exists for the 96-cout tile only");
     static_assert(MF > 1 || ZP != 1, "the 32-cout tile has no up-sampled zero-position form");
     constexpr bool ZPOS = ZP != 0;
@@ -820,11 +853,12 @@
                 const auto r_out = rsrc_of(d.out);
                 const auto r_z = rsrc_of(DACT ? d.dact_z : d.out);
                 const auto r_res = rsrc_of(RES ? d.res : d.out);
+                const auto r_dout = rsrc_of(EPX == 2 ? d.out_dact : d.out);
                 const float* el = ubuf + ((q + 1) & 1) * W4_UBUF + (wave * 8 * MF * 64 + lane_e) * 2;
                 f32x2 el0[MF > 1 ? 4 * (MF - 1) : 1], el1[MF > 1 ? 4 * (MF - 1) : 1];
 #pragma unroll
                 for (int m = 0; m < MF; ++m) {
-                    if constexpr (EPM != 0) __builtin_amdgcn_sched_barrier(0);
+                    if constexpr (EPM != 0 || EPX != 0) __builtin_amdgcn_sched_barrier(0);
                     f32x4 s0[4], s1[4];
 #pragma unroll
                     for (int nu = 0; nu < 4; ++nu) {
@@ -855,7 +889,7 @@
                     }
 #pragma unroll
                     for (int r = 0; r < 4; ++r) {
-                        if constexpr (DACT_KIND == 1) { if (r == 2) __builtin_amdgcn_sched_barrier(0); }
+                        if constexpr (DACT_KIND == 1 || EPX == 1 || EPX == 2) { if (r == 2) __builtin_amdgcn_sched_barrier(0); }
                         const int so = (16 * m + r) * hw_o * 4;
                         f32x2 y0 = {y00[r], y01[r]}, y1 = {y10[r], y11[r]};
                         f32x2 e0, e1;
@@ -874,7 +908,10 @@
                                 q0 = __builtin_bit_cast(f32x2, __builtin_amdgcn_raw_buffer_load_b64(r_z, lo0, so, 0));
                                 q1 = __builtin_bit_cast(f32x2, __builtin_amdgcn_raw_buffer_load_b64(r_z, lo1, so, 0));
                             }
-                            if (DACT_KIND == 1 || d.act_d == SDA_ACT_SILU) {
+                            if constexpr (DACT_KIND == 3) {
+                                y0 *= q0;
+                                y1 *= q1;
+                            } else if (DACT_KIND == 1 || d.act_d == SDA_ACT_SILU) {
                                 y0 *= w4_dsilu2(q0);
                                 y1 *= w4_dsilu2(q1);
                             } else {
@@ -890,6 +927,15 @@
                                 y1 += __builtin_bit_cast(f32x2, __builtin_amdgcn_raw_buffer_load_b64(r_res, lo1, so, 0));
                             }
                         }
+                        if constexpr (EPX == 1 || EPX == 2) {
+                            f32x2 dz0, dz1;
+                            w4_silu_dsilu2<EPX == 2>(y0, y0, dz0);
+                            w4_silu_dsilu2<EPX == 2>(y1, y1, dz1);
+                            if constexpr (EPX == 2) {
+                                __builtin_amdgcn_raw_buffer_store_b64(__builtin_bit_cast(w4_u32x2, dz0), r_dout, lo0, so, 0);
+                                __builtin_amdgcn_raw_buffer_store_b64(__builtin_bit_cast(w4_u32x2, dz1), r_dout, lo1, so, 0);
+                            }
+                        }
                         if (!SDA_DBG(g, 8)) {
                             __builtin_amdgcn_raw_buffer_store_b64(__builtin_bit_cast(w4_u32x2, y0), r_out, lo0, so, 0);
                             __builtin_amdgcn_raw_buffer_store_b64(__builtin_bit_cast(w4_u32x2, y1), r_out, lo1, so, 0);
@@ -900,6 +946,7 @@
             using K0 = std::integral_constant<int, 0>;
             using K1 = std::integral_constant<int, 1>;
             using K2 = std::integral_constant<int, 2>;
+            using K3 = std::integral_constant<int, 3>;
             if constexpr (ZP == 2) {
                 const int wo_p = d.wo >> 1, hw_p = (d.ho >> 1) * wo_p;
                 const int lo_p = ((4 * kq_e) * hw_p + (4 * tt.by + (t >> 3)) * wo_p + 8 * tt.bx + (t & 7)) * 4;
@@ -919,6 +966,8 @@
                 }
             } else if constexpr (EPM == 0) {
                 run(K0{}, std::false_type{});
+            } else if constexpr (EPX == 3) {
+                run(K3{}, std::false_type{});
             } else if constexpr (EPI) {
                 if (d.dact_z) run(K1{}, std::false_type{});
                 else run(K0{}, std::true_type{});
@@ -936,7 +985,7 @@
     W4_TRACE_OUT();
 }
 
-#ifdef SDA_W4_VARIANTS
+#if defined(SDA_W4_VARIANTS) && !defined(SDA_W4_ACT_UNIT)
 static long long* w4_trace_buf = nullptr;
 static int w4_trace_grid = 0;
 extern "C" int sda_w4_trace_read(double* out) {
@@ -952,16 +1001,30 @@
 }
 #endif
 
-template <bool MOD, bool LN, bool SILU, int EPI, int VAR, int ZP, int MF>
+template <bool MOD, bool LN, bool SILU, int EPI, int VAR, int ZP, int MF, int EPX = 0>
 static int wino4_launch_mf(const sda_conv_desc* d, const Wino4Geom& g, int grid, hipStream_t stream) {
     static_assert(W4_LDS_BYTES_OF(MF) <= 160 * 1024, "LDS");
     static bool attr_set[SDA_MAX_DEVICES];
-    const int rc = sda_raise_dyn_lds(reinterpret_cast<const void*>(conv_wino4_kernel<MOD, LN, SILU, EPI, VAR, ZP, MF>), W4_LDS_BYTES_OF(MF), attr_set);
+    const int rc = sda_raise_dyn_lds(reinterpret_cast<const void*>(conv_wino4_kernel<MOD, LN, SILU, EPI, VAR, ZP, MF, EPX>), W4_LDS_BYTES_OF(MF), attr_set);
     if (rc != SDA_OK) return rc;
-    hipLaunchKernelGGL((conv_wino4_kernel<MOD, LN, SILU, EPI, VAR, ZP, MF>), dim3(grid), dim3(512), (size_t)W4_LDS_BYTES_OF(MF), stream, *d, g);
+    hipLaunchKernelGGL((conv_wino4_kernel<MOD, LN, SILU, EPI, VAR, ZP, MF, EPX>), dim3(grid), dim3(512), (size_t)W4_LDS_BYTES_OF(MF), stream, *d, g);
     return sda_launch_status();
 }
 
+#ifdef SDA_W4_ACT_UNIT
+int sda_wino4_launch_epx(const sda_conv_desc* d, const Wino4Geom& g, int grid, int epm, hipStream_t stream) {
+    if (d->act_out != SDA_ACT_NONE) {
+        const bool two = d->out_dact != nullptr;
+        if (d->mod) return two ? wino4_launch_mf<true, true, false, 0, 0, 0, 3, 2>(d, g, grid, stream)
+                               : wino4_launch_mf<true, true, false, 0, 0, 0, 3, 1>(d, g, grid, stream);
+        return two ? wino4_launch_mf<false, false, false, 0, 0, 0, 3, 2>(d, g, grid, stream)
+                   : wino4_launch_mf<false, false, false, 0, 0, 0, 3, 1>(d, g, grid, stream);
+    }
+    if (!d->dact_mul) return SDA_E_UNSUPPORTED;
+    return epm == 1 ? wino4_launch_mf<false, false, false, 1, 0, 0, 3, 3>(d, g, grid, stream)
+                    : wino4_launch_mf<false, false, false, 2, 0, 0, 3, 3>(d, g, grid, stream);
+}
+#else
 template <bool MOD, bool LN, bool SILU, int EPI, int VAR, int ZP = 0>
 static int wino4_launch_t(const sda_conv_desc* d, const Wino4Geom& g, int grid, hipStream_t stream) {
     if constexpr ((VAR == 0 || VAR == 11) && EPI != 1) {
@@ -983,7 +1046,7 @@
 static int wino4_epm(const sda_conv_desc* d, const Wino4Geom& g) {
     static const bool epi_on = !(getenv("SDA_W4_EPI") && atoi(getenv("SDA_W4_EPI")) == 0);
     const bool epi = epi_on && g.mf == 3 && ((d->res != nullptr) != (d->dact_z != nullptr)) && g.nstage >= 12 &&
-                     (!d->dact_z || d->act_d == SDA_ACT_SILU);
+                     (!d->dact_z || d->act_d == SDA_ACT_SILU || d->dact_mul);
     return epi ? 1 : ((d->res || d->dact_z) ? 2 : 0);
 }
 
@@ -1019,6 +1082,7 @@
               : epm == 2 ? wino4_launch_t<MOD, LN, SILU, 2, 0>(d, g, grid, stream)                                             \
                          : wino4_launch_t<MOD, LN, SILU, 0, 0>(d, g, grid, stream))
     const int zp = wino4_zp(d, g);
+    if (d->act_out != SDA_ACT_NONE || d->dact_mul) return sda_wino4_launch_epx(d, g, grid, epm, stream);
 #ifdef SDA_W4_VARIANTS
     if (zp && getenv("SDA_W4_VAR") && atoi(getenv("SDA_W4_VAR")) == 11) {
         static long long* tbuf = nullptr;
@@ -1174,3 +1238,4 @@
     hipLaunchKernelGGL(pack_wino4_zp_kernel, dim3(blocks), dim3(256), 0, (hipStream_t)stream, w_wino4, dst, k_pad / 8, m_pad / W4_BM_OF(mf), mf);
     return sda_launch_status();
 }
+#endif
diff --git a/sda_amd/csrc/conv_wino4_act.hip b/sda_amd/csrc/conv_wino4_act.hip
--- /dev/null
+++ b/sda_amd/csrc/conv_wino4_act.hip
@@ -0,0 +1,2 @@
+#define SDA_W4_ACT_UNIT
+#include "conv_wino4.hip"
diff --git a/sda_amd/engine.py b/sda_amd/engine.py
--- a/sda_amd/engine.py
+++ b/sda_amd/engine.py
@@ -7,7 +7,7 @@
 from torch import Tensor
 
 from . import ops
-from ._lib import SdaHipError
+from ._lib import ACT_IDS, SdaHipError
 from .ops import PackedConv, conv_out_size, make_conv_desc
 
 
@@ -144,7 +144,8 @@
                 zins=(1, 1), bias: Optional[Tensor] = None, mod: Optional[Tensor] = None, mod_sn: int = 0,
                 ln=None, act_in: int = 0, dact_z: Optional[Tensor] = None, act_d: int = 0, res: Optional[Tensor] = None,
                 ctx: Optional[Tensor] = None, cctx: int = 0, ctx_sn: int = 0, pad=None, parity4_w: Optional[Tensor] = None,
-                pool=(1, 1), x_amax=None, out_amax: Optional[Tensor] = None, h2_only: bool = False):
+                pool=(1, 1), x_amax=None, out_amax: Optional[Tensor] = None, h2_only: bool = False,
+                act_out: int = 0, out_dact: Optional[Tensor] = None, dact_mul: bool = False, plan_only: bool = False):
     out_strides = (0, 0, 0, 0)
     if not out.is_contiguous():
         out_strides = tuple(out.stride())
@@ -164,7 +165,14 @@
                        dact_z_ptr=None if dact_z is None else dact_z.data_ptr(), act_d=act_d,
                        res_ptr=None if res is None else res.data_ptr(),
                        w_wino4_ptr=None if getattr(pk, 'wino4', None) is None else pk.wino4.data_ptr(),
-                       pad=pad, out_strides=out_strides, pool=pool, w_wino4_zp_ptr=None if zp is None else zp.data_ptr())
+                       pad=pad, out_strides=out_strides, pool=pool, w_wino4_zp_ptr=None if zp is None else zp.data_ptr(),
+                       act_out=act_out, out_dact_ptr=None if out_dact is None else out_dact.data_ptr(), dact_mul=dact_mul)
+    if plan_only:
+        return ops.conv_path(d)
+    if act_out or dact_mul:
+        assert getattr(pk, 'h2', None) is None and parity4_w is None and tuple(pool) == (1, 1) and not h2_only
+        ops.conv_igemm(d)
+        return d
     if pool != (1, 1):
         if tuple(pool) == (2, 2) and ops.H2_POOL and x_amax is not None and getattr(pk, 'h2', None) is not None:
             packing = pk.h2_pool()
@@ -569,7 +577,27 @@
         row = mod_all[lo:] if per_image else mod_all
         return row[:, blk.mod_off:], (self.mod_total if per_image else 0)
 
-    def _block_fwd(self, blk: _Block, a: Tensor, mod_all, lo, per_image, saved):
+    def _act_once(self, blk: _Block, a: Tensor, mod, mod_sn) -> bool:
+        n, c, h, w = a.shape
+        if not ops.act_once_width(c) or blk.act != ACT_IDS['SiLU'] or mod is None:
+            return False
+        key = (n, h, w, mod_sn, a.device, ops.MULTIPLY)
+        hit = getattr(blk, '_act_once', None)
+        if hit is None or hit[0] != key:
+            c1, c2 = blk.conv1, blk.conv2
+            p1, p2, p2t = c1.fwd(), c2.fwd(), c2.bwd()
+            ok = all(getattr(pk, 'h2', None) is None for pk in (p1, p2, p2t)) and (c1.sh, c1.sw, c2.sh, c2.sw) == (1, 1, 1, 1)
+            if ok:
+                t = torch.empty_like(a)
+                src = planar_source(t)
+                ok = (launch_conv(p1, src, t, h, w, circular=c1.circular, bias=p1.bias, mod=mod, mod_sn=mod_sn, ln=(t, t),
+                                  act_out=blk.act, out_dact=a, plan_only=True) == 2 and
+                      launch_conv(p2, src, t, h, w, circular=c2.circular, bias=p2.bias, res=a, plan_only=True) == 2 and
+                      launch_conv(p2t, src, t, h, w, circular=c2.circular, dact_z=a, dact_mul=True, plan_only=True) == 2)
+            hit = blk._act_once = (key, ok)
+        return hit[1]
+
+    def _block_fwd(self, blk: _Block, a: Tensor, mod_all, lo, per_image, saved, train: bool = False):
         n, c, h, w = a.shape
         dev = a.device
         mod, mod_sn = self._mod_for(blk, mod_all, lo, per_image)
@@ -589,6 +617,18 @@
         mean = torch.empty(n * h * w, device=dev, dtype=torch.float32)
         rstd = torch.empty_like(mean)
         ops.ln_stats(a, mod, mod_sn, blk.ln.eps, self.unbiased, mean, rstd)
+        if not train and self._act_once(blk, a, mod, mod_sn):
+            s = torch.empty_like(a)
+            dz = torch.empty_like(a) if saved is not None else None
+            pk = c1.fwd()
+            launch_conv(pk, planar_source(a), s, h, w, circular=c1.circular, bias=pk.bias, mod=mod, mod_sn=mod_sn, ln=(mean, rstd),
+                        act_out=blk.act, out_dact=dz)
+            y = torch.empty_like(a)
+            pk = c2.fwd()
+            launch_conv(pk, planar_source(s), y, h, w, circular=c2.circular, bias=pk.bias, res=a)
+            if saved is not None:
+                saved.append((a, mean, rstd, None, dz))
+            return y
         z = torch.empty_like(a)
         pk = c1.fwd()
         z_amax = getattr(pk, 'out_amax', None)
@@ -638,7 +678,7 @@
             dims.append((h, w))
             for bi, blk in enumerate(lev.descent):
                 rec = [] if save else None
-                a = self._block_fwd(blk, a, mod_all, lo, per_image, rec)
+                a = self._block_fwd(blk, a, mod_all, lo, per_image, rec, train)
                 if save:
                     saved['blocks'][('d', lvl, bi)] = rec[0]
             skips.append(a)
@@ -647,7 +687,7 @@
             lev = L[lvl]
             for bi, blk in enumerate(lev.ascent):
                 rec = [] if save else None
-                a = self._block_fwd(blk, a, mod_all, lo, per_image, rec)
+                a = self._block_fwd(blk, a, mod_all, lo, per_image, rec, train)
                 if save:
                     saved['blocks'][('a', lvl, bi)] = rec[0]
             tl = lev.tail
@@ -676,11 +716,13 @@
         return saved
 
     def _block_bwd(self, blk: _Block, g: Tensor, rec, mod_all, lo, per_image, g_amax_in=None, pg: Optional['ParamGrads'] = None):
-        a, mean, rstd, z = rec
+        a, mean, rstd, z = rec[:4]
+        dz = rec[4] if len(rec) > 4 else None
+        assert dz is None or (pg is None and z is None), 'the training route keeps z'
         n, c, h, w = a.shape
         mod, mod_sn = self._mod_for(blk, mod_all, lo, per_image)
         c1, c2 = blk.conv1, blk.conv2
-        if (pg is None and c1.circular == c2.circular and (c1.sh, c1.sw, c2.sh, c2.sw) == (1, 1, 1, 1) and
+        if (dz is None and pg is None and c1.circular == c2.circular and (c1.sh, c1.sw, c2.sh, c2.sw) == (1, 1, 1, 1) and
                 ops.block1d_eligible(c, h, c1.fwd(), c2.fwd())):
             gx = torch.empty_like(a)
             ops.block1d_bwd(g, a, z, mean, rstd, mod, mod_sn, c1.bwd(), c2.bwd(), c1.circular, blk.act, self.unbiased, gx)
@@ -690,7 +732,10 @@
         g_amax = gz_amax = None
         if getattr(pk2, 'h2', None) is not None and g.is_contiguous():
             g_amax, gz_amax = (g_amax_in if g_amax_in is not None else ops.absmax(g, pk2.in_amax)), pk2.out_amax
-        d2 = launch_conv(pk2, planar_source(g), gz, h, w, circular=c2.circular, dact_z=z, act_d=blk.act, x_amax=g_amax, out_amax=gz_amax)
+        if dz is not None:
+            d2 = launch_conv(pk2, planar_source(g), gz, h, w, circular=c2.circular, dact_z=dz, dact_mul=True)
+        else:
+            d2 = launch_conv(pk2, planar_source(g), gz, h, w, circular=c2.circular, dact_z=z, act_d=blk.act, x_amax=g_amax, out_amax=gz_amax)
         if not (d2 is not None and d2.w_h2):
             gz_amax = None
         if pg is not None:
diff --git a/sda_amd/ops.py b/sda_amd/ops.py
--- a/sda_amd/ops.py
+++ b/sda_amd/ops.py
@@ -74,7 +74,8 @@
                    stride_h=1, stride_w=1, circular=False, up_h=1, up_w=1, zins_h=1, zins_w=1,
                    ctx_ptr=None, cctx=0, ctx_sn=0, mod_ptr=None, mod_sn=0, ln_mean_ptr=None, ln_rstd_ptr=None,
                    act_in=0, bias_ptr=None, dact_z_ptr=None, act_d=0, res_ptr=None,
-                   w_wino4_ptr=None, pad=None, out_strides=(0, 0, 0, 0), pool=(1, 1), w_wino4_zp_ptr=None) -> ConvDesc:
+                   w_wino4_ptr=None, pad=None, out_strides=(0, 0, 0, 0), pool=(1, 1), w_wino4_zp_ptr=None,
+                   act_out=0, out_dact_ptr=None, dact_mul=False) -> ConvDesc:
     d = ConvDesc()
     d.x = x_ptr
     d.x_sn_outer, d.x_sn_inner, d.n_inner, d.x_n_off = x_sn_outer, x_sn_inner, n_inner, x_n_off
@@ -99,6 +100,7 @@
     d.out_sn, d.out_sc, d.out_sy, d.out_sx = out_strides
     d.pool_h, d.pool_w = pool
     d.w_wino4_zp = w_wino4_zp_ptr
+    d.act_out, d.out_dact, d.dact_mul = act_out, out_dact_ptr, int(bool(dact_mul))
     return d
 
 
@@ -218,6 +220,21 @@
 
 
 PARITY4 = os.environ.get('SDA_CONV_PAR4', '1') != '0'
+
+W4_ACT_ONCE = os.environ.get('SDA_W4_ACT_ONCE', '1') != '0'
+ACT_ONCE_CHANNELS = frozenset((384,))
+ACT_ONCE_FORCE = False
+
+
+def set_act_once(mode) -> object:
+    global W4_ACT_ONCE, ACT_ONCE_FORCE
+    prev = True if ACT_ONCE_FORCE else (None if W4_ACT_ONCE else False)
+    W4_ACT_ONCE, ACT_ONCE_FORCE = mode is not False, mode is True
+    return prev
+
+
+def act_once_width(c: int) -> bool:
+    return W4_ACT_ONCE and (ACT_ONCE_FORCE or c in ACT_ONCE_CHANNELS)
 WINO4_BM64 = os.environ.get('SDA_W4_BM64', '1') != '0'
 
 
```

Result: no change. 0.1374 diffusion-steps/s, median of 6 (+0.3%).
